# davidskdds/DMSA_LiDAR_SLAM

Measured on AMD Instinct MI355X. Metric: DMSA iterations/sec (10-scan window, 131072 pts/scan), higher is better.
Workload: dtype f32 points/Gaussians, f64 residual sums and normal equations

## Files before the change

### dmsa_lidar_slam_amd/_capi.py

```python
from __future__ import annotations

import ctypes as C
import os

import numpy as np

c_double_p = C.POINTER(C.c_double)
c_float_p = C.POINTER(C.c_float)
c_int32_p = C.POINTER(C.c_int32)
c_int64_p = C.POINTER(C.c_int64)
c_uint32_p = C.POINTER(C.c_uint32)
c_uint64_p = C.POINTER(C.c_uint64)

DMSA_OK = 0
DMSA_ERR_INVALID = -1
DMSA_ERR_NO_DEVICE = -2
DMSA_ERR_HIP = -3
DMSA_ERR_DEPTH = -4
DMSA_ERR_NOMEM = -5

STOP_NUM_ITER, STOP_FEW_GAUSSIANS, STOP_NAN, STOP_NO_IMPROVEMENT, STOP_EPSILON = range(5)

FLAG_POSE_TABLE_HOST = 0x1
FLAG_FIXED_ITERS = 0x2
# ... 262 lines not shown
        "dmsa_window_upload": (C.c_int, [vp, C.POINTER(WindowProblem)]),
        "dmsa_keyframes_upload": (C.c_int, [vp, C.POINTER(KeyframeProblem)]),
        "dmsa_centralize": (C.c_int, [vp]),
        "dmsa_decentralize": (C.c_int, [vp]),
        "dmsa_get_params": (C.c_int, [vp, c_double_p, c_int32_p]),
        "dmsa_set_params": (C.c_int, [vp, c_double_p]),
        "dmsa_additional_errors": (C.c_int, [vp, c_double_p, C.c_int32, c_int32_p]),
        "dmsa_pose_tables": (C.c_int, [vp, C.c_int32, c_double_p, c_float_p]),
        "dmsa_set_pose_tables": (C.c_int, [vp, C.c_int32, c_float_p]),
        "dmsa_num_table_rows": (C.c_int, [vp, c_int32_p]),
        "dmsa_transform_points": (C.c_int, [vp, C.c_int32, c_float_p]),
        "dmsa_build_gaussians": (C.c_int, [vp, C.POINTER(Settings), c_int32_p, c_int64_p]),
        "dmsa_eval_residuals": (C.c_int, [vp, c_double_p]),
        "dmsa_normal_equations": (C.c_int, [vp, C.c_int32, C.c_int32, c_double_p, C.c_double, C.c_double, c_double_p, c_double_p]),
        "dmsa_pose_table_derivatives": (C.c_int, [vp, c_double_p]),
        "dmsa_analytic_jacobian": (C.c_int, [vp, c_double_p, c_double_p]),
        "dmsa_get_voxel_level": (C.c_int, [vp, C.c_int32, C.POINTER(VoxelLevelInfo), c_uint64_p, c_uint32_p, c_int32_p]),
        "dmsa_get_gaussians": (C.c_int, [vp, c_int32_p, c_int32_p, c_float_p, c_float_p]),
        "dmsa_get_timing": (C.c_int, [vp, C.POINTER(Timing), C.c_int32]),
        "dmsa_synchronize": (C.c_int, [vp]),
        "dmsa_get_trace": (C.c_int, [vp, C.POINTER(IterTrace), C.c_int32]),
        "dmsa_detmath_eval": (C.c_int, [vp, C.c_int32, c_double_p, c_double_p, C.c_int64, c_double_p]),
        "dmsa_sort_pairs": (C.c_int, [vp, C.POINTER(C.c_uint32), C.POINTER(C.c_uint32), C.c_int64, C.c_uint32, C.POINTER(C.c_uint32), C.POINTER(C.c_uint32)]),
        "dmsa_leaf_segments": (C.c_int, [vp, C.POINTER(C.c_uint32), C.c_int64, C.c_uint32, c_int32_p, c_int32_p, c_int32_p]),
        "dmsa_serial_fallback_sums": (C.c_int, [vp, C.c_int32, C.POINTER(C.c_uint64)]),
        "dmsa_adaptive_step_size": (C.c_int, [vp, c_double_p, c_double_p, C.c_double, c_int32_p]),
        "dmsa_default_debug_options": (None, [C.POINTER(DebugOptions)]),
        "dmsa_create_ex": (C.c_int, [C.c_int, C.c_uint32, C.POINTER(DebugOptions), C.POINTER(vp)]),
        "dmsa_create_ex2": (C.c_int, [C.c_int, C.c_uint32, C.POINTER(DebugOptions), C.c_uint32, C.POINTER(vp)]),
        "dmsa_create_named": (C.c_int, [C.c_int, C.c_uint32, C.POINTER(DebugOptions), C.c_uint32, C.c_char_p, C.POINTER(vp)]),
        "dmsa_get_debug_counters": (C.c_int, [vp, C.POINTER(DebugCounters)]),
        "dmsa_debug_level_size_classes": (C.c_int, [vp, c_int32_p]),
        "dmsa_debug_next_head": (C.c_int, [vp, c_int64_p]),
        "dmsa_debug_pow_minus_one": (C.c_int, [vp, c_int32_p, C.c_int32, c_float_p]),
        "dmsa_debug_limit_covariance": (C.c_int, [vp, c_float_p, C.c_int64, c_float_p, c_float_p, c_float_p, c_int32_p, c_int32_p]),
        "dmsa_sort_pairs64": (C.c_int, [vp, c_uint64_p, c_uint32_p, C.c_int64, C.c_uint32, c_uint64_p, c_uint32_p]),
        "dmsa_scan_i32": (C.c_int, [vp, c_int32_p, C.c_int64, C.c_int32, c_int32_p]),
        "dmsa_window_upload_aos": (C.c_int, [vp, C.POINTER(WindowProblem), C.POINTER(AosView), C.c_int32, C.POINTER(AosView)]),
        "dmsa_keyframes_upload_aos": (C.c_int, [vp, C.POINTER(KeyframeProblem), C.POINTER(AosView), C.c_int32]),
        "dmsa_optimize_window_aos": (C.c_int, [vp, C.POINTER(WindowProblem), C.POINTER(AosView), C.c_int32, C.POINTER(AosView), C.POINTER(Settings), C.POINTER(Report)]),
        "dmsa_optimize_keyframes_aos": (C.c_int, [vp, C.POINTER(KeyframeProblem), C.POINTER(AosView), C.c_int32, C.POINTER(Settings), C.POINTER(Report)]),
        "dmsa_get_global_points_aos": (C.c_int, [vp, C.c_void_p, C.c_int64, C.c_int32, C.c_int32, C.c_int32]),
        "dmsa_reserve": (C.c_int, [vp, C.c_int64, C.c_int32, C.c_int32]),
        "dmsa_window_ring_push_aos": (C.c_int, [vp, C.POINTER(AosView), C.c_int32]),
        "dmsa_window_upload_from_ring_aos": (C.c_int, [vp, C.POINTER(WindowProblem), C.c_double, C.POINTER(AosView)]),
        "dmsa_window_ring_create": (C.c_int, [vp, C.POINTER(WindowRingConfig)]),
        "dmsa_window_ring_push": (C.c_int, [vp, c_float_p, c_double_p, c_int32_p, C.c_int64]),
        "dmsa_window_ring_points": (C.c_int, [vp, c_int32_p, c_int64_p]),
        "dmsa_window_upload_from_ring": (C.c_int, [vp, C.POINTER(WindowProblem), C.c_double]),
        "dmsa_lm_solve": (C.c_int, [c_double_p, c_double_p, C.c_int32, C.c_double, C.c_int32, c_double_p]),
        "dmsa_lm_solve_device": (C.c_int, [vp, c_double_p, c_double_p, C.c_int32, C.c_double, C.c_double, c_double_p, c_int32_p]),
        "dmsa_neighbourhood_ranges": (C.c_int, [C.c_int32, C.c_int32, C.POINTER(C.c_int32), C.POINTER(C.c_int32)]),
        "dmsa_submap_poses": (C.c_int, [C.c_int32, c_double_p, c_double_p, C.c_int32, C.c_int32, c_double_p, c_double_p, c_double_p, c_double_p]),
        "dmsa_update_poses_from_submap": (C.c_int, [C.c_int32, c_double_p, c_double_p, C.c_int32, C.c_int32, c_double_p, c_double_p]),
        "dmsa_select_static_points": (C.c_int, [vp, C.POINTER(StaticSelectProblem), c_float_p, c_int32_p, C.c_int64, c_int32_p, C.POINTER(StaticSelectResult)]),
        "dmsa_get_overlap": (C.c_int, [vp, c_float_p, C.c_int64, c_float_p, C.c_int64, C.c_float, c_float_p, c_int64_p]),
        "dmsa_random_grid_downsampling": (C.c_int, [vp, c_float_p, C.c_int64, C.c_float, C.c_uint32, c_int32_p, C.c_int64, c_int64_p]),
        "dmsa_radius_exists": (C.c_int, [vp, c_float_p, C.c_int64, c_float_p, C.c_int64, C.c_float, C.POINTER(C.c_uint8)]),
        "dmsa_preprocess_scan": (C.c_int, [vp, c_float_p, C.c_int64, C.POINTER(PreprocessConfig), c_float_p, c_int32_p, C.c_int64, c_int64_p, c_float_p]),
        "dmsa_imu_buffer_create": (C.c_int, [C.c_int32, C.POINTER(vp)]),
        "dmsa_imu_buffer_destroy": (None, [vp]),
        "dmsa_imu_buffer_add": (C.c_int, [vp, c_double_p, c_double_p, C.c_double]),
        "dmsa_imu_buffer_closest": (C.c_int, [vp, C.c_double, c_double_p, c_double_p, c_double_p]),
        "dmsa_imu_buffer_state": (C.c_int, [vp, c_int32_p, c_int32_p, c_double_p, c_double_p, c_double_p]),
        "dmsa_traj_dims": (C.c_int, [C.c_double, C.c_double, C.c_double, c_double_p, c_int32_p]),
        "dmsa_traj_grids": (C.c_int, [C.c_double, C.c_double, C.c_int32, C.c_int32, c_double_p, c_double_p, c_int32_p]),
# ... 42 lines not shown
        "dmsa_pcd_header_normals_binary": (C.c_int, [C.c_int64, C.c_char_p, C.c_int32]),
        "dmsa_dense_cloud_save_pcd_normals": (C.c_int, [vp, C.c_char_p, c_int64_p, c_int64_p]),
        "dmsa_default_dense_outlier_config": (None, [C.POINTER(DenseOutlierConfig)]),
        "dmsa_dense_cloud_knn_mean_distance": (C.c_int, [vp, C.POINTER(DenseOutlierConfig), C.c_int64, C.c_int64, c_float_p]),
        "dmsa_dense_cloud_classify_outliers": (C.c_int, [vp, C.POINTER(DenseOutlierConfig), C.POINTER(C.c_uint8), C.POINTER(DenseOutlierStats)]),
        "dmsa_dense_outlier_threshold": (C.c_int, [C.c_int64, C.c_int64, C.c_int64, C.c_float, c_double_p, c_double_p, c_double_p]),
        "dmsa_dense_cloud_remove_outliers": (C.c_int, [vp, c_int64_p]),
        "dmsa_dense_cloud_save_pcd_retained": (C.c_int, [vp, C.c_char_p, c_int64_p, c_int64_p]),
        "dmsa_default_dense_carve_config": (None, [C.POINTER(DenseCarveConfig)]),
        "dmsa_dense_carve_walk": (C.c_int, [C.c_float, c_float_p, c_float_p, c_int32_p, C.c_int64, c_int64_p]),
        "dmsa_dense_carve_sees_through": (C.c_int, [C.POINTER(DenseCarveConfig), c_float_p, c_float_p, c_float_p]),
        "dmsa_dense_cloud_carve_walk_rows": (C.c_int, [vp, C.POINTER(DenseCarveConfig), C.c_int64, C.c_int64, c_int32_p, c_uint64_p]),
        "dmsa_dense_cloud_count_passes": (C.c_int, [vp, C.POINTER(DenseCarveConfig), c_uint32_p, C.POINTER(DenseCarveStats)]),
        "dmsa_dense_cloud_remove_transients": (C.c_int, [vp, c_int64_p]),
        "dmsa_dense_cloud_with_intensity": (C.c_int, [vp]),
        "dmsa_dense_cloud_has_intensity": (C.c_int, [vp]),
        "dmsa_decode_pointcloud2_field": (C.c_int, [vp, C.POINTER(PointCloud2), C.POINTER(PointCloud2Field), c_float_p]),
        "dmsa_dense_cloud_add_pointcloud2_field": (C.c_int, [vp, C.POINTER(PointCloud2), C.c_int32, C.POINTER(PointCloud2Field), c_float_p, C.c_int64, c_int64_p,
                                                             C.POINTER(DenseStats)]),
        "dmsa_sensor_intensity_field": (C.c_int, [C.c_int32, C.POINTER(PointCloud2Field)]),
        "dmsa_pcd_header_xyzi_binary": (C.c_int, [C.c_int64, C.c_char_p, C.c_int32]),
        "dmsa_pcd_header_xyzi_normals_binary": (C.c_int, [C.c_int64, C.c_char_p, C.c_int32]),
    }
    for name, (res, args) in sig.items():
        fn = getattr(lib, name)
        fn.restype = res
        fn.argtypes = args
    _lib = lib
    return lib


EXPORTED_SYMBOLS = (
    "dmsa_window_upload_aos dmsa_keyframes_upload_aos dmsa_optimize_window_aos dmsa_optimize_keyframes_aos dmsa_get_global_points_aos dmsa_reserve dmsa_window_ring_push_aos dmsa_window_upload_from_ring_aos "
    "dmsa_create dmsa_create_ex dmsa_create_ex2 dmsa_create_named dmsa_default_debug_options dmsa_get_debug_counters dmsa_debug_next_head dmsa_debug_level_size_classes dmsa_debug_pow_minus_one dmsa_debug_limit_covariance dmsa_sort_pairs64 dmsa_scan_i32 dmsa_destroy dmsa_last_error dmsa_default_settings dmsa_optimize_window dmsa_optimize_keyframes "
    "dmsa_get_global_points dmsa_window_upload dmsa_keyframes_upload dmsa_centralize dmsa_decentralize dmsa_get_params "
    "dmsa_set_params dmsa_additional_errors dmsa_pose_tables dmsa_set_pose_tables dmsa_num_table_rows dmsa_transform_points dmsa_build_gaussians "
    "dmsa_eval_residuals dmsa_normal_equations dmsa_pose_table_derivatives dmsa_analytic_jacobian dmsa_get_voxel_level dmsa_get_gaussians dmsa_get_timing dmsa_synchronize dmsa_get_trace dmsa_detmath_eval dmsa_lm_solve dmsa_lm_solve_device dmsa_serial_fallback_sums dmsa_sort_pairs dmsa_leaf_segments dmsa_neighbourhood_ranges dmsa_submap_poses dmsa_update_poses_from_submap dmsa_optimize_resident dmsa_adaptive_step_size dmsa_get_poses "
    "dmsa_select_static_points dmsa_get_overlap dmsa_random_grid_downsampling dmsa_radius_exists dmsa_preprocess_scan "
    "dmsa_imu_buffer_create dmsa_imu_buffer_destroy dmsa_imu_buffer_add dmsa_imu_buffer_closest dmsa_imu_buffer_state dmsa_traj_dims dmsa_traj_grids "
    "dmsa_traj_tform_indices dmsa_traj_transfer_imu dmsa_traj_preint_factors dmsa_traj_update_initial_guess dmsa_traj_submap_gravity_estimate "
    "dmsa_window_ring_create dmsa_window_ring_push dmsa_window_ring_points dmsa_window_upload_from_ring "
    "dmsa_raw_open dmsa_raw_close dmsa_raw_next dmsa_raw_create dmsa_raw_write_pointcloud2 dmsa_raw_write_imu dmsa_raw_finish "
    "dmsa_decode_pointcloud2 dmsa_format_tum_pose dmsa_compose_nonkeyframe_pose dmsa_update_normals dmsa_make_keyframe_cloud "
    "dmsa_get_global_normals dmsa_pcd_header_pointnormal dmsa_format_pcd_rows dmsa_save_pcd_ascii dmsa_save_pcd_ascii_ex"
).split()

DENSE_CLOUD_SYMBOLS = (
    "dmsa_default_dense_config dmsa_dense_cloud_create dmsa_dense_cloud_destroy dmsa_dense_cloud_interpolate dmsa_dense_cloud_add_scan "
    "dmsa_dense_cloud_add_pointcloud2 dmsa_dense_cloud_stats dmsa_dense_cloud_reserve dmsa_dense_cloud_table_info dmsa_pcd_header_xyz_binary "
    "dmsa_dense_cloud_open_pcd dmsa_dense_cloud_close_pcd dmsa_parse_tum_poses"
).split()

DENSE_NORMALS_SYMBOLS = (
    "dmsa_default_dense_normals_config dmsa_dense_cloud_retain dmsa_dense_cloud_retained dmsa_dense_cloud_neighbour_moments "
    "dmsa_dense_cloud_compute_normals dmsa_dense_normal_from_moments dmsa_pcd_header_normals_binary dmsa_dense_cloud_save_pcd_normals"
).split()

DENSE_OUTLIERS_SYMBOLS = (
    "dmsa_default_dense_outlier_config dmsa_dense_cloud_knn_mean_distance dmsa_dense_cloud_classify_outliers dmsa_dense_outlier_threshold "
    "dmsa_dense_cloud_remove_outliers dmsa_dense_cloud_save_pcd_retained"
).split()

DENSE_CARVE_SYMBOLS = (
    "dmsa_default_dense_carve_config dmsa_dense_carve_walk dmsa_dense_carve_sees_through dmsa_dense_cloud_carve_walk_rows "
    "dmsa_dense_cloud_count_passes dmsa_dense_cloud_remove_transients"
).split()

# ... 5 lines not shown
```

### dmsa_lidar_slam_amd/api.py

```python
from __future__ import annotations

import ctypes as C

import numpy as np

from . import _capi as capi
from .problems import ContinuousTrajectory, DmsaOptimSettings, MapManagement


class DmsaError(RuntimeError):
    pass


NAMED_SWITCHES = ("fit_by_level", "batch_stamps", "one_readback", "next_head")


class DmsaOptimizer:

    def __init__(self, device: int = 0, pose_table_host: bool = False, fixed_iters: bool = False, stage_timers: bool = False, debug: dict | None = None):
        self._lib = capi.load_library()
        self._ctx = C.c_void_p()
        flags = (capi.FLAG_POSE_TABLE_HOST if pose_table_host else 0) | (capi.FLAG_FIXED_ITERS if fixed_iters else 0)
        flags |= capi.FLAG_STAGE_TIMERS if stage_timers else 0
        if debug:
            opts = capi.DebugOptions()
            self._lib.dmsa_default_debug_options(C.byref(opts))
            named = []
            for k, v in debug.items():
                if k in NAMED_SWITCHES:
                    named.append(f"{k}={int(v)}")
                elif not hasattr(opts, k):
                    raise KeyError(f"unknown debug switch {k!r} (include/dmsa_debug.h)")
                else:
                    setattr(opts, k, int(v))
            rc = self._lib.dmsa_create_named(int(device), flags, C.byref(opts), C.sizeof(opts), ",".join(named).encode() if named else None, C.byref(self._ctx))
        else:
            rc = self._lib.dmsa_create(int(device), flags, C.byref(self._ctx))
        if rc != capi.DMSA_OK:
            self._ctx = None
            raise DmsaError(f"dmsa_create(device={device}) failed with {rc} (no usable HIP device; there is no CPU fallback)")
        self._problem = None
        self._cprob = None

    def close(self):
        if getattr(self, "_ctx", None):
            self._lib.dmsa_destroy(self._ctx)
            self._ctx = None
# ... 114 lines not shown
        return out

    def limitCovariance(self, cov):
        A = np.ascontiguousarray(np.asarray(cov, np.float32).reshape(-1, 3, 3))
        n = A.shape[0]
        At = np.ascontiguousarray(A.transpose(0, 2, 1))
        out, Vt = np.zeros_like(At), np.zeros_like(At)
        ev = np.zeros((n, 3), np.float32)
        it, info = np.zeros(n, np.int32), np.zeros(n, np.int32)
        self._check(self._lib.dmsa_debug_limit_covariance(self._ctx, capi.ptr(At, C.c_float), n, capi.ptr(out, C.c_float), capi.ptr(ev, C.c_float),
                                                          capi.ptr(Vt, C.c_float), capi.ptr(it, C.c_int32), capi.ptr(info, C.c_int32)), "debug_limit_covariance")
        return np.ascontiguousarray(out.transpose(0, 2, 1)), ev, np.ascontiguousarray(Vt.transpose(0, 2, 1)), it, info

    def optimizeResident(self, settings: DmsaOptimSettings) -> capi.Report:
        cs = settings.to_c()
        rep = capi.Report()
        self._check(self._lib.dmsa_optimize_resident(self._ctx, C.byref(cs), C.byref(rep)), "optimize_resident")
        return rep

    def adaptiveStepSize(self, params, step, error0: float):
        p = np.ascontiguousarray(params, np.float64).copy()
        st = np.ascontiguousarray(step, np.float64)
        k = C.c_int32()
        self._check(self._lib.dmsa_adaptive_step_size(self._ctx, capi.ptr(p, C.c_double), capi.ptr(st, C.c_double), float(error0), C.byref(k)), "adaptive_step_size")
        return p, int(k.value)

    def debugCounters(self) -> dict:
        c = capi.DebugCounters()
        self._check(self._lib.dmsa_get_debug_counters(self._ctx, C.byref(c)), "get_debug_counters")
        out = {n: int(getattr(c, n)) for n, _ in c._fields_}
        head = np.zeros(2, np.int64)
        self._check(self._lib.dmsa_debug_next_head(self._ctx, capi.ptr(head, C.c_int64)), "debug_next_head")
        out["next_head_iterations"], out["next_head_mismatches"] = int(head[0]), int(head[1])
        return out

    def levelSizeClasses(self):
        out = np.zeros(9, np.int32)
        self._check(self._lib.dmsa_debug_level_size_classes(self._ctx, capi.ptr(out, C.c_int32)), "debug_level_size_classes")
        return out[:8].reshape(2, 4).copy(), bool(out[8])

    def lastError(self) -> str:
        msg = self._lib.dmsa_last_error(self._ctx)
        return msg.decode() if msg else ""

    def poses(self):
        p = self._problem
        n = p.relOrientations.shape[0]
        ro, rt = np.zeros((n, 3)), np.zeros((n, 3))
        self._check(self._lib.dmsa_get_poses(self._ctx, capi.ptr(ro, C.c_double), capi.ptr(rt, C.c_double)), "get_poses")
        return ro, rt

    def globalPoints(self) -> np.ndarray:
        n = self._num_points()
        out = np.zeros((n, 4), np.float32)
        self._check(self._lib.dmsa_get_global_points(self._ctx, capi.ptr(out, C.c_float), n), "get_global_points")
        return out

    def getGlobalNormals(self) -> np.ndarray:
        n = self._num_points()
        out = np.zeros((n, 4), np.float32)
        self._check(self._lib.dmsa_get_global_normals(self._ctx, capi.ptr(out, C.c_float), n), "get_global_normals")
        return out

    def upload(self, pointSet):
        cp = pointSet.to_c()
        if isinstance(pointSet, ContinuousTrajectory):
# ... 210 lines not shown
```

### dmsa_lidar_slam_amd/csrc/context.cpp

```cpp
#include "dmsa_ctx.h"

#include <cstddef>

WorkerPool& workers(dmsa_ctx* ctx) {
    if (!ctx->pool) {
        const unsigned want = (unsigned)std::max(1, ctx->dbg.host_threads);
        ctx->pool = new WorkerPool((int)std::min(want, std::max(2u, std::thread::hardware_concurrency())));
    }
    return *ctx->pool;
}
hipEvent_t get_event(dmsa_ctx* ctx) {
    if (!ctx->free_events.empty()) {
        hipEvent_t e = ctx->free_events.back();
        ctx->free_events.pop_back();
        return e;
    }
    hipEvent_t e;
    (void)hipEventCreate(&e);
    return e;
}
void drain_timers(dmsa_ctx* ctx) {
    std::vector<EventPair> later;
    for (auto& ev : ctx->pending) {
        if (hipEventQuery(ev.b) == hipErrorNotReady) {
// ... 324 lines not shown
    SW(key_compress, 1, kMin, kMax),
    SW(fused_segments, 1, kMin, kMax),
    SW(sort_prehist, 0, kMin, kMax),
    SW(overlap_batch, 1, kMin, kMax),
    SW(serial_tree, 1, 0, 3),
    SW(host_threads, 16, 1, 64),
    SW(solve_threads, 12, 1, 16),
    SW(host_timeline, 0, kMin, kMax),
    SW(trace_time, 0, kMin, kMax),
    SW(fused_leaf_scan, 1, kMin, kMax),
    SW(device_sync, 1, kMin, kMax),
    SW(shared_rotations, 1, kMin, kMax),
    SW(eval_skip, 1, kMin, kMax),
    SW(sync_fault, 0, kMin, kMax),
    SW(speculation_fault, 0, kMin, kMax),
    SW(voxel_coherence, 0, kMin, kMax),
    SW(lm_stream, 1, kMin, kMax),
    SW(stream_priority, 0, kMin, kMax),
    SW(gap_stamps, 0, kMin, kMax),
    SW(lattice_hint, 1, kMin, kMax),
    SW(fit_classes, 7, kMin, kMax),
    SW(eigen_l1_bytes, 32 * 1024, 4096, kMax, true),
    SW(small_threshold, 0, kMin, kMax),
    SW(skip_stats, 0, kMin, kMax),
    SW(small_voxel, 0, kMin, kMax),
    SW(long_split, 1, kMin, kMax),
    SW(long_log2, 0, kMin, kMax),
    SW(sort_items, 0, kMin, kMax),
    SW(trial_rows_aside, 1, kMin, kMax),
    {"batch_stamps", sizeof(dmsa_debug_options), 1, 0, 1},
    {"one_readback", sizeof(dmsa_debug_options) + 4, 1, 0, 1},
    {"fit_by_level", sizeof(dmsa_debug_options) + 8, 1, 0, 2},
    {"next_head", sizeof(dmsa_debug_options) + 12, 1, 0, 3},
};
#undef SW
constexpr size_t kNumSwitches = sizeof(kSwitches) / sizeof(kSwitches[0]);
static_assert(kNumSwitches == sizeof(dmsa_switches) / 4 && sizeof(dmsa_switches) == sizeof(dmsa_debug_options) + 16, "one table row per field of dmsa_switches");
constexpr bool switches_in_struct_order() {
    for (size_t i = 0; i < kNumSwitches; ++i)
        if (kSwitches[i].offset != 4 * i) return false;
    return true;
}
static_assert(switches_in_struct_order(), "row i of the table describes field i of dmsa_switches");
int32_t& value(dmsa_switches* o, const Switch& sw) { return *reinterpret_cast<int32_t*>(reinterpret_cast<char*>(o) + sw.offset); }
bool is_public(const Switch& sw) { return sw.offset < sizeof(dmsa_debug_options); }
int32_t& public_value(dmsa_debug_options* o, const Switch& sw) { return *reinterpret_cast<int32_t*>(reinterpret_cast<char*>(o) + sw.offset); }
}

extern "C" {

void dmsa_default_debug_options(dmsa_debug_options* o) {
    if (!o) return;
    for (const Switch& sw : kSwitches)
        if (is_public(sw)) public_value(o, sw) = sw.def;
}
static void apply_named_switches(dmsa_switches* o, const char* e, const char* where) {
    if (!e) return;
    std::string text(e);
    size_t at = 0;
    while (at < text.size()) {
        size_t end = text.find(',', at);
        if (end == std::string::npos) end = text.size();
        const std::string item = text.substr(at, end - at);
        const size_t eq = item.find('=');
        if (eq != std::string::npos) {
            const std::string name = item.substr(0, eq);
            bool known = false;
            for (const Switch& sw : kSwitches)
                if (name == sw.name) value(o, sw) = std::atoi(item.c_str() + eq + 1), known = true;
            if (!known) std::fprintf(stderr, "[dmsa] %s: unknown switch '%s' ignored\n", where, name.c_str());
// ... 10 lines not shown
}
int dmsa_create_named(int device, uint32_t flags, const dmsa_debug_options* options, uint32_t options_bytes, const char* named, dmsa_ctx** out) {
    if (!out) return DMSA_ERR_INVALID;
    dmsa_switches dbg;
    for (const Switch& sw : kSwitches) value(&dbg, sw) = sw.def;
    if (options) {
        if (options_bytes < 4 || options_bytes % 4 != 0 || options_bytes > sizeof(dmsa_debug_options)) return DMSA_ERR_INVALID;
        std::memcpy(static_cast<dmsa_debug_options*>(&dbg), options, options_bytes);
    }
    apply_named_switches(&dbg, named, "dmsa_create_named");
    apply_named_switches(&dbg, std::getenv("DMSA_DEBUG"), "DMSA_DEBUG");
    for (const Switch& sw : kSwitches) {
        int32_t& v = value(&dbg, sw);
        v = v < sw.lo ? (sw.low_is_default ? sw.def : sw.lo) : std::min(v, sw.hi);
    }
    *out = nullptr;
    int count = 0;
    if (hipGetDeviceCount(&count) != hipSuccess || count <= 0 || device < 0 || device >= count) return DMSA_ERR_NO_DEVICE;
    if (hipSetDevice(device) != hipSuccess) return DMSA_ERR_NO_DEVICE;
    dmsa_ctx* ctx = new (std::nothrow) dmsa_ctx();
    if (!ctx) return DMSA_ERR_NOMEM;
    if (flags & ~(DMSA_FLAG_POSE_TABLE_HOST | DMSA_FLAG_FIXED_ITERS | DMSA_FLAG_MIRROR_SUMS | DMSA_FLAG_STAGE_TIMERS)) {
        delete ctx;
        return DMSA_ERR_INVALID;
    }
    ctx->device = device, ctx->flags = flags;
    ctx->dbg = dbg;
    int prio_least = 0, prio_greatest = 0;
    (void)hipDeviceGetStreamPriorityRange(&prio_least, &prio_greatest);
    auto make_stream = [&](hipStream_t* st, int bit) {
        return hipStreamCreateWithPriority(st, hipStreamNonBlocking, ((dbg.stream_priority >> bit) & 1) ? prio_greatest : prio_least / 2 + prio_greatest / 2);
    };
    bool made = make_stream(&ctx->stream, 0) == hipSuccess && make_stream(&ctx->stream2, 1) == hipSuccess && make_stream(&ctx->stream3, 2) == hipSuccess &&
                hipEventCreateWithFlags(&ctx->ev_counts, hipEventDisableTiming) == hipSuccess;
    for (StreamDep* d : ctx->deps) made = made && d->create_events() == hipSuccess;
    if (!made) {
        dmsa_destroy(ctx);
        return DMSA_ERR_HIP;
    }
    if (ctx->h_rb.ensure(sizeof(dmsa_ctx::Readback), nullptr) != hipSuccess) {
        dmsa_destroy(ctx);
        return DMSA_ERR_NOMEM;
    }
    std::memset(ctx->h_rb.p, 0, sizeof(dmsa_ctx::Readback));
    ctx->h_lattice = ctx->rb()->lattice;
    if (hipDeviceGetAttribute(&ctx->wall_clock_khz, hipDeviceAttributeWallClockRate, device) != hipSuccess || ctx->wall_clock_khz <= 0)
        ctx->wall_clock_khz = 0, ctx->dbg.batch_stamps = 0;
    if (ctx->d_sync.ensure(SYNC_SLOTS * 4) != hipSuccess || hipMemsetAsync(ctx->d_sync.p, 0, SYNC_SLOTS * 4, ctx->stream) != hipSuccess ||
        ctx->d_batch_clock.ensure(16) != hipSuccess || hipMemsetAsync(ctx->d_batch_clock.p, 0, 16, ctx->stream) != hipSuccess || hipStreamSynchronize(ctx->stream) != hipSuccess) {
        dmsa_destroy(ctx);
        return DMSA_ERR_HIP;
    }
    *out = ctx;
    return DMSA_OK;
}

void dmsa_destroy(dmsa_ctx* ctx) {
    if (!ctx) return;
    (void)hipSetDevice(ctx->device);
    for (hipStream_t st : {ctx->stream, ctx->stream2, ctx->stream3})
        if (st) (void)hipStreamSynchronize(st);
    drain_timers(ctx);
    for (hipEvent_t e : ctx->free_events) (void)hipEventDestroy(e);
    if (ctx->ev_counts) (void)hipEventDestroy(ctx->ev_counts);
    delete ctx->pool;
    pcd_release(ctx);
    delete ctx->sp;
    for (hipStream_t st : {ctx->stream3, ctx->stream2, ctx->stream})
        if (st) (void)hipStreamDestroy(st);
    delete ctx;
}

const char* dmsa_last_error(const dmsa_ctx* ctx) { return ctx ? ctx->err.c_str() : "null context"; }

void dmsa_default_settings(dmsa_settings* s) {
    if (!s) return;
    s->num_iter = 15, s->epsilon = 1e-5, s->use_analytic_jacobi = 0, s->step_length_optim = 0.05, s->max_step = 0.01, s->gauss_split = 0;
    s->grid_size_1_factor = 2.0f, s->grid_size_2_factor = 5.0f, s->min_num_points_per_set = 6, s->min_num_gaussians = 30;
    s->lambda_diag = 0.00001f, s->use_centralization = 1;
}

int dmsa_window_upload(dmsa_ctx* ctx, const dmsa_window_problem* p) {
    if (!ctx || !p || p->num_points < 0 || p->num_static < 0) return DMSA_ERR_INVALID;
    if ((p->num_points > 0 && (!p->xyz_local || !p->tform_idx || !p->ring_id)) || (p->num_static > 0 && (!p->xyz_static || !p->ring_id_static))) {
        ctx->err = "invalid window problem (null point arrays)";
        return DMSA_ERR_INVALID;
    }
    CHK(window_upload_begin(ctx, p, p->num_points, p->num_static));
    const size_t n = (size_t)ctx->n;
    CHK(ensure_stage(ctx, n * 20 + 64));
    float* loc = ctx->h_stage.as<float>();
    int32_t* ring = reinterpret_cast<int32_t*>(ctx->h_stage.as<char>() + n * 16);
    const int32_t id_row = p->n_total;
    const int64_t N = ctx->N, S = ctx->S;
    std::atomic<bool> bad_row{false};
    auto pack = [&](int64_t i0, int64_t i1) {
        for (int64_t i = i0; i < i1; ++i) {
            if (i < N) {
                const int32_t row = p->tform_idx[i];
                if (row < 0 || row >= p->n_total) {
                    bad_row = true;
// ... 61 lines not shown
```

### dmsa_lidar_slam_amd/csrc/dev_sync.h

```cpp
#pragma once
#include <hip/hip_runtime.h>

#include <cstdint>

namespace dmsa {

struct DevSync {
    const uint32_t* wait_counter = nullptr;
    uint32_t wait_target = 0;
    uint32_t* signal_counter = nullptr;
    int32_t* timed_out = nullptr;
};

struct BatchStamp {
    const long long* begin = nullptr;
    unsigned long long* ticks = nullptr;
};

enum SyncSlot : int {
    SYNC_TIER_FORK = 0,
    SYNC_TIER_JOIN = 1,
    SYNC_TIMED_OUT = 2,
    SYNC_LOOP_STATE = 5,
    SYNC_TABLES = 6,
    SYNC_CLASSES = 7,
    SYNC_LATTICE = 8,
    SYNC_LEVEL1 = 9,
    SYNC_SMALL_L0 = 10,
    SYNC_TRIAL_STEP = 11,
    SYNC_TRIAL_ROWS = 12,
    SYNC_SIZES0 = 13,
    SYNC_SIZES1 = 14,
    SYNC_CLASSES0 = 15,
    SYNC_CLASSES1 = 16,
    SYNC_FIT1 = 17,
    SYNC_BATCH_BEGIN = 18,
    SYNC_SLOTS = 24
};

#if defined(__HIPCC__)
__device__ __forceinline__ void dev_sync_signal(uint32_t* counter) {
    __threadfence();
    __hip_atomic_fetch_add(counter, 1u, __ATOMIC_RELAXED, __HIP_MEMORY_SCOPE_AGENT);
}
constexpr int kSyncMaxSpins = 1 << 23;
__device__ __forceinline__ void dev_sync_wait(const uint32_t* counter, uint32_t target, int32_t* timed_out, int max_spins = kSyncMaxSpins) {
    uint32_t v = 0;
    for (int spin = 0; spin < max_spins; ++spin) {
        v = __hip_atomic_load(counter, __ATOMIC_RELAXED, __HIP_MEMORY_SCOPE_AGENT);
        if ((int32_t)(v - target) >= 0) {
            __builtin_amdgcn_fence(__ATOMIC_ACQUIRE, "agent");
            return;
        }
        if (spin < 4096)
            __builtin_amdgcn_s_sleep(1);
        else
            __builtin_amdgcn_s_sleep(8);
    }
    if (timed_out != nullptr) timed_out[0] = 1, timed_out[1] = (int32_t)target, timed_out[2] = (int32_t)v;
}
__device__ __forceinline__ void dev_sync_enter(const DevSync& sy) {
    if (sy.wait_counter != nullptr && threadIdx.x == 0) dev_sync_wait(sy.wait_counter, sy.wait_target, sy.timed_out);
}
__device__ __forceinline__ void dev_sync_leave(const DevSync& sy) {
    if (sy.signal_counter != nullptr) {
        __syncthreads();
        if (threadIdx.x == 0) dev_sync_signal(sy.signal_counter);
    }
}
// ... 9 lines not shown
```

### dmsa_lidar_slam_amd/csrc/dmsa_api.cpp

```cpp
#include "dmsa_ctx.h"

extern "C" {


int dmsa_centralize(dmsa_ctx* ctx) {
    if (!ctx || ctx->model == MODEL_NONE) return DMSA_ERR_INVALID;
    if (ctx->model == MODEL_KEYFRAMES) return DMSA_OK;
    if (ctx->centralized) return DMSA_OK;
    CHK(set_device(ctx));
    WindowHost& w = ctx->win;
    w.origin = {w.ctrl.rel_t[0], w.ctrl.rel_t[1], w.ctrl.rel_t[2]};
    w.ctrl.rel_t[0] = w.ctrl.rel_t[1] = w.ctrl.rel_t[2] = 0.0;
    w.ctrl.relative_to_global();
    launch_shift_points(ctx->d_local.as<float4>() + ctx->N, ctx->S, (float)w.origin.x, (float)w.origin.y, (float)w.origin.z, -1.0f, ctx->stream);
    HIPCHK(hipGetLastError());
    ctx->centralized = true;
    return DMSA_OK;
}

int dmsa_decentralize(dmsa_ctx* ctx) {
    if (!ctx || ctx->model == MODEL_NONE) return DMSA_ERR_INVALID;
    if (ctx->model == MODEL_KEYFRAMES) return DMSA_OK;
    if (!ctx->centralized) return DMSA_OK;
    CHK(set_device(ctx));
// ... 367 lines not shown
    out->skip_pairs = (int64_t)st[0], out->skip_pairs_equal = (int64_t)st[1], out->skip_mismatches = (int64_t)st[2];
    unsigned long long sp[2] = {0, 0};
    if (ctx->d_split_stats.p) {
        unsigned long long stripes[128];
        HIPCHK(hipStreamSynchronize(ctx->stream));
        HIPCHK(hipStreamSynchronize(ctx->stream2));
        HIPCHK(hipMemcpy(stripes, ctx->d_split_stats.p, sizeof(stripes), hipMemcpyDeviceToHost));
        for (int k = 0; k < 64; ++k) sp[0] += stripes[2 * k], sp[1] += stripes[2 * k + 1];
    }
    out->split_blocks = (int64_t)sp[0], out->split_blocks_skipped = (int64_t)sp[1];
    unsigned long long changed = 0;
    if (ctx->d_coh_count.p) {
        HIPCHK(hipStreamSynchronize(ctx->stream));
        HIPCHK(hipMemcpy(&changed, ctx->d_coh_count.p, 8, hipMemcpyDeviceToHost));
    }
    out->voxel_codes_compared = ctx->coh_compared, out->voxel_codes_changed = (int64_t)changed, out->voxel_lattice_changes = ctx->coh_lattice_changes;
    out->lattice_hints_held = ctx->lattice_hints_held, out->lattice_replays = ctx->lattice_replays;
    out->small_voxel_launches = ctx->small_voxel_launches, out->small_voxel_fallbacks = ctx->small_voxel_fallbacks;
    return DMSA_OK;
}

int dmsa_debug_next_head(dmsa_ctx* ctx, int64_t* out2) {
    if (!ctx || !out2) return DMSA_ERR_INVALID;
    CHK(set_device(ctx));
    unsigned long long differing = 0;
    if (ctx->d_head_mismatches.p) {
        HIPCHK(hipStreamSynchronize(ctx->stream));
        HIPCHK(hipMemcpy(&differing, ctx->d_head_mismatches.p, 8, hipMemcpyDeviceToHost));
    }
    out2[0] = ctx->next_head_iterations, out2[1] = (int64_t)differing;
    return DMSA_OK;
}

int dmsa_debug_level_size_classes(dmsa_ctx* ctx, int32_t* out9) {
    if (!ctx || !out9) return DMSA_ERR_INVALID;
    std::memset(out9, 0, 9 * sizeof(int32_t));
    if (!ctx->gaussians_valid || !ctx->fit_guess_level) return DMSA_OK;
    for (int l = 0; l < 2; ++l) {
        const SerialCounts& c = ctx->serial_counts_level[l];
        out9[4 * l] = c.n_long, out9[4 * l + 1] = c.n_chain - c.n_long, out9[4 * l + 2] = c.n_small, out9[4 * l + 3] = c.max_members;
    }
    out9[8] = 1;
    return DMSA_OK;
}

int dmsa_get_timing(dmsa_ctx* ctx, dmsa_timing* t, int32_t reset) {
    if (!ctx) return DMSA_ERR_INVALID;
    CHK(set_device(ctx));
    HIPCHK(enqueue_batch_ticks(ctx));
    HIPCHK(hipStreamSynchronize(ctx->stream));
    drain_timers(ctx);
    if (t) {
        t->residual_kernel_ms = ctx->t_ms[T_RESIDUAL], t->residual_launches = ctx->residual_launches, t->residual_evaluations = ctx->residual_evals;
        t->residual_algorithmic_bytes = ctx->residual_bytes;
        t->residual_unit_bytes = ctx->residual_unit_bytes;
        t->voxelize_ms = ctx->t_ms[T_VOXEL], t->gaussian_fit_ms = ctx->t_ms[T_FIT], t->pose_table_ms = ctx->t_ms[T_TABLE];
        t->normal_eq_ms = ctx->t_ms[T_NORMAL], t->total_ms = ctx->t_ms[T_TOTAL];
    }
    if (reset) {
        for (double& v : ctx->t_ms) v = 0.0;
        ctx->residual_launches = 0, ctx->residual_evals = 0, ctx->residual_bytes = 0.0, ctx->residual_unit_bytes = 0.0;
    }
    return DMSA_OK;
}

int dmsa_sort_pairs(dmsa_ctx* ctx, const uint32_t* keys, const uint32_t* values, int64_t n, uint32_t end_bit, uint32_t* keys_sorted, uint32_t* values_sorted) {
// ... 207 lines not shown
```

### dmsa_lidar_slam_amd/csrc/dmsa_ctx.h

```cpp
#pragma once
#include <hip/hip_runtime.h>

#include <algorithm>
#include <atomic>
#include <cassert>
#include <chrono>
#include <cmath>
#include <condition_variable>
#include <cstddef>
#include <cstdio>
#include <cstdlib>
#include <cstring>
#include <functional>
#include <limits>
#include <mutex>
#include <string>
#include <thread>
#include <vector>

#include "../../include/dmsa_hip.h"
#include "../../include/dmsa_debug.h"
#include "../../include/dmsa_static_points.h"
#include "../../include/dmsa_window_setup.h"
#include "../../include/dmsa_wire_formats.h"
// ... 210 lines not shown
    long generation_ = 0;
    bool stop_ = false;
};

struct WindowRing {
    int num_scans = 0;
    int64_t cap = 0;
    int head = 0, filled = 0;
    std::vector<int64_t> count;
    DevBuf xyz, stamp, id;
};

struct HostTimeline {
    bool on = false;
    std::vector<std::pair<const char*, std::chrono::steady_clock::time_point>> marks;
    void reset() { marks.clear(); }
    void mark(const char* what) {
        if (on) marks.emplace_back(what, std::chrono::steady_clock::now());
    }
    void print() const {
        if (!on || marks.size() < 2) return;
        std::fprintf(stderr, "[host timeline]");
        for (size_t i = 1; i < marks.size(); ++i)
            std::fprintf(stderr, " %s %.0f |", marks[i].first, std::chrono::duration<double, std::micro>(marks[i].second - marks[i - 1].second).count());
        std::fprintf(stderr, " total %.0f us\n", std::chrono::duration<double, std::micro>(marks.back().second - marks.front().second).count());
    }
};

struct dmsa_switches : dmsa_debug_options {
    int32_t batch_stamps = 1;
    int32_t one_readback = 1;
    int32_t fit_by_level = 1;
    int32_t next_head = 1;
};

struct dmsa_ctx {
    int device = 0;
    uint32_t flags = 0;
    WindowRing ring;
    dmsa_switches dbg{};
    hipStream_t stream = nullptr, stream2 = nullptr;
    hipStream_t stream3 = nullptr;
    StreamDep tier_fork{this, SYNC_TIER_FORK, 1}, tier_join{this, SYNC_TIER_JOIN, 2} , loop_state{this, SYNC_LOOP_STATE, 1},
        tables{this, SYNC_TABLES, 1}, classes{this, SYNC_CLASSES, 1}, lattice{this, SYNC_LATTICE, 1}, level1{this, SYNC_LEVEL1, 1}, small_l0{this, SYNC_SMALL_L0, 0},
        trial_step{this, SYNC_TRIAL_STEP, 0}, trial_rows{this, SYNC_TRIAL_ROWS, 0}, sizes0{this, SYNC_SIZES0, 1}, sizes1{this, SYNC_SIZES1, 1},
        classes0{this, SYNC_CLASSES0, 1}, classes1{this, SYNC_CLASSES1, 1}, fit1{this, SYNC_FIT1, 1};
    StreamDep* const deps[15] = {&tier_fork, &tier_join, &loop_state, &tables, &classes, &lattice, &level1, &small_l0, &trial_step, &trial_rows,
                                 &sizes0, &sizes1, &classes0, &classes1, &fit1};
    int tablesT_batch = 0;
    hipEvent_t ev_counts = nullptr;
    std::string err;

    Model model = MODEL_NONE;
    int64_t n = 0, N = 0, S = 0;
    int rows = 0;
    WindowHost win;
    KeyframeHost key;
    bool centralized = false;
    float min_grid_size = 0.3f;

    DevBuf d_local, d_nlocal, d_ring, d_global, d_nglobal;
    DevBuf d_tables, d_ctrl, d_stamps, d_fhw, d_trajtime;
    int batch = 0;
    PinnedRing h_pin, h_xpin;
    std::vector<float> h_tables;
    PinnedBuf h_stage;
    DevBuf d_aabb, d_code[2], d_idx[2], d_code_s[2], d_idx_s[2], d_head[2], d_leaf_incl[2], d_leaf_start[2], d_slot_acc[2], d_slot_cnt[2],
        d_gauss_of_slot[2], d_memb_of_slot[2], d_pos_slot_rank[2], d_nsorted[2], d_pair_d[2], d_sort_tmp[2], d_scan_tmp[2];
    struct Readback {
        LatticeTable lattice[2];
        GaussCounts g;
        SerialCounts sc;
        SerialCounts sc_level[2];
        IterResult prev;
        double errs[16];
        unsigned long long batch_ticks;
    };
    static constexpr size_t kReadbackBytes = offsetof(Readback, errs);
    DevBuf d_readback;
    DevView d_lattice, d_counts;
    IterResult* d_prev_result() const { return reinterpret_cast<IterResult*>(d_readback.as<char>() + offsetof(Readback, prev)); }
// ... 26 lines not shown
    int64_t lattice_hints_held = 0, lattice_replays = 0;
    DevBuf d_fit_sums;
    DevBuf d_memb_q;
    DevBuf d_pow_codes;
    int64_t pow_n = 0;
    DevBuf d_gauss_rows;
    DevBuf d_row_range;
    DevBuf d_skip_stats;
    int skip_stats_evals = 0;
    DevBuf d_code_prev[2], d_coh_count;
    LatticeTable coh_lattice[2]{};
    bool coh_valid[2] = {false, false}, coh_key32[2] = {false, false}, coh_pending[2] = {false, false}, coh_count_zeroed = false;
    int64_t coh_n[2] = {0, 0};
    int64_t coh_compared = 0, coh_lattice_changes = 0;
    DevBuf d_split_stats;
    int64_t skip_pairs = 0;
    bool fit_guess_valid = false;
    SerialCounts serial_counts{0, 0, 0, 0};
    SerialCounts serial_counts_level[2] = {{0, 0, 0, 0}, {0, 0, 0, 0}};
    bool fit_guess_level = false;
    bool E_is_jacobian = false;
    bool aabb_fresh = false;
    const float* base_table = nullptr;
    LoopModel loop_model{};
    DevBuf d_imu_idx, d_imu_rot, d_imu_pos, d_imu_vel, d_imu_cov;
    DevBuf d_key_grav, d_key_plaus, d_key_odom_t, d_key_odom_R;
    DevBuf d_loop_state;
    DevBuf d_loop_vec;
    DevBuf d_ctrl0;
    DevBuf d_table0;
    DevBuf d_trial_tables;
    DevBuf d_head_check, d_head_mismatches;
    int64_t next_head_iterations = 0;
    DevBuf d_loop_extra;
    DevBuf d_loop_iter;
    DevBuf d_panel_work;
    uint32_t panel_epoch = 0;
    int panel_P = -1;
    DevBuf d_rot_same;
    DevBuf d_sync;
    int wait_seq = 0;
    long long* stamp_voxel = nullptr;
    long long* stamp_fit = nullptr;
    int voxel_calls = 0;
    int small_voxel_launches = 0, small_voxel_fallbacks = 0;
    int sync_retries = 0, speculation_retries = 0;
    DevBuf d_aos_raw, d_aos_idx;
    DevBuf d_static_keep;
    DevBuf d_ctrl_pm, d_dT;
    PinnedBuf h_results;
    const void* rb_extra_src = nullptr;
    void* rb_extra_dst = nullptr;
    size_t rb_extra_bytes = 0;
    int M = 0, M1 = 0;
    int64_t Mm = 0;
    bool gaussians_valid = false;
    DevBuf d_E, d_ne_partial, d_Hp, d_sq_partial, d_sq_out;
    int64_t ldE = 0;
    int extra_rows = 0;
    DevBuf d_batch_clock;
    unsigned long long batch_ticks_seen = 0;
    int wall_clock_khz = 0;
    bool batch_ticks_dirty = false, batch_ticks_in_flight = false;
    std::vector<EventPair> pending;
    std::vector<hipEvent_t> free_events;
    double t_ms[T_COUNT] = {0, 0, 0, 0, 0, 0};
// ... 40 lines not shown
        if (!on) return;
        (void)hipEventRecord(ev.b, ctx->stream);
        ctx->pending.push_back(ev);
    }
};
void drain_timers(dmsa_ctx* ctx);
hipError_t enqueue_batch_ticks(dmsa_ctx* ctx);
hipError_t sync_spin(hipStream_t stream);
int set_device(dmsa_ctx* ctx);
bool sync_wait_timed_out(dmsa_ctx* ctx, std::string* what);
int num_params(const dmsa_ctx* ctx);
PoseChain& chain(dmsa_ctx* ctx);
int num_extra_rows(const dmsa_ctx* ctx);
int alloc_point_buffers(dmsa_ctx* ctx);
int upload_powm1_codes(dmsa_ctx* ctx, int64_t counts);
int upload_loop_model(dmsa_ctx* ctx);
int upload_common(dmsa_ctx* ctx);
void write_back_poses(const PoseChain& c, double* rel_o, double* rel_t);
int ensure_stage(dmsa_ctx* ctx, size_t bytes);
int window_upload_begin(dmsa_ctx* ctx, const dmsa_window_problem* p, int64_t N, int64_t S);
int window_upload_finish(dmsa_ctx* ctx, const dmsa_window_problem* p);
int keyframes_upload_begin(dmsa_ctx* ctx, const dmsa_keyframe_problem* p, int64_t n_points);
int keyframes_upload_finish(dmsa_ctx* ctx, const dmsa_keyframe_problem* p);
int pointcloud2_layout(const dmsa_pointcloud2* msg, int32_t sensor, PointCloud2Fields* f_out, uint64_t* n_out);
int pointcloud2_field_layout(const dmsa_pointcloud2* msg, uint32_t index, uint32_t datatype, uint32_t* offset_out);
void pcd_release(dmsa_ctx* ctx);
int build_gaussians(dmsa_ctx* ctx, const dmsa_settings& s, const std::function<int()>& overlap = nullptr, bool allow_speculation = true,
                    bool allow_compression = true, bool allow_small = true);
int build_tables(dmsa_ctx* ctx, int B, const std::vector<double>& globs, hipStream_t stream = nullptr);
void append_glob(const PoseChain& c, std::vector<double>& out);
void host_set_params(dmsa_ctx* ctx, const double* p);
int transform_points(dmsa_ctx* ctx, int b);
int ensure_E(dmsa_ctx* ctx, int B);
int run_residuals(dmsa_ctx* ctx, int B, const std::vector<double>* extra, const double* d_extra = nullptr, const uint32_t* rot_same = nullptr,
                  const int2* row_range = nullptr );
int device_lm_step(dmsa_ctx* ctx, const double* d_Hp, int P, double lambda, double alpha, double max_step, double* d_step, LoopFlags* d_flags);
constexpr double kTableDerivStep = 1e-5;
int check_analytic_jacobian(dmsa_ctx* ctx, int P);
int host_table_derivatives(dmsa_ctx* ctx, hipStream_t stream);
int upload_extra(dmsa_ctx* ctx, const std::vector<double>& extra, int B);
int analytic_columns(dmsa_ctx* ctx, int P, double inv_h, const float* table0);
int optimize(dmsa_ctx* ctx, const dmsa_settings& s, dmsa_report* rep);
int adaptive_step_size(dmsa_ctx* ctx, double* params, const double* step, double error0, int32_t* best_k);
```

### dmsa_lidar_slam_amd/csrc/dmsa_kernels.h

```cpp
#pragma once
#include <hip/hip_runtime.h>
#include <cstdint>

#include "dev_sync.h"

namespace dmsa {

constexpr int kMaxLatticeEvents = 64;
constexpr int kAabbBlock = 1024;
constexpr uint32_t kStaticRowFlag = 0;

struct LatticeTable {
    int32_t num_events;
    int32_t final_depth;
    int32_t status;
    int32_t defined;
    int64_t first_idx;
    int64_t event_idx[kMaxLatticeEvents + 1];
    double mn[kMaxLatticeEvents + 1][3];
    uint32_t suffix_shift[kMaxLatticeEvents + 1][3];
    int32_t depth[kMaxLatticeEvents + 1];
    double final_mn[3];
    int32_t nbits[3];
    int32_t total_bits;
    uint32_t key_base[3];
    int32_t compressed;
    int32_t out_of_range;
    int32_t pad3;
    uint64_t code_or;
};
__host__ __device__ inline uint64_t lattice_invalid_code(const LatticeTable& t) {
    return (1ull << (t.compressed ? t.total_bits : 3 * t.final_depth)) | t.code_or;
}

struct LevelCounts {
    int32_t num_leaves;
    int32_t num_gauss;
    int32_t num_memb;
    int32_t pad;
};

struct GaussCounts {
// ... 15 lines not shown
    uint32_t* code_s[2];
    uint32_t* idx_s[2];
    GaussCounts* counts;
    float4* memb_local;
    int32_t* memb_idx;
    int32_t* memb_g;
    int32_t* seg_off;
    uint32_t* sync;
    uint32_t sync_target;
    int32_t* timed_out;
    long long* stamps;
};
int small_voxel_max_points();
void launch_voxel_small(const SmallVoxelArgs& a, hipStream_t s);

void launch_transform(const float4* local, const float4* table, float4* global, int64_t n, hipStream_t s);
void launch_transform_normals(const float4* local, const float4* nlocal, const float4* table, float4* global, float4* nglobal, int64_t n, hipStream_t s);
void launch_shift_points(float4* pts, int64_t n, float ox, float oy, float oz, float sign, hipStream_t s);

void launch_window_pose_tables(const double* ctrl, const double* stamps, const double* fh_w, const double* traj_time, int B, int C, int n_t,
                               float* tables, float* tablesT , hipStream_t s,
                               uint32_t* rot_same = nullptr );
void launch_keyframe_pose_tables(const double* frames, int B, int F, float* tables, float* tablesT, hipStream_t s, uint32_t* rot_same = nullptr);
void launch_window_pose_table_deriv(const double* ctrl_pm, const double* stamps, const double* fh_w, const double* traj_time, int P, int C, int n_t, double h,
                                    double* dT, hipStream_t s);
void launch_keyframe_pose_table_deriv(const double* ctrl_pm, int P, int F, double h, double* dT, hipStream_t s);

void launch_detmath_eval(int fn, const double* x, const double* y, int64_t n, double* out, hipStream_t s);

void launch_transform_aabb(const float4* local, const float4* nlocal, const float4* table, float4* global, float4* nglobal, int64_t n, float* aabb, void* zero,
                           size_t zero_bytes, hipStream_t s);
void launch_transform_aabb_adopt(const float4* local, float4* table0, const float4* trials, int rows, const int32_t* head_k, float4* global, int64_t n,
                                 float* aabb, void* zero, size_t zero_bytes, hipStream_t s);
void launch_count_word_mismatches(const void* a, const void* b, int words, unsigned long long* count, hipStream_t s);
void launch_block_aabb(const float4* global, int64_t n, float* aabb , void* zero, size_t zero_bytes, hipStream_t s);
void launch_lattice(const float4* global, int64_t n, const float* aabb, int nb, double res0, double res1, bool compress, LatticeTable* tables ,
                    void* sort_header0, void* sort_header1, hipStream_t s, uint32_t* done = nullptr ,
                    bool use_hint = false );
struct SortPlan;
void launch_voxel_keys(const float4* global, int64_t n, LatticeTable* table, double res, void* code, bool key32, uint32_t* idx, uint64_t code_or,
                       const SortPlan* sort, hipStream_t s);
void launch_head_flags(const void* code_sorted, bool key32, int64_t n, const LatticeTable* table, int32_t* head, hipStream_t s);
struct ChainedScanCall {
    unsigned long long* state;
    uint32_t epoch, ticket_base;
};
constexpr int kLeafSegmentWords = 1, kLeafFinalizeWords = 4;
int leaf_segment_tiles(int64_t n);
void launch_leaf_segments(const void* code_sorted, bool key32, int64_t n, const LatticeTable* table, int32_t* leaf_incl, int32_t* leaf_start, LevelCounts* counts,
                          const ChainedScanCall& call, hipStream_t s);
void launch_leaf_starts(const int32_t* head, const int32_t* leaf_of_pos, const void* code_sorted, bool key32, const LatticeTable* table, int64_t n,
                        int32_t* leaf_start, LevelCounts* counts, hipStream_t s);
void launch_leaf_accept(const int32_t* leaf_start, const uint32_t* idx_sorted, const int32_t* ring, const LevelCounts* counts, int min_pts,
                        int64_t capacity , int32_t* slot_acc , int32_t* slot_cnt, hipStream_t s);
size_t split_scratch_bytes(int64_t n);
void launch_leaf_split(const int32_t* leaf_incl, const int32_t* leaf_start, const uint32_t* idx_sorted, const int32_t* ring, const float4* nglobal,
                       const LevelCounts* counts, int min_pts, int64_t n, float4* nsorted , unsigned long long* pair_best ,
                       int32_t* slot_acc, int32_t* slot_cnt, int32_t* pos_slot_rank, hipStream_t s,
                       unsigned long long* block_stats = nullptr );
void launch_leaf_scan(const int32_t* slot_acc, const int32_t* slot_cnt, int32_t* gauss_of_slot, int32_t* memb_of_slot, LevelCounts* counts, hipStream_t s);
int leaf_finalize_tiles(int64_t n);
void launch_leaf_finalize(const int32_t* slot_acc, const int32_t* slot_cnt, int64_t n , int32_t* gauss_of_slot, int32_t* memb_of_slot,
                          LevelCounts* counts, const ChainedScanCall& call, hipStream_t s,
                          int32_t* gauss_size = nullptr );
void launch_count_code_changes(const void* now, void* prev, bool key32, int64_t n, bool compare, unsigned long long* count, hipStream_t s);
void launch_gather_members(const int32_t* leaf_of_pos, const int32_t* leaf_start, const uint32_t* idx_sorted, const void* code_sorted, bool key32,
                           const LatticeTable* table, const int32_t* slot_acc, const int32_t* gauss_of_slot, const int32_t* memb_of_slot,
                           const int32_t* pos_slot_rank , const float4* local, const int32_t* slot_cnt, const GaussCounts* counts, int level,
                           int64_t n, float4* memb_local, int32_t* memb_idx, int32_t* memb_g, int32_t* seg_off, hipStream_t s,
                           uint32_t* start_signal = nullptr );
void launch_gauss_fit_all(const float4* memb_local, const int32_t* seg_off, const float* table0, const uint32_t* order, const int32_t* sc, const int first[3],
                          const int tasks[3], float* sums, GaussCounts* counts, float* info12, bool with_weights, int id_row, int2* gauss_rows, int eigen_l1_bytes,
                          const uint32_t* pow_codes, int pow_n, float* memb_q , size_t q_stride, hipStream_t s,
                          const int32_t* size0 = nullptr, const int32_t* size1 = nullptr );
// ... 24 lines not shown
```

### dmsa_lidar_slam_amd/csrc/dmsa_kernels.hip

```cpp
#include "dmsa_kernels.h"
#include "dev_sync.h"
#include "k1_pose_math.h"
#include "radix_sort_dev.h"
#include "wave_prims.h"
#include "chained_scan.h"

#include <cfloat>
#include <climits>
#include <type_traits>
#include <cmath>
#include <cstdlib>
#include <cstring>
#include <cstdio>

#include "../../include/dmsa_detmath.h"
#include "../../include/dmsa_hip.h"

namespace dmsa {

__global__ __launch_bounds__(256) void k_transform(const float4* __restrict__ local, const float4* __restrict__ table, float4* __restrict__ global,
                                                   int64_t n) {
    const int64_t stride = (int64_t)gridDim.x * blockDim.x;
    for (int64_t i = (int64_t)blockIdx.x * blockDim.x + threadIdx.x; i < n; i += stride) {
        const float4 p = local[i];
// ... 305 lines not shown
        }
    }
    const int wave = threadIdx.x >> 6, lane = threadIdx.x & 63;
    for (int a = 0; a < 3; ++a) {
        mn[a] = wave_allminf(mn[a]);
        mx[a] = wave_allmaxf(mx[a]);
    }
    if (lane == 0)
        for (int a = 0; a < 3; ++a) s_red[wave][a] = mn[a], s_red[wave][3 + a] = mx[a];
    __syncthreads();
    if (threadIdx.x < 6) {
        float v = s_red[0][threadIdx.x];
        for (int w = 1; w < 4; ++w) v = threadIdx.x < 3 ? fminf(v, s_red[w][threadIdx.x]) : fmaxf(v, s_red[w][threadIdx.x]);
        aabb[(size_t)blockIdx.x * 8 + threadIdx.x] = v;
    }
}
template <bool kNormals>
__global__ __launch_bounds__(256) void k_transform_aabb(const float4* __restrict__ local, const float4* __restrict__ nlocal, const float4* __restrict__ table,
                                                        float4* __restrict__ global, float4* __restrict__ nglobal, int64_t n, float* __restrict__ aabb,
                                                        uint32_t* __restrict__ zero, int zero_words) {
    transform_aabb_body<kNormals>(local, nlocal, table, global, nglobal, n, aabb, zero, zero_words);
}
__global__ __launch_bounds__(256) void k_transform_aabb_adopt(const float4* __restrict__ local, float4* table0, const float4* trials, int table_f4,
                                                              const int32_t* __restrict__ head_k, float4* __restrict__ global, int64_t n,
                                                              float* __restrict__ aabb, uint32_t* __restrict__ zero, int zero_words) {
    const int k = *head_k;
    const float4* table = table0;
    if (k > 0) {
        table = trials + (size_t)(k - 1) * table_f4;
        for (int i = blockIdx.x * 256 + threadIdx.x; i < table_f4; i += gridDim.x * 256) table0[i] = table[i];
    }
    transform_aabb_body<false>(local, nullptr, table, global, nullptr, n, aabb, zero, zero_words);
}
__global__ __launch_bounds__(256) void k_count_word_mismatches(const uint32_t* __restrict__ a, const uint32_t* __restrict__ b, int words,
                                                               unsigned long long* __restrict__ count) {
    const int i = blockIdx.x * 256 + threadIdx.x;
    if (i < words && a[i] != b[i]) atomicAdd(count, 1ull);
}
void launch_transform_aabb_adopt(const float4* local, float4* table0, const float4* trials, int rows, const int32_t* head_k, float4* global, int64_t n,
                                 float* aabb, void* zero, size_t zero_bytes, hipStream_t s) {
    const int nb = (int)((n + kAabbBlock - 1) / kAabbBlock);
    hipLaunchKernelGGL(k_transform_aabb_adopt, dim3(nb), dim3(256), 0, s, local, table0, trials, 3 * rows, head_k, global, n, aabb, static_cast<uint32_t*>(zero),
                       (int)(zero_bytes / 4));
}
void launch_count_word_mismatches(const void* a, const void* b, int words, unsigned long long* count, hipStream_t s) {
    if (words > 0)
        hipLaunchKernelGGL(k_count_word_mismatches, dim3((words + 255) / 256), dim3(256), 0, s, static_cast<const uint32_t*>(a), static_cast<const uint32_t*>(b),
                           words, count);
}
void launch_transform_aabb(const float4* local, const float4* nlocal, const float4* table, float4* global, float4* nglobal, int64_t n, float* aabb, void* zero,
                           size_t zero_bytes, hipStream_t s) {
    if (n <= 0) {
        if (zero_bytes) (void)hipMemsetAsync(zero, 0, zero_bytes, s);
        return;
    }
    const int nb = (int)((n + kAabbBlock - 1) / kAabbBlock);
    if (nlocal)
        hipLaunchKernelGGL(k_transform_aabb<true>, dim3(nb), dim3(256), 0, s, local, nlocal, table, global, nglobal, n, aabb, static_cast<uint32_t*>(zero),
                           (int)(zero_bytes / 4));
    else
        hipLaunchKernelGGL(k_transform_aabb<false>, dim3(nb), dim3(256), 0, s, local, nlocal, table, global, nglobal, n, aabb, static_cast<uint32_t*>(zero),
                           (int)(zero_bytes / 4));
}
void launch_block_aabb(const float4* global, int64_t n, float* aabb, void* zero, size_t zero_bytes, hipStream_t s) {
    if (n <= 0) {
        if (zero_bytes) (void)hipMemsetAsync(zero, 0, zero_bytes, s);
        return;
    }
    const int nb = (int)((n + kAabbBlock - 1) / kAabbBlock);
    hipLaunchKernelGGL(k_block_aabb, dim3(nb), dim3(256), 0, s, global, n, aabb, static_cast<uint32_t*>(zero), (int)(zero_bytes / 4));
}

struct LatticeRun {
    double mn[3], mx[3];
    int depth, defined, nev, status;
};

__device__ void lattice_adopt(LatticeRun& st, const float4 p, const double res, int64_t idx, LatticeTable* tab, uint32_t (*shifts)[3]) {
    const double eps = (double)FLT_EPSILON;
    const float pc[3] = {p.x, p.y, p.z};
    while (true) {
// ... 18 lines not shown
            side = (double)(1u << st.depth) * res - eps;
            for (int a = 0; a < 3; ++a) st.mx[a] = st.mn[a] + side;
            tab->event_idx[st.nev] = idx;
            st.nev += 1;
            for (int a = 0; a < 3; ++a) tab->mn[st.nev][a] = st.mn[a];
            tab->depth[st.nev] = st.depth;
        } else {
            for (int a = 0; a < 3; ++a) {
                st.mn[a] = (double)pc[a] - res / 2;
                st.mx[a] = (double)pc[a] + res / 2;
            }
            unsigned mk[3];
            for (int a = 0; a < 3; ++a) mk[a] = (unsigned)ceil((st.mx[a] - st.mn[a] - eps) / res);
            const unsigned mv = max(max(max(mk[0], mk[1]), mk[2]), 2u);
            st.depth = (int)max(min(32u, (unsigned)ceil(log((double)mv) / log(2.0) - eps)), 0u);
            const double side = (double)(1u << st.depth) * res;
            for (int a = 0; a < 3; ++a) {
                const double over = (side - (st.mx[a] - st.mn[a])) / 2.0;
                if (over > eps) {
                    st.mn[a] -= over;
                    st.mx[a] += over;
                }
            }
            st.defined = 1;
            tab->first_idx = idx;
            for (int a = 0; a < 3; ++a) tab->mn[0][a] = st.mn[a];
            tab->depth[0] = st.depth;
        }
    }
}

constexpr int kLatticeThreads = 1024;
constexpr int kLatticeLdsBlocks = 2048;
__global__ __launch_bounds__(kLatticeThreads) void k_lattice(const float4* __restrict__ global, int64_t n, const float* __restrict__ aabb, int nb, double res0,
                                                            double res1, int compress, LatticeTable* __restrict__ tables, uint32_t* __restrict__ sort_header0,
                                                            uint32_t* __restrict__ sort_header1, uint32_t* done ,
                                                            int use_hint ) {
    static_assert(kLatticeThreads == kAabbBlock, "one thread per point of a block");
#ifdef DMSA_LATTICE_TIMING
    const long long lt0 = wall_clock64();
#define LAT_STAMP(k) if (threadIdx.x == 0) tables[blockIdx.x].mn[kMaxLatticeEvents - 8 + (k)][0] = (double)(wall_clock64() - lt0);
#else
#define LAT_STAMP(k)
#endif
    {
        uint32_t* h = blockIdx.x == 0 ? sort_header0 : sort_header1;
        if (h != nullptr)
            for (unsigned i = threadIdx.x; i < sizeof(SortHeader) / 4; i += kLatticeThreads) h[i] = 0u;
    }
    constexpr int kWaves = kLatticeThreads / 64;
    __shared__ float s_glob[kWaves][6];
    __shared__ LatticeRun st;
    __shared__ uint32_t s_shift[kMaxLatticeEvents][3];
    __shared__ int s_red[2][kWaves];
    __shared__ float s_bb[kLatticeLdsBlocks][6];
    int red_phase = 0;
    LatticeTable* tab = tables + blockIdx.x;
    const double res = blockIdx.x == 0 ? res0 : res1;
    const int tid = threadIdx.x, wave = tid >> 6, lane = tid & 63;
    if (tid == 0) {
        st.defined = 0, st.depth = 0, st.nev = 0, st.status = 0;
        for (int a = 0; a < 3; ++a) st.mn[a] = 0.0, st.mx[a] = 0.0;
        if (!use_hint) tab->first_idx = -1;
    }
    __shared__ int s_ok, s_E, s_nown;
    __shared__ long long s_ev[kMaxLatticeEvents + 1];
    __shared__ long long s_own[kMaxLatticeEvents + 1];
    __shared__ float4 s_q[kMaxLatticeEvents + 1];
    __shared__ double s_bmn[kMaxLatticeEvents + 1][3], s_bmx[kMaxLatticeEvents + 1][3];
    __shared__ double s_tmn[kMaxLatticeEvents + 1][3];
    __shared__ int s_tdepth[kMaxLatticeEvents + 1], s_hdr[3];
    __shared__ int s_e0[kMaxLatticeEvents + 2];
    __shared__ float s_fmn[kMaxLatticeEvents + 1][3], s_fmx[kMaxLatticeEvents + 1][3];
    if (use_hint && tid >= kLatticeThreads - 128 && tid - (kLatticeThreads - 128) <= kMaxLatticeEvents) {
        const int t = tid - (kLatticeThreads - 128);
        s_tdepth[t] = tab->depth[t];
        for (int a = 0; a < 3; ++a) s_tmn[t][a] = tab->mn[t][a];
        if (t < kMaxLatticeEvents) s_ev[1 + t] = tab->event_idx[t];
        if (t == 0) s_hdr[0] = tab->num_events, s_hdr[1] = tab->status, s_hdr[2] = tab->defined, s_ev[0] = tab->first_idx;
    }
    {
        float g6[6] = {INFINITY, INFINITY, INFINITY, -INFINITY, -INFINITY, -INFINITY};
        for (int b2 = tid; b2 < nb; b2 += kLatticeThreads) {
            const float4 lo = *reinterpret_cast<const float4*>(aabb + (size_t)b2 * 8), hi = *reinterpret_cast<const float4*>(aabb + (size_t)b2 * 8 + 4);
            const float bb[6] = {lo.x, lo.y, lo.z, lo.w, hi.x, hi.y};
            if (b2 < kLatticeLdsBlocks)
                for (int a = 0; a < 6; ++a) s_bb[b2][a] = bb[a];
            if (bb[0] <= bb[3])
                for (int a = 0; a < 3; ++a) g6[a] = fminf(g6[a], bb[a]), g6[3 + a] = fmaxf(g6[3 + a], bb[3 + a]);
        }
        for (int a = 0; a < 3; ++a) g6[a] = wave_allminf(g6[a]), g6[3 + a] = wave_allmaxf(g6[3 + a]);
        if (lane == 0)
            for (int a = 0; a < 6; ++a) s_glob[wave][a] = g6[a];
    }
    __syncthreads();
    auto block_min = [&](int v) {
        v = wave_allmin(v);
        if (lane == 0) s_red[red_phase][wave] = v;
        __syncthreads();
        int m = s_red[red_phase][0];
#pragma unroll
        for (int w = 1; w < kWaves; ++w) m = min(m, s_red[red_phase][w]);
        red_phase ^= 1;
        return m;
    };
    LAT_STAMP(0)
    constexpr int kHintBlocks = 12;
    bool verified = false;
    if (use_hint) {
        if (tid == 0) {
            const int E = s_hdr[0];
            const long long first = s_ev[0];
            int ok = s_hdr[1] == 0 && s_hdr[2] == 1 && E >= 0 && E <= kMaxLatticeEvents && first >= 0 && first < n && n < (1ll << 31) - kAabbBlock;
            int nown = 0;
            if (ok) {
                long long prev = first;
                s_own[nown] = first / kAabbBlock, s_e0[nown] = 0, nown += 1;
                for (int e = 0; e < E; ++e) {
                    const long long ie = s_ev[1 + e];
                    ok = ok && ie > first && ie >= prev && ie < n;
                    if (ok && ie / kAabbBlock != s_own[nown - 1]) s_own[nown] = ie / kAabbBlock, s_e0[nown] = e, nown += 1;
                    prev = ie;
                }
                s_e0[nown] = E;
            }
            ok = ok && nown <= kHintBlocks;
            s_ok = ok, s_E = ok ? E : 0, s_nown = ok ? nown : 0;
        }
        __syncthreads();
        LAT_STAMP(1)
        if (s_ok && tid <= s_E) s_q[tid] = global[s_ev[tid]];
        float4 own_pt[kHintBlocks];
        const int nown = s_nown;
#pragma unroll
        for (int k = 0; k < kHintBlocks; ++k) {
            const long long pi = k < nown ? s_own[k] * kAabbBlock + tid : n;
            own_pt[k] = pi < n ? global[pi] : make_float4(NAN, NAN, NAN, 0.0f);
        }
        __syncthreads();
        LAT_STAMP(2)
        if (s_ok && tid == 0) {
            const int E = s_E;
            const double eps = (double)FLT_EPSILON;
            LatticeRun c;
            c.defined = 0, c.depth = 0, c.nev = 0, c.status = 0;
            int ok = 1;
            {
                const float4 q = s_q[0];
                const float pc[3] = {q.x, q.y, q.z};
                ok = ok && isfinite(q.x) && isfinite(q.y) && isfinite(q.z);
                for (int a = 0; a < 3; ++a) c.mn[a] = (double)pc[a] - res / 2, c.mx[a] = (double)pc[a] + res / 2;
                unsigned mk[3];
                for (int a = 0; a < 3; ++a) mk[a] = (unsigned)ceil((c.mx[a] - c.mn[a] - eps) / res);
                const unsigned mv = max(max(max(mk[0], mk[1]), mk[2]), 2u);
                c.depth = (int)max(min(32u, (unsigned)ceil(log((double)mv) / log(2.0) - eps)), 0u);
                const double side = (double)(1u << c.depth) * res;
                for (int a = 0; a < 3; ++a) {
                    const double over = (side - (c.mx[a] - c.mn[a])) / 2.0;
                    if (over > eps) c.mn[a] -= over, c.mx[a] += over;
                }
                c.defined = 1;
                for (int a = 0; a < 3; ++a) ok = ok && __double_as_longlong(c.mn[a]) == __double_as_longlong(s_tmn[0][a]);
                ok = ok && c.depth == s_tdepth[0];
                for (int a = 0; a < 3; ++a) s_bmn[0][a] = c.mn[a], s_bmx[0][a] = c.mx[a];
            }
            for (int e = 0; e < E && ok; ++e) {
                const float4 q = s_q[1 + e];
                const float pc[3] = {q.x, q.y, q.z};
                ok = ok && isfinite(q.x) && isfinite(q.y) && isfinite(q.z);
                bool lo[3], hi[3], viol = false;
// ... 65 lines not shown
#pragma unroll
            for (int k = 0; k < kHintBlocks; ++k) {
                if (k < nown) {
                    const float4 q = own_pt[k];
                    const int base = (int)s_own[k] * kAabbBlock, e0 = s_e0[k], e1 = s_e0[k + 1];
                    float imn[3] = {s_fmn[e0][0], s_fmn[e0][1], s_fmn[e0][2]}, imx[3] = {s_fmx[e0][0], s_fmx[e0][1], s_fmx[e0][2]};
                    for (int e = e0 + 1; e <= e1; ++e)
                        for (int a = 0; a < 3; ++a) imn[a] = fmaxf(imn[a], s_fmn[e][a]), imx[a] = fminf(imx[a], s_fmx[e][a]);
                    const bool inside0 = base + tid > first32 && q.x >= imn[0] && q.x < imx[0] && q.y >= imn[1] && q.y < imx[1] && q.z >= imn[2] && q.z < imx[2];
                    if (!inside0 && isfinite(q.x) && isfinite(q.y) && isfinite(q.z)) {
                        int ep = e0;
                        bool trig = base + tid == first32;
                        for (int e = e0; e < e1; ++e) {
                            const int le = (int)s_ev[1 + e] - base;
                            ep += le < tid ? 1 : 0, trig = trig || le == tid;
                        }
                        const float c3[3] = {q.x, q.y, q.z};
                        if (base + tid < first32)
                            bad = 1;
                        else if (!trig && !fits(c3, c3, ep))
                            bad = 1;
                    }
                }
            }
            verified = block_min(bad ? 0 : 1) == 1;
        }
        LAT_STAMP(4)
        __syncthreads();
        if (!verified && tid == 0) {
            st.defined = 0, st.depth = 0, st.nev = 0, st.status = 0;
            for (int a = 0; a < 3; ++a) st.mn[a] = 0.0, st.mx[a] = 0.0;
            tab->first_idx = -1;
        }
        __syncthreads();
    }
    LAT_STAMP(5)
    int cursor = verified ? nb : 0;
    while (cursor < nb) {
        int found = INT_MAX;
        for (int base = cursor; base < nb; base += kLatticeThreads) {
            const int blk = base + tid;
            int cand = INT_MAX;
            if (blk < nb) {
                float bb[6];
                if (blk < kLatticeLdsBlocks) {
                    for (int a = 0; a < 6; ++a) bb[a] = s_bb[blk][a];
                } else {
                    for (int a = 0; a < 6; ++a) bb[a] = aabb[(size_t)blk * 8 + a];
                }
                if (bb[0] <= bb[3]) {
                    bool viol = !st.defined;
                    for (int a = 0; a < 3; ++a) viol = viol || (double)bb[a] < st.mn[a] || (double)bb[3 + a] >= st.mx[a];
                    if (viol) cand = blk;
                }
            }
            const int m = block_min(cand);
            if (m != INT_MAX) {
                found = m;
                break;
            }
        }
        if (found == INT_MAX) break;
        const int64_t pi = (int64_t)found * kAabbBlock + tid;
        float4 p = float4{0.0f, 0.0f, 0.0f, 0.0f};
        bool live = false;
        if (pi < n) {
            p = global[pi];
            live = isfinite(p.x) && isfinite(p.y) && isfinite(p.z);
        }
        int from = 0;
        while (true) {
            int cand = INT_MAX;
            if (live && tid >= from) {
                bool viol = !st.defined;
                viol = viol || (double)p.x < st.mn[0] || (double)p.x >= st.mx[0];
                viol = viol || (double)p.y < st.mn[1] || (double)p.y >= st.mx[1];
                viol = viol || (double)p.z < st.mn[2] || (double)p.z >= st.mx[2];
                if (viol) cand = tid;
            }
            const int m = block_min(cand);
            if (m == INT_MAX) break;
            if (tid == m) lattice_adopt(st, p, res, pi, tab, s_shift);
            __syncthreads();
            if (st.status != 0) break;
            from = m + 1;
        }
        if (st.status != 0) break;
        cursor = found + 1;
    }
    __syncthreads();
    LAT_STAMP(6)
    if (tid == 0) {
        tab->num_events = st.nev;
        tab->final_depth = st.depth;
        tab->status = st.status;
        tab->defined = st.defined;
        for (int a = 0; a < 3; ++a) tab->final_mn[a] = st.mn[a];
        int total = 0;
        for (int a = 0; a < 3; ++a) {
            float lo = s_glob[0][a], hi = s_glob[0][3 + a];
            for (int w = 1; w < kWaves; ++w) lo = fminf(lo, s_glob[w][a]), hi = fmaxf(hi, s_glob[w][3 + a]);
            int bits = st.depth;
            uint32_t base = 0;
            if (st.defined && lo <= hi) {
                const long long maxk = (1ll << st.depth) - 1;
                long long klo = (long long)floor(((double)lo - st.mn[a]) / res) - 1, khi = (long long)floor(((double)hi - st.mn[a]) / res) + 1;
                klo = klo < 0 ? 0 : klo, khi = khi > maxk ? maxk : khi;
                bits = 0;
                while (bits < st.depth && (klo >> bits) != (khi >> bits)) ++bits;
                base = (uint32_t)(klo >> bits);
            }
            tab->nbits[a] = bits, tab->key_base[a] = base;
            total += bits;
        }
        tab->compressed = compress, tab->out_of_range = 0, tab->code_or = 0;
        tab->pad3 = verified ? 1 : 0;
        tab->total_bits = total;
        uint32_t acc[3] = {0, 0, 0};
        for (int a = 0; a < 3; ++a) tab->suffix_shift[st.nev][a] = 0;
        for (int e = st.nev - 1; e >= 0; --e)
            for (int a = 0; a < 3; ++a) {
                acc[a] += s_shift[e][a];
                tab->suffix_shift[e][a] = acc[a];
            }
    }
    LAT_STAMP(7)
    if (done != nullptr) {
        __syncthreads();
        if (threadIdx.x == 0) dev_sync_signal(done);
    }
}
void launch_lattice(const float4* global, int64_t n, const float* aabb, int nb, double res0, double res1, bool compress, LatticeTable* tables,
                    void* sort_header0, void* sort_header1, hipStream_t s, uint32_t* done, bool use_hint) {
    hipLaunchKernelGGL(k_lattice, dim3(2), dim3(kLatticeThreads), 0, s, global, n, aabb, nb, res0, res1, compress ? 1 : 0, tables,
                       static_cast<uint32_t*>(sort_header0), static_cast<uint32_t*>(sort_header1), done, use_hint ? 1 : 0);
}

__device__ __forceinline__ uint64_t spread3(uint32_t v) {
    uint64_t x = v & 0x1fffffull;
    x = (x | x << 32) & 0x1f00000000ffffull;
    x = (x | x << 16) & 0x1f0000ff0000ffull;
    x = (x | x << 8) & 0x100f00f00f00f00full;
    x = (x | x << 4) & 0x10c30c30c30c30c3ull;
    x = (x | x << 2) & 0x1249249249249249ull;
    return x;
}

template <typename KeyT>
__global__ __launch_bounds__(256) void k_voxel_keys(const float4* __restrict__ global, int64_t n, LatticeTable* __restrict__ table, double res,
                                                    KeyT* __restrict__ code, uint32_t* __restrict__ idx, uint64_t code_or, SortHeader* __restrict__ sort_header,
                                                    uint32_t* __restrict__ sort_state, size_t sort_state_words, int sort_passes, uint32_t sort_last_mask) {
    __shared__ LatticeTable t;
    __shared__ uint32_t s_h[kSortMaxPasses][kSortBins];
    const bool counting = sort_header != nullptr && sizeof(KeyT) == 4;
    if (counting) {
        for (int p = 0; p < kSortMaxPasses; ++p) s_h[p][threadIdx.x] = 0u;
        for (size_t i = (size_t)blockIdx.x * blockDim.x + threadIdx.x; i < sort_state_words; i += (size_t)gridDim.x * blockDim.x) sort_state[i] = 0u;
    }
    {
        const int words = sizeof(LatticeTable) / 4;
        const uint32_t* src = reinterpret_cast<const uint32_t*>(table);
        uint32_t* dst = reinterpret_cast<uint32_t*>(&t);
        for (int i = threadIdx.x; i < words; i += blockDim.x) dst[i] = src[i];
    }
    __syncthreads();
    if (threadIdx.x == 0) t.code_or = code_or;
    if (blockIdx.x == 0 && threadIdx.x == 0) table->code_or = code_or;
    __syncthreads();
    const int nev = t.num_events;
    const uint64_t invalid = lattice_invalid_code(t);
    const int nx = t.nbits[0], ny = t.nbits[1], nz = t.nbits[2];
    const int maxb = max(nx, max(ny, nz));
    const int64_t last_ev = nev > 0 ? t.event_idx[nev - 1] : -1;
    const int64_t stride = (int64_t)gridDim.x * blockDim.x;
    for (int64_t i = (int64_t)blockIdx.x * blockDim.x + threadIdx.x; i < n; i += stride) {
        const float4 p = global[i];
        uint64_t c = invalid;
        if (isfinite(p.x) && isfinite(p.y) && isfinite(p.z)) {
            int e = nev;
            if (i < last_ev) {
                e = 0;
                while (e < nev && t.event_idx[e] <= i) ++e;
            }
            const uint32_t mask = (1u << t.depth[e]) - 1u;
            const uint32_t kx = ((uint32_t)(((double)p.x - t.mn[e][0]) / res) & mask) + t.suffix_shift[e][0];
            const uint32_t ky = ((uint32_t)(((double)p.y - t.mn[e][1]) / res) & mask) + t.suffix_shift[e][1];
            const uint32_t kz = ((uint32_t)(((double)p.z - t.mn[e][2]) / res) & mask) + t.suffix_shift[e][2];
            if (t.compressed) {
                if ((kx >> nx) != t.key_base[0] || (ky >> ny) != t.key_base[1] || (kz >> nz) != t.key_base[2]) table->out_of_range = 1;
                uint64_t cc = 0;
                for (int l = maxb - 1; l >= 0; --l) {
                    if (l < nx) cc = (cc << 1) | ((kx >> l) & 1u);
                    if (l < ny) cc = (cc << 1) | ((ky >> l) & 1u);
                    if (l < nz) cc = (cc << 1) | ((kz >> l) & 1u);
                }
                c = cc | code_or;
            } else {
                c = (spread3(kx) << 2) | (spread3(ky) << 1) | spread3(kz) | code_or;
            }
        }
        code[i] = (KeyT)c;
        idx[i] = (uint32_t)i;
        if (counting) sort_hist_add(s_h, sort_passes, sort_last_mask, (uint32_t)c, true);
    }
    if (counting) {
        __syncthreads();
        for (int p = 0; p < sort_passes; ++p) {
            const uint32_t v = s_h[p][threadIdx.x];
            if (v) atomicAdd(&sort_header->hist[p][threadIdx.x], v);
        }
    }
}
void launch_voxel_keys(const float4* global, int64_t n, LatticeTable* table, double res, void* code, bool key32, uint32_t* idx, uint64_t code_or,
                       const SortPlan* sort, hipStream_t s) {
    if (n <= 0) return;
    SortHeader* h = sort && key32 ? sort->header : nullptr;
    if (key32)
        hipLaunchKernelGGL(k_voxel_keys<uint32_t>, dim3(grid_for(n, 256)), dim3(256), 0, s, global, n, table, res, (uint32_t*)code, idx, code_or, h,
                           h ? sort->tile_state : nullptr, h ? sort->state_words : (size_t)0, h ? sort->passes : 0, h ? sort->last_mask : 255u);
    else
        hipLaunchKernelGGL(k_voxel_keys<uint64_t>, dim3(grid_for(n, 256)), dim3(256), 0, s, global, n, table, res, (uint64_t*)code, idx, code_or,
                           (SortHeader*)nullptr, (uint32_t*)nullptr, (size_t)0, 0, 255u);
}

template <typename KeyT>
__global__ __launch_bounds__(256) void k_count_code_changes(const KeyT* __restrict__ now, KeyT* __restrict__ prev, int64_t n, int compare, unsigned long long* __restrict__ count) {
    const int64_t i = (int64_t)blockIdx.x * blockDim.x + threadIdx.x;
    bool diff = false;
    if (i < n) {
        const KeyT c = now[i];
        diff = compare && prev[i] != c;
        prev[i] = c;
    }
    const unsigned long long m = __ballot(diff);
    if ((threadIdx.x & 63) == 0 && m) atomicAdd(count, (unsigned long long)__popcll(m));
}
void launch_count_code_changes(const void* now, void* prev, bool key32, int64_t n, bool compare, unsigned long long* count, hipStream_t s) {
    if (n <= 0) return;
    const dim3 grid((unsigned)((n + 255) / 256));
    if (key32)
        hipLaunchKernelGGL(k_count_code_changes<uint32_t>, grid, dim3(256), 0, s, (const uint32_t*)now, (uint32_t*)prev, n, compare ? 1 : 0, count);
    else
        hipLaunchKernelGGL(k_count_code_changes<uint64_t>, grid, dim3(256), 0, s, (const uint64_t*)now, (uint64_t*)prev, n, compare ? 1 : 0, count);
}

template <typename KeyT>
__global__ __launch_bounds__(256) void k_head_flags(const KeyT* __restrict__ code, int64_t n, const LatticeTable* __restrict__ table,
                                                    int32_t* __restrict__ head) {
    const KeyT invalid = (KeyT)lattice_invalid_code(*table);
    const int64_t stride = (int64_t)gridDim.x * blockDim.x;
// ... 1990 lines not shown
```

### dmsa_lidar_slam_amd/csrc/loop_kernels.h

```cpp
#pragma once
#include <hip/hip_runtime.h>
#include <cstdint>

#include "dev_sync.h"
#include "pose_math.h"

namespace dmsa {

struct LoopModel {
    int model;
    int n;
    int P;
    int extra;
    const double* stamps;
    const double* fhw;
    const double* traj_time;
    ImuConsts imu;
    KeyframeRowConsts key;
};

inline size_t loop_state_doubles(int n) { return 12 * (size_t)n; }

struct IterResult {
    int32_t stop;
// ... 2 lines not shown
};
struct LoopFlags {
    int32_t stop;
    int32_t nan;
    int32_t head_k;
    int32_t pad;
};

bool loop_chain_fits(const LoopModel& m);
void launch_loop_begin(const LoopModel& m, double* state0, double* paramVec, double* ctrl0, LoopFlags* flags, hipStream_t s,
                       uint32_t* state_ready = nullptr );
void launch_loop_chain(const LoopModel& m, int mode, const double* state_in, double* state_out, const double* paramVec, const double* step, double increment,
                       double* ctrl, double* extra, const LoopFlags* flags, hipStream_t s,
                       int part = 0 ,
                       uint32_t* start_signal = nullptr );
void launch_loop_chain_central(const LoopModel& m, const double* state_in, double h, double* ctrl, const LoopFlags* flags, hipStream_t s);
void launch_loop_scatter_extra(const double* extra, int B, int a, double* E, int64_t ldE, int M, hipStream_t s);
constexpr int kLoopSolveMaxP = 64;
void launch_loop_lm_step(const double* Hp, int P, double lambda, double alpha, double max_step, double* step, LoopFlags* flags, hipStream_t s);
void launch_loop_lm_step_partials(const double* partial, int nsplit, int nt, int P, double lambda, double alpha, double max_step, double* step, LoopFlags* flags,
                                  double* error0_out, hipStream_t s);
constexpr int kLoopPanelMaxP = 1024;
constexpr int kLoopStreamMaxP = 192;
size_t loop_panel_solve_doubles(int P);
void launch_loop_lm_panels(const double* Hp, int P, double lambda, double alpha, double max_step, double* work, unsigned int epoch, double* step,
                           LoopFlags* flags, hipStream_t s);
bool loop_lm_stream_fits(int P);
void launch_loop_lm_stream(const double* Hp, int P, double lambda, double alpha, double max_step, double* work, unsigned int epoch, double* step,
                           LoopFlags* flags, hipStream_t s);
void launch_loop_step_finish(int P, double max_step, double* step, LoopFlags* flags, hipStream_t s);
void launch_loop_finish(const LoopModel& m, const double* state_jac, const double* state_trial, double* state0, double* paramVec, const double* step,
                        const double* error0, const double* trial_errs, int trial_nsplit, int fixed_iters, double epsilon, IterResult* result, LoopFlags* flags,
                        double* ctrl0, int chain_next, hipStream_t s, uint32_t* state_ready = nullptr ,
                        IterResult* result_slot = nullptr );

}
```

### dmsa_lidar_slam_amd/csrc/loop_kernels.hip

```cpp
#include "loop_kernels.h"
#include "wave_prims.h"

#include <cfloat>

namespace dmsa {

namespace {

constexpr int kWave = 64;

__device__ __forceinline__ void store_mat(double* dst, const Mat3& M) {
#pragma unroll
    for (int i = 0; i < 9; ++i) dst[i] = M.a[i];
}
__device__ __forceinline__ Mat3 load_mat(const double* src) {
    Mat3 M;
#pragma unroll
    for (int i = 0; i < 9; ++i) M.a[i] = src[i];
    return M;
}

__device__ void wave_relative_to_global(int n, const double* rel_o, const double* rel_t, double* glob_o, double* glob_t, double* sE, double* sR) {
    const int lane = threadIdx.x;
    for (int k = lane; k < n; k += kWave) store_mat(sE + 9 * k, so3_exp(col3(rel_o, k)));
// ... 1155 lines not shown
        double ss = 0.0;
        for (int i = 0; i < P; ++i) ss += c.org[i] * c.org[i];
        const double norm = sqrt(ss);
        int stop = 0;
        if (best == 0 && !fixed_iters)
            stop = 3;
        else if (norm < epsilon && !fixed_iters)
            stop = 4;
        s_best = best, s_stop = stop, s_norm = norm;
        result->stop = stop, result->best_k = best, result->error0 = error0, result->step_norm = norm;
        if (result_slot != nullptr) *result_slot = *result;
        if (stop != 0) flags->stop = stop;
        flags->head_k = stop == 0 && chain_next ? best : 0;
    }
    __syncthreads();
    load_state(state_trial, n, c.rel_o, c.rel_t, c.glob_o, c.glob_t);
    if (s_stop != 3) {
        const int best = s_best;
        for (int i = threadIdx.x; i < P; i += kWave) c.par[i] = best > 0 ? paramVec[i] + 0.1 * (double)best * c.org[i] : paramVec[i];
        __syncthreads();
        set_params_lds(n, c.par, c.rel_o, c.rel_t);
        if (m.model == 2) wave_relative_to_global(n, c.rel_o, c.rel_t, c.glob_o, c.glob_t, c.E, c.R);
    }
    store_state(state0, n, c.rel_o, c.rel_t, c.glob_o, c.glob_t);
    if (s_stop == 0 && chain_next) {
        __syncthreads();
        begin_body(m, c, state0, paramVec, ctrl0);
    }
}
__global__ __launch_bounds__(kWave) void k_loop_finish(const LoopModel m, const double* __restrict__ state_jac, const double* __restrict__ state_trial,
                                                       double* __restrict__ state0, double* __restrict__ paramVec, const double* __restrict__ step,
                                                       const double* __restrict__ error0_ptr, const double* __restrict__ errs, int errs_nsplit,
                                                       int fixed_iters, double epsilon, IterResult* __restrict__ result, LoopFlags* __restrict__ flags,
                                                       double* __restrict__ ctrl0, int chain_next, uint32_t* state_ready, IterResult* __restrict__ result_slot) {
    extern __shared__ double sm[];
    loop_finish_body(sm, m, state_jac, state_trial, state0, paramVec, step, error0_ptr, errs, errs_nsplit, fixed_iters, epsilon, result, flags, ctrl0, chain_next,
                     result_slot);
    DevSync sy;
    sy.signal_counter = state_ready;
    dev_sync_leave(sy);
}

}

constexpr size_t kChainLdsMax = 160 * 1024 - 256;
bool loop_chain_fits(const LoopModel& m) { return chain_lds_bytes(m) <= kChainLdsMax; }
static void chain_lds_allow(size_t bytes) {
    if (bytes <= 64 * 1024) return;
    (void)hipFuncSetAttribute(reinterpret_cast<const void*>(k_loop_begin), hipFuncAttributeMaxDynamicSharedMemorySize, (int)kChainLdsMax);
    (void)hipFuncSetAttribute(reinterpret_cast<const void*>(k_loop_chain), hipFuncAttributeMaxDynamicSharedMemorySize, (int)kChainLdsMax);
    (void)hipFuncSetAttribute(reinterpret_cast<const void*>(k_loop_finish), hipFuncAttributeMaxDynamicSharedMemorySize, (int)kChainLdsMax);
    (void)hipFuncSetAttribute(reinterpret_cast<const void*>(k_loop_chain_central), hipFuncAttributeMaxDynamicSharedMemorySize, (int)kChainLdsMax);
}
void launch_loop_chain_central(const LoopModel& m, const double* state_in, double h, double* ctrl, const LoopFlags* flags, hipStream_t s) {
    if (m.P <= 0) return;
    chain_lds_allow(chain_lds_bytes(m));
    hipLaunchKernelGGL(k_loop_chain_central, dim3(2 * m.P), dim3(kWave), chain_lds_bytes(m), s, m, state_in, h, ctrl, flags);
}
void launch_loop_begin(const LoopModel& m, double* state0, double* paramVec, double* ctrl0, LoopFlags* flags, hipStream_t s, uint32_t* state_ready) {
    chain_lds_allow(chain_lds_bytes(m));
    hipLaunchKernelGGL(k_loop_begin, dim3(1), dim3(kWave), chain_lds_bytes(m), s, m, state0, paramVec, ctrl0, flags, state_ready);
}
void launch_loop_chain(const LoopModel& m, int mode, const double* state_in, double* state_out, const double* paramVec, const double* step, double increment,
                       double* ctrl, double* extra, const LoopFlags* flags, hipStream_t s, int part, uint32_t* start_signal) {
    const int B = mode == 0 ? 1 + m.P : 9;
    chain_lds_allow(chain_lds_bytes(m));
    hipLaunchKernelGGL(k_loop_chain, dim3(B), dim3(kWave), chain_lds_bytes(m), s, m, mode, state_in, state_out, paramVec, step, increment, ctrl, extra, flags,
                       mode == 1 ? part : 0, start_signal);
// ... 43 lines not shown
void launch_loop_lm_panels(const double* Hp, int P, double lambda, double alpha, double max_step, double* work, unsigned int epoch, double* step,
                           LoopFlags* flags, hipStream_t s) {
    const int nblocks = (2 * P + kPanel - 1) / kPanel;
    const int threads = ((P + 63) / 64) * 64;
    const size_t lds = kPanelLdsHead * sizeof(double) + ((size_t)P + 2) / 2 * sizeof(double) + sizeof(double) + (size_t)P * sizeof(double) + 64;
    hipLaunchKernelGGL(k_loop_lm_panels, dim3(nblocks), dim3(threads), lds, s, Hp, P, lambda, alpha, max_step, work, epoch, step, flags);
}
__global__ __launch_bounds__(64) void k_sync_signal(uint32_t* counter) {
    if (threadIdx.x == 0) dev_sync_signal(counter);
}
__global__ __launch_bounds__(64) void k_sync_wait(const uint32_t* counter, uint32_t target, int32_t* timed_out, int max_spins, const uint32_t* counter2, uint32_t target2,
                                                  uint32_t* pass_on, BatchStamp stamp) {
    if (threadIdx.x == 0) {
        dev_sync_wait(counter, target, timed_out, max_spins);
        if (counter2 != nullptr) dev_sync_wait(counter2, target2, timed_out);
        if (pass_on != nullptr) dev_sync_signal(pass_on);
        if (stamp.ticks != nullptr) *stamp.ticks += (unsigned long long)(wall_clock64() - *stamp.begin);
    }
}
__global__ __launch_bounds__(64) void k_stamp(long long* slot) {
    if (threadIdx.x == 0) *slot = wall_clock64();
}
void launch_stamp(long long* slot, hipStream_t s) { hipLaunchKernelGGL(k_stamp, dim3(1), dim3(64), 0, s, slot); }
void launch_sync_signal(uint32_t* counter, hipStream_t s) { hipLaunchKernelGGL(k_sync_signal, dim3(1), dim3(64), 0, s, counter); }
void launch_sync_wait(const uint32_t* counter, uint32_t target, int32_t* timed_out, hipStream_t s, int max_spins, const uint32_t* counter2, uint32_t target2,
                      uint32_t* pass_on, BatchStamp stamp) {
    hipLaunchKernelGGL(k_sync_wait, dim3(1), dim3(64), 0, s, counter, target, timed_out, max_spins, counter2, target2, pass_on, stamp);
}
void launch_loop_step_finish(int P, double max_step, double* step, LoopFlags* flags, hipStream_t s) {
    hipLaunchKernelGGL(k_loop_step_finish, dim3(1), dim3(64), 0, s, P, max_step, step, flags);
}
void launch_loop_finish(const LoopModel& m, const double* state_jac, const double* state_trial, double* state0, double* paramVec, const double* step,
                        const double* error0, const double* trial_errs, int trial_nsplit, int fixed_iters, double epsilon, IterResult* result, LoopFlags* flags,
                        double* ctrl0, int chain_next, hipStream_t s, uint32_t* state_ready, IterResult* result_slot) {
    chain_lds_allow(chain_lds_bytes(m));
    hipLaunchKernelGGL(k_loop_finish, dim3(1), dim3(kWave), chain_lds_bytes(m), s, m, state_jac, state_trial, state0, paramVec, step, error0, trial_errs,
                       trial_nsplit, fixed_iters, epsilon, result, flags, ctrl0, chain_next, state_ready, result_slot);
}

}
```

### dmsa_lidar_slam_amd/csrc/optimize_loop.cpp

```cpp
#include "dmsa_ctx.h"

int build_tables(dmsa_ctx* ctx, int B, const std::vector<double>& globs, hipStream_t stream) {
    if (stream == nullptr) stream = ctx->stream;
    if (stream == ctx->stream) CHK(ctx->tables.wait_owed(ctx->stream));
    ScopedTimer tm(ctx, T_TABLE);
    const int rows = ctx->rows;
    HIPCHK(ctx->d_tables.ensure((size_t)B * rows * 48));
    const int np = ctx->model == MODEL_WINDOW ? ctx->win.ctrl.n : ctx->key.frames.n;
    if (ctx->flags & DMSA_FLAG_POSE_TABLE_HOST) {
        ctx->h_tables.resize((size_t)B * rows * 12);
        auto build_range = [&](int b0, int b1) {
            PoseChain tmp;
            tmp.resize(np);
            for (int b = b0; b < b1; ++b) {
                for (int k = 0; k < np; ++k)
                    for (int c = 0; c < 3; ++c) {
                        tmp.glob_o[3 * k + c] = globs[((size_t)b * np + k) * 6 + c];
                        tmp.glob_t[3 * k + c] = globs[((size_t)b * np + k) * 6 + 3 + c];
                    }
                float* T = &ctx->h_tables[(size_t)b * rows * 12];
                if (ctx->model == MODEL_WINDOW)
                    window_dense_table(tmp, ctx->win.stamps, ctx->win.fh, ctx->win.traj_time, T);
                else
                    keyframe_table(tmp, T);
// ... 60 lines not shown
}

int transform_points(dmsa_ctx* ctx, int b) {
    const float4* table = ctx->d_tables.as<float4>() + (size_t)b * ctx->rows * 3;
    ctx->base_table = reinterpret_cast<const float*>(table);
    if (ctx->model == MODEL_KEYFRAMES)
        launch_transform_normals(ctx->d_local.as<float4>(), ctx->d_nlocal.as<float4>(), table, ctx->d_global.as<float4>(), ctx->d_nglobal.as<float4>(),
                                 ctx->n, ctx->stream);
    else
        launch_transform(ctx->d_local.as<float4>(), table, ctx->d_global.as<float4>(), ctx->n, ctx->stream);
    HIPCHK(hipGetLastError());
    return DMSA_OK;
}


int ensure_E(dmsa_ctx* ctx, int B) {
    const int a = num_extra_rows(ctx);
    ctx->extra_rows = a;
    const int64_t ld = (((int64_t)ctx->M + a) + 31) / 32 * 32;
    ctx->ldE = ld;
    HIPCHK(ctx->d_E.ensure((size_t)B * ld * 8));
    return DMSA_OK;
}
int upload_extra(dmsa_ctx* ctx, const std::vector<double>& extra, int B) {
    const int a = ctx->extra_rows;
    const size_t need = (size_t)a * B;
    double* slot = nullptr;
    HIPCHK(ctx->h_xpin.next(need, ctx->stream, &slot));
    std::memcpy(slot, extra.data(), need * sizeof(double));
    HIPCHK(hipMemcpy2DAsync(ctx->d_E.as<double>() + ctx->M, (size_t)ctx->ldE * 8, slot, (size_t)a * 8, (size_t)a * 8, (size_t)B, hipMemcpyHostToDevice,
                            ctx->stream));
    return DMSA_OK;
}
int run_residuals(dmsa_ctx* ctx, int B, const std::vector<double>* extra, const double* d_extra, const uint32_t* rot_same, const int2* row_range) {
    CHK(ensure_E(ctx, B));
    CHK(ctx->tables.wait_owed(ctx->stream));
    const int a = ctx->extra_rows;
    if (a > 0 && d_extra != nullptr)
        launch_loop_scatter_extra(d_extra, B, a, ctx->d_E.as<double>(), ctx->ldE, ctx->M, ctx->stream);
    if (a > 0 && extra != nullptr) CHK(upload_extra(ctx, *extra, B));
    if (!ctx->order_valid) {
        ctx->err = "residuals: no size-class order (build the Gaussians first)";
        return DMSA_ERR_INVALID;
    }
    {
        HIPCHK(ctx->d_tablesT.ensure((size_t)B * ctx->rows * 48));
        const bool two = ctx->dbg.serial_streams >= 2 && ctx->serial_counts.n_long > 0;
        const bool three = two && ctx->dbg.serial_streams >= 3;
        BatchStamp stamp;
        if (ctx->dbg.batch_stamps != 0 && two && ctx->tier_join.by_counter() && ctx->d_batch_clock.p != nullptr) {
            stamp.begin = reinterpret_cast<const long long*>(ctx->d_sync.as<uint32_t>() + SYNC_BATCH_BEGIN), stamp.ticks = ctx->d_batch_clock.as<unsigned long long>();
            ctx->batch_ticks_dirty = true;
        }
        ScopedTimer tm(ctx, T_RESIDUAL, stamp.ticks != nullptr);
        if (ctx->tablesT_batch != B) launch_transpose_tables(ctx->d_tables.as<float>(), ctx->rows, B, ctx->d_tablesT.as<float>(), ctx->stream);
        hipStream_t s_long = ctx->stream;
        hipStream_t s_mid = two ? ctx->stream2 : ctx->stream;
        hipStream_t s_small = three ? ctx->stream3 : s_mid;
        const int2* gauss_rows = row_range ? ctx->d_gauss_rows.as<int2>() : nullptr;
        uint32_t* fork_signal = ctx->tier_fork.kernel_signal(ctx->stream, s_mid);
        const bool dev_sync = fork_signal != nullptr;
        if (!dev_sync) {
            CHK(ctx->tier_fork.signal(ctx->stream, s_mid));
            CHK(ctx->tier_fork.wait(s_mid, ctx->stream));
            if (three) CHK(ctx->tier_fork.wait(s_small, ctx->stream));
        }
        LongSplit split_store;
        const LongSplit* split = nullptr;
        const bool split_auto = ctx->dbg.long_split == 1 && ctx->serial_counts.n_long <= 16 && B <= 32 && ctx->model == MODEL_WINDOW;
        if ((split_auto || ctx->dbg.long_split >= 2) && ctx->serial_counts.n_long > 0 && ctx->dbg.serial_tree != 0) {
            const SerialShape shp = serial_shape(B);
            const size_t items = (size_t)ctx->serial_counts.n_long * shp.nsub_long;
            split_store.helpers = 8;
            split_store.lead_gaussians = 16;
            split_store.min_members = ctx->dbg.long_split >= 2 ? ctx->dbg.long_split : 0;
            const size_t H = (size_t)split_store.helpers;
            if (items > ctx->long_split_items) {
                const size_t cap = items + items / 2 + 16;
                HIPCHK(ctx->d_long_split.ensure(cap * (8 + 48 * 4 + H * 16 * 12) + 64));
                HIPCHK(hipMemsetAsync(ctx->d_long_split.p, 0, ctx->d_long_split.cap, ctx->stream));
                ctx->long_split_items = cap;
            }
            const size_t cap = ctx->long_split_items;
            char* w = ctx->d_long_split.as<char>();
            split_store.partial = reinterpret_cast<double*>(w), w += cap * H * 16 * 8;
            split_store.means = reinterpret_cast<float*>(w), w += cap * 48 * 4;
            split_store.partial_key = reinterpret_cast<int*>(w), w += cap * H * 16 * 4;
            split_store.done = reinterpret_cast<uint32_t*>(w), w += cap * 4;
            split_store.ready = reinterpret_cast<uint32_t*>(w);
            split_store.timed_out = StreamDep::timed_out(ctx);
            ctx->long_split_epoch += 1;
            if (ctx->long_split_epoch == 0) ctx->long_split_epoch = 1;
            split_store.epoch = ctx->long_split_epoch;
            split = &split_store;
        }
        if (dev_sync) {
            launch_residuals_serial(ctx->d_memb_local.as<float4>(), ctx->d_seg_off.as<int32_t>(), ctx->d_info12.as<float>(), ctx->d_tablesT.as<float>(), B,
                                    ctx->d_order.as<uint32_t>(), ctx->serial_counts, ctx->d_E.as<double>(), ctx->ldE, s_long, s_mid, s_small, ctx->dbg.serial_tree,
                                    fork_signal, 1, rot_same, row_range, gauss_rows, split);
            CHK(ctx->tier_fork.wait(s_mid, ctx->stream));
            if (three) CHK(ctx->tier_fork.wait(s_small, ctx->stream));
            launch_residuals_serial(ctx->d_memb_local.as<float4>(), ctx->d_seg_off.as<int32_t>(), ctx->d_info12.as<float>(), ctx->d_tablesT.as<float>(), B,
                                    ctx->d_order.as<uint32_t>(), ctx->serial_counts, ctx->d_E.as<double>(), ctx->ldE, s_long, s_mid, s_small, ctx->dbg.serial_tree, nullptr, 6,
                                    rot_same, row_range, gauss_rows);
        } else {
            launch_residuals_serial(ctx->d_memb_local.as<float4>(), ctx->d_seg_off.as<int32_t>(), ctx->d_info12.as<float>(), ctx->d_tablesT.as<float>(), B,
                                    ctx->d_order.as<uint32_t>(), ctx->serial_counts, ctx->d_E.as<double>(), ctx->ldE, s_long, s_mid, s_small, ctx->dbg.serial_tree,
                                    nullptr, 7, rot_same, row_range, gauss_rows, split);
        }
        if (dev_sync) {
            CHK(ctx->tier_join.signal(s_mid, ctx->stream));
            if (three) CHK(ctx->tier_join.signal(s_small, ctx->stream));
            WaitCarry end;
            end.stamp = stamp;
            CHK(ctx->tier_join.wait(ctx->stream, s_mid, 0, &end));
        } else {
            if (three) {
                CHK(ctx->tier_join.signal(s_small, ctx->stream, 1));
                CHK(ctx->tier_join.wait(ctx->stream, s_small, 1));
            }
            CHK(ctx->tier_join.signal(s_mid, ctx->stream));
            CHK(ctx->tier_join.wait(ctx->stream, s_mid));
        }
    }
    ctx->E_is_jacobian = false;
    ctx->residual_launches += 1;
    ctx->residual_evals += B;
    ctx->residual_bytes += 16.0 * (double)ctx->Mm + 48.0 * ctx->M + (double)B * (48.0 * ctx->rows + 8.0 * ctx->M);
    ctx->residual_unit_bytes += (double)B * (16.0 * (double)ctx->Mm + 56.0 * ctx->M + 48.0 * ctx->rows);
    HIPCHK(hipGetLastError());
    return DMSA_OK;
}


static int host_adaptive_step_size(dmsa_ctx* ctx, int P, std::vector<double>& paramVec, const std::vector<double>& step, double error0, int* bestK_out) {
    std::vector<double> globs, extra, test((size_t)P);
    int bestK = 0;
        globs.clear(), extra.clear();
        if (ctx->model == MODEL_KEYFRAMES && P >= 48) {
            const int a = num_extra_rows(ctx);
            const size_t gsz = (size_t)chain(ctx).n * 6;
            globs.resize(9 * gsz);
            extra.resize((size_t)9 * a);
            const KeyframeHost base = ctx->key;
            workers(ctx).run_all([&](int t, int nthr) {
                KeyframeHost kh = base;
                std::vector<double> tp((size_t)P), g;
// ... 483 lines not shown
    {
        PoseChain& c = chain(ctx);
        double* pin = nullptr;
        CHK(pinned_doubles(ctx, st, &pin));
        std::copy(c.rel_o.begin(), c.rel_o.end(), pin);
        std::copy(c.rel_t.begin(), c.rel_t.end(), pin + 3 * n);
        std::copy(c.glob_o.begin(), c.glob_o.end(), pin + 6 * n);
        std::copy(c.glob_t.begin(), c.glob_t.end(), pin + 9 * n);
        HIPCHK(hipMemcpyAsync(S0, pin, st * 8, hipMemcpyHostToDevice, ctx->stream));
        HIPCHK(hipMemsetAsync(ctx->d_loop_iter.p, 0, sizeof(LoopFlags) + (size_t)(num_iter + 1) * sizeof(IterResult), ctx->stream));
    }
    mark("seeded");
    long long* iter_stamps = nullptr;
    CHK(gap_stamps_begin(ctx, num_iter, &iter_stamps));
    HostLmSolve lm;
    int last_M = 0, last_M1 = 0;
    int64_t last_Mm = 0;
    int nan_evals = 0;
    hipStream_t side = ctx->dbg.dual_stream != 0 ? ctx->stream3 : ctx->stream;
    constexpr int64_t kNextHeadMinPoints = 0;
    const int head_mode = ctx->dbg.next_head;
    const bool head_on = head_mode != 0 && ctx->model == MODEL_WINDOW && ctx->n > 0 && (ctx->flags & DMSA_FLAG_STAGE_TIMERS) == 0 && (a == 0 || head_mode == 3) &&
                         (head_mode >= 2 || ctx->n >= kNextHeadMinPoints);
    if (head_on) {
        HIPCHK(ctx->d_trial_tables.ensure((size_t)9 * ctx->rows * 48));
        if (head_mode == 3) {
            HIPCHK(ctx->d_head_check.ensure((size_t)ctx->rows * 48));
            if (ctx->d_head_mismatches.p == nullptr) {
                HIPCHK(ctx->d_head_mismatches.ensure(8));
                HIPCHK(hipMemsetAsync(ctx->d_head_mismatches.p, 0, 8, ctx->stream));
            }
        }
    }
    for (int iter = 0; iter < num_iter; ++iter) {
        ctx->tl.on = ctx->dbg.host_timeline != 0, ctx->tl.reset(), ctx->tl.mark("start");
        if (iter_stamps) {
            launch_stamp(iter_stamps + 8 * iter + 0, ctx->stream);
            ctx->stamp_voxel = iter_stamps + 8 * iter + 1, ctx->stamp_fit = iter_stamps + 8 * iter + 2;
        }
        if (iter == 0)
            launch_loop_begin(m, S0, d_param, ctx->d_ctrl0.as<double>(), d_flags, ctx->stream, ctx->loop_state.kernel_signal(ctx->stream, side));
        const bool adopt = head_on && iter > 0;
        if (!adopt) {
            ScopedTimer tm(ctx, T_TABLE);
            CHK(device_tables(ctx, 1, ctx->d_ctrl0.as<double>(), ctx->d_table0.as<float>(), nullptr, ctx->stream));
        }
        ctx->base_table = ctx->d_table0.as<float>();
        if (adopt) {
            ScopedTimer tm(ctx, T_VOXEL);
            launch_transform_aabb_adopt(ctx->d_local.as<float4>(), ctx->d_table0.as<float4>(), ctx->d_trial_tables.as<float4>(), ctx->rows, &d_flags->head_k,
                                        ctx->d_global.as<float4>(), ctx->n, ctx->d_aabb.as<float>(), ctx->d_counts.p, sizeof(GaussCounts) + sizeof(SerialCounts),
                                        ctx->stream);
            ctx->aabb_fresh = true;
            ctx->next_head_iterations += 1;
            if (head_mode == 3) {
                CHK(device_tables(ctx, 1, ctx->d_ctrl0.as<double>(), ctx->d_head_check.as<float>(), nullptr, ctx->stream));
                launch_count_word_mismatches(ctx->d_table0.p, ctx->d_head_check.p, ctx->rows * 12, ctx->d_head_mismatches.as<unsigned long long>(), ctx->stream);
            }
        } else {
            ScopedTimer tm(ctx, T_VOXEL);
            launch_transform_aabb(ctx->d_local.as<float4>(), ctx->model == MODEL_KEYFRAMES ? ctx->d_nlocal.as<float4>() : nullptr, ctx->d_table0.as<float4>(),
                                  ctx->d_global.as<float4>(), ctx->model == MODEL_KEYFRAMES ? ctx->d_nglobal.as<float4>() : nullptr, ctx->n,
                                  ctx->d_aabb.as<float>(), ctx->d_counts.p, sizeof(GaussCounts) + sizeof(SerialCounts), ctx->stream);
            ctx->aabb_fresh = true;
        }
        if (!ctx->loop_state.by_counter()) CHK(ctx->loop_state.signal(ctx->stream, side));
        CHK(ctx->loop_state.wait(side, ctx->stream));
        launch_loop_chain(m, 0, S0, S1, d_param, d_step, increment, ctx->d_ctrl.as<double>(), d_extra_jac, d_flags, side);
        uint32_t* rot_same = ctx->dbg.shared_rotations != 0 && !analytic ? ctx->d_rot_same.as<uint32_t>() : nullptr;
        if (analytic) {
            launch_loop_chain_central(m, S0, kTableDerivStep, ctx->d_ctrl_pm.as<double>(), d_flags, side);
            CHK(table_derivatives(ctx, ctx->d_ctrl_pm.as<double>(), side));
            CHK(device_tables(ctx, 1, ctx->d_ctrl.as<double>(), ctx->d_tables.as<float>(), ctx->d_tablesT.as<float>(), side));
            ctx->batch = 1, ctx->tablesT_batch = 1;
        } else {
            CHK(device_tables(ctx, 1 + P, ctx->d_ctrl.as<double>(), ctx->d_tables.as<float>(), ctx->d_tablesT.as<float>(), side, rot_same));
            ctx->batch = 1 + P, ctx->tablesT_batch = 1 + P;
        }
        if (skip_mode != 0)
            launch_eval_row_ranges(m.model, ctx->d_ctrl.as<double>(), 1 + P, n, ctx->d_stamps.as<double>(), ctx->d_trajtime.as<double>(), ctx->rows - 1,
                                   ctx->d_row_range.as<int2>(), side);
        CHK(ctx->tables.signal_owed(side, ctx->stream));
        ctx->tl.mark("begin+batch enq");
        if (iter > 0 && ctx->dbg.one_readback == 0) {
            ctx->rb_extra_src = d_results + (iter - 1), ctx->rb_extra_dst = h_results + (iter - 1), ctx->rb_extra_bytes = sizeof(IterResult);
        } else {
            ctx->rb_extra_bytes = 0;
        }
        const int rc = build_gaussians(ctx, s);
        ctx->rb_extra_bytes = 0;
        CHK(rc);
        if (iter > 0 && ctx->dbg.one_readback != 0) h_results[iter - 1] = ctx->rb()->prev;
        drain_timers(ctx);
        ctx->tl.mark("build_gaussians (incl. sync A)");
        if (iter == 0) mark("first-counts");
        if (iter == 1) mark("second-counts");
        if (iter > 1 && ctx->dbg.trace_time >= 2) {
            char what[96];
            std::snprintf(what, sizeof(what), "[M %d Mm %lld grown %lld] counts", ctx->M, (long long)ctx->Mm, DevBuf::reallocations());
            mark(what);
        }
        if (iter > 0 && h_results[iter - 1].stop != 0) break;
        ++iters;
        last_M = ctx->M, last_M1 = ctx->M1, last_Mm = ctx->Mm;
        ctx->trace.push_back(dmsa_iter_trace{ctx->M, ctx->M1, ctx->Mm, 0.0, 0.0, 0, 0});
        if (ctx->M < s.min_num_gaussians) {
            stop = DMSA_STOP_FEW_GAUSSIANS;
            break;
        }
        if (analytic) {
            ctx->evaluations += 1;
            CHK(ensure_E(ctx, 1 + P));
            CHK(run_residuals(ctx, 1, nullptr));
            if (a > 0) launch_loop_scatter_extra(d_extra_jac, 1 + P, a, ctx->d_E.as<double>(), ctx->ldE, ctx->M, ctx->stream);
            CHK(analytic_columns(ctx, P, one_div_incr, ctx->d_table0.as<float>()));
        } else {
            ctx->evaluations += 1 + P;
            if (skip_mode != 0) ctx->skip_pairs += (int64_t)ctx->M * P;
            CHK(run_residuals(ctx, 1 + P, nullptr, d_extra_jac, rot_same, skip_mode == 1 ? ctx->d_row_range.as<int2>() : nullptr));
        }
        const int rowsE = ctx->M + ctx->extra_rows;
        const bool stamps = ctx->dbg.gap_stamps != 0;
        if (stamps) {
// ... 26 lines not shown
            const std::vector<double>& step = lm.step;
            for (double v : step) host_nan = host_nan || std::isnan(v);
            double* pin = nullptr;
            CHK(pinned_doubles(ctx, (size_t)P, &pin));
            std::memcpy(pin, step.data(), (size_t)P * 8);
            HIPCHK(hipMemcpyAsync(d_step, pin, (size_t)P * 8, hipMemcpyHostToDevice, ctx->stream));
            launch_loop_step_finish(P, s.max_step, d_step, d_flags, ctx->stream);
            ctx->tl.mark("solve");
        }
        if (stamps) launch_stamp(ctx->d_gap_stamps.as<long long>() + 2, ctx->stream);
        if (iter_stamps) launch_stamp(iter_stamps + 8 * iter + 5, ctx->stream);
        const bool rows_aside = ctx->dbg.trial_rows_aside != 0 && a > 0 && ctx->model == MODEL_WINDOW && ctx->trial_step.by_counter() && side != ctx->stream;
        if (rows_aside) {
            CHK(ensure_E(ctx, 9));
            launch_loop_chain(m, 1, S1, S2, d_param, d_step, increment, ctx->d_ctrl.as<double>(), d_extra_trial, d_flags, ctx->stream, 1,
                              ctx->trial_step.kernel_signal(ctx->stream, side));
            CHK(ctx->trial_step.wait(side, ctx->stream));
            launch_loop_chain(m, 1, S1, S2, d_param, d_step, increment, ctx->d_ctrl.as<double>(), d_extra_trial, d_flags, side, 2);
            launch_loop_scatter_extra(d_extra_trial, 9, a, ctx->d_E.as<double>(), ctx->ldE, ctx->M, side);
            CHK(ctx->trial_rows.signal(side, ctx->stream));
        } else {
            launch_loop_chain(m, 1, S1, S2, d_param, d_step, increment, ctx->d_ctrl.as<double>(), d_extra_trial, d_flags, ctx->stream);
        }
        {
            ScopedTimer tm(ctx, T_TABLE);
            CHK(device_tables(ctx, 9, ctx->d_ctrl.as<double>(), head_on ? ctx->d_trial_tables.as<float>() : ctx->d_tables.as<float>(), ctx->d_tablesT.as<float>(),
                              ctx->stream));
            ctx->batch = 9, ctx->tablesT_batch = 9;
        }
        if (stamps) launch_stamp(ctx->d_gap_stamps.as<long long>() + 3, ctx->stream);
        if (iter_stamps) launch_stamp(iter_stamps + 8 * iter + 6, ctx->stream);
        if (!host_nan) ctx->evaluations += 9;
        nan_evals = host_nan ? 0 : 9;
        CHK(run_residuals(ctx, 9, nullptr, rows_aside ? nullptr : d_extra_trial));
        {
            ScopedTimer tm(ctx, T_NORMAL);
            HIPCHK(ctx->d_sq_partial.ensure((size_t)squared_sums_blocked_partial_doubles(rowsE, P, 9) * 8));
            DevSync rows_in;
            if (rows_aside) ctx->trial_rows.kernel_wait(rows_in);
            launch_squared_sums_blocked(ctx->d_E.as<double>(), ctx->ldE, rowsE, P, 9, ctx->d_sq_partial.as<double>(), nullptr, ctx->stream,
                                        rows_aside ? &rows_in : nullptr);
        }
        {
            launch_loop_finish(m, S1, S2, S0, d_param, d_step, d_error0, ctx->d_sq_partial.as<double>(), normal_equations_partials(rowsE, P).nsplit, fixed ? 1 : 0,
                               s.epsilon, d_results + iter, d_flags, ctx->d_ctrl0.as<double>(), iter + 1 < num_iter ? 1 : 0, ctx->stream,
                               ctx->loop_state.kernel_signal(ctx->stream, side), ctx->dbg.one_readback != 0 ? ctx->d_prev_result() : nullptr);
        }
        if (iter_stamps) launch_stamp(iter_stamps + 8 * iter + 7, ctx->stream);
        HIPCHK(hipGetLastError());
        ctx->tl.mark("iteration enq");
        if (host_nan) break;
    }
    ctx->tl.print();
    mark("all-enqueued");
    std::vector<double> fin(st);
    {
        double* pin = nullptr;
        CHK(pinned_doubles(ctx, st, &pin));
        HIPCHK(hipMemcpyAsync(pin, S0, st * 8, hipMemcpyDeviceToHost, ctx->stream));
        if (iters > 0) HIPCHK(hipMemcpyAsync(h_results, d_results, (size_t)iters * sizeof(IterResult), hipMemcpyDeviceToHost, ctx->stream));
        HIPCHK(enqueue_batch_ticks(ctx));
        HIPCHK(hipStreamSynchronize(ctx->stream));
        std::copy(pin, pin + st, fin.begin());
    }
    mark("state-back");
    drain_timers(ctx);
    ctx->stamp_voxel = ctx->stamp_fit = nullptr;
    CHK(gap_stamps_print(ctx, iter_stamps, iters, P));
    {
        PoseChain& c = chain(ctx);
        std::copy(fin.begin(), fin.begin() + 3 * n, c.rel_o.begin());
        std::copy(fin.begin() + 3 * n, fin.begin() + 6 * n, c.rel_t.begin());
        std::copy(fin.begin() + 6 * n, fin.begin() + 9 * n, c.glob_o.begin());
        std::copy(fin.begin() + 9 * n, fin.begin() + 12 * n, c.glob_t.begin());
    }
    for (int i = 0; i < iters && i < (int)ctx->trace.size(); ++i) {
        const IterResult& r = h_results[i];
        const bool ran = !(stop == DMSA_STOP_FEW_GAUSSIANS && i == iters - 1);
        if (!ran) break;
// ... 17 lines not shown
```

### dmsa_lidar_slam_amd/csrc/voxelize_driver.cpp

```cpp
#include "dmsa_ctx.h"

int build_gaussians(dmsa_ctx* ctx, const dmsa_settings& s, const std::function<int()>& overlap, bool allow_speculation, bool allow_compression, bool allow_small) {
    const int64_t n = ctx->n;
    ctx->gaussians_valid = false;
    ctx->order_valid = false;
    ctx->M = 0, ctx->M1 = 0, ctx->Mm = 0;
    const bool lvl_on[2] = {s.grid_size_1_factor > std::numeric_limits<float>::min(), s.grid_size_2_factor > std::numeric_limits<float>::min()};
    ctx->level_res[0] = (double)(s.grid_size_1_factor * ctx->min_grid_size);
    ctx->level_res[1] = (double)(s.grid_size_2_factor * ctx->min_grid_size);
    if (!lvl_on[0]) ctx->level_res[0] = ctx->level_res[1];
    if (!lvl_on[1]) ctx->level_res[1] = ctx->level_res[0];
    const bool compress = ctx->dbg.key_compress != 0 && allow_compression;
    const bool small = allow_small && ctx->dbg.small_voxel != 0 && n <= small_voxel_max_points() && lvl_on[0] && lvl_on[1] &&
                       !(s.gauss_split != 0 && ctx->model == MODEL_KEYFRAMES) && ctx->dbg.voxel_coherence == 0;
    ctx->voxel_calls += 1;
    if (allow_speculation && ctx->dbg.speculation_fault > 0 && ctx->voxel_calls == ctx->dbg.speculation_fault)
        for (int l = 0; l < 2; ++l) {
            if (ctx->depth_guess[l] > 1) ctx->depth_guess[l] -= 1;
            if (ctx->bits_guess[l] > 3) ctx->bits_guess[l] -= 3;
        }
    const bool speculate = small || (allow_speculation && ctx->depth_guess[0] >= 0 && ctx->depth_guess[1] >= 0 && ctx->depth_guess[0] < 20 && ctx->depth_guess[1] < 20 &&
                                     (!compress || (ctx->bits_guess[0] >= 0 && ctx->bits_guess[1] >= 0)));
    const bool prehist = ctx->dbg.sort_prehist != 0;
    const bool two = ctx->dbg.dual_stream != 0 && lvl_on[0] && lvl_on[1];
    hipStream_t st[2] = {ctx->stream, two ? ctx->stream2 : ctx->stream};
    const bool by_level = (ctx->dbg.fit_by_level >= 2 || (ctx->dbg.fit_by_level == 1 && n >= 200000)) && two && !small && ctx->dbg.fused_leaf_scan != 0;
    int32_t* const gsize[2] = {ctx->d_gauss_size[0].as<int32_t>(), ctx->d_gauss_size[1].as<int32_t>()};
    uint32_t* lattice_signal = nullptr;
    {
        ScopedTimer tm(ctx, T_VOXEL);
        const int nb = (int)((n + kAabbBlock - 1) / kAabbBlock);
        if (!ctx->aabb_fresh)
            launch_block_aabb(ctx->d_global.as<float4>(), n, ctx->d_aabb.as<float>(), ctx->d_counts.p, sizeof(GaussCounts) + sizeof(SerialCounts),
                              ctx->stream);
        ctx->aabb_fresh = false;
        if (!small) lattice_signal = ctx->lattice.kernel_signal(ctx->stream, st[1], 2);
        launch_lattice(ctx->d_global.as<float4>(), n, ctx->d_aabb.as<float>(), nb, ctx->level_res[0], ctx->level_res[1], compress,
                       ctx->d_lattice.as<LatticeTable>(), ctx->d_sort_tmp[0].p, ctx->d_sort_tmp[1].p, ctx->stream,
                       lattice_signal, ctx->dbg.lattice_hint != 0 && ctx->lattice_hint_valid);
        ctx->lattice_hint_valid = true;
        if (!speculate) {
            HIPCHK(hipMemcpyAsync(ctx->h_lattice, ctx->d_lattice.p, 2 * sizeof(LatticeTable), hipMemcpyDeviceToHost, ctx->stream));
            HIPCHK(sync_spin(ctx->stream));
        }
    }
    int sort_depth[2], sort_bits[2];
    for (int l = 0; l < 2; ++l) {
        sort_depth[l] = speculate ? ctx->depth_guess[l] : ctx->h_lattice[l].final_depth;
        sort_bits[l] = !compress ? 3 * sort_depth[l] : (speculate ? ctx->bits_guess[l] : ctx->h_lattice[l].total_bits);
        if (!speculate && lvl_on[l] && ctx->h_lattice[l].status != 0) return ctx->h_lattice[l].status;
    }
    GaussCounts* counts = ctx->d_counts.as<GaussCounts>();
    const bool split = s.gauss_split != 0 && ctx->model == MODEL_KEYFRAMES;
    if (split && !ctx->d_split_stats.p) {
        HIPCHK(ctx->d_split_stats.ensure(64 * 16));
        HIPCHK(hipMemsetAsync(ctx->d_split_stats.p, 0, 64 * 16, ctx->stream));
        HIPCHK(hipStreamSynchronize(ctx->stream));
    }
    if (split)
        for (int l = 0; l < 2; ++l) {
            HIPCHK(ctx->d_pos_slot_rank[l].ensure((size_t)n * 4));
            HIPCHK(ctx->d_nsorted[l].ensure((size_t)n * 16));
            HIPCHK(ctx->d_pair_d[l].ensure(split_scratch_bytes(n)));
        }
    bool k32v[2] = {false, false};
    if (ctx->dbg.trace_time >= 3) std::fprintf(stderr, "[voxelize] key bits (without the marker of non-finite points): level 0 %d, level 1 %d\n", sort_bits[0], sort_bits[1]);
    const int tag_bit = std::max(sort_bits[0], sort_bits[1]) + 1;
    const unsigned end_bit = (unsigned)(tag_bit + 1);
    const bool k32 = small || end_bit <= 32;
    {
        const size_t ksz = k32 ? 4 : 8;
        for (int l = 0; l < 2; ++l) {
            k32v[l] = ctx->key32[l] = k32;
            ctx->code_v[l] = ctx->d_code[0].as<char>() + (size_t)l * n * ksz, ctx->code_s_v[l] = ctx->d_code_s[0].as<char>() + (size_t)l * n * ksz;
            ctx->idx_v[l] = ctx->d_idx[0].as<uint32_t>() + (size_t)l * n, ctx->idx_s_v[l] = ctx->d_idx_s[0].as<uint32_t>() + (size_t)l * n;
        }
    }
    const bool merged = ctx->dbg.merge_sort < 0 ? n <= (int64_t)(1 << 20) : ctx->dbg.merge_sort != 0;
    const bool prepared = prehist && k32;
    const int items = ctx->dbg.sort_items;
    SortPlan plan[2];
    for (int l = 0; l < 2 && !small; ++l)
        plan[l] = merged ? sort_pairs_u32_plan(ctx->d_sort_tmp[0].p, (size_t)(2 * n), end_bit, items)
                         : sort_pairs_u32_plan(ctx->d_sort_tmp[l].p, (size_t)n, (unsigned)(sort_bits[l] + 1), items);
    auto stage_keys = [&](int l, hipStream_t stream) {
        SortPlan pl = plan[l];
        if (merged && l == 1) pl.state_words = 0;
        launch_voxel_keys(ctx->d_global.as<float4>(), n, ctx->d_lattice.as<LatticeTable>() + l, ctx->level_res[l], ctx->code_v[l], k32, ctx->idx_v[l],
                          l == 0 ? 0ull : (1ull << tag_bit), prepared ? &pl : nullptr, stream);
        if (ctx->dbg.voxel_coherence != 0 && lvl_on[l]) {
            const size_t ksz = k32 ? 4 : 8;
            const bool compare = ctx->coh_valid[l] && ctx->d_code_prev[l].cap >= (size_t)n * ksz && ctx->coh_key32[l] == k32 && ctx->coh_n[l] == n;
            if (ctx->d_code_prev[l].ensure((size_t)n * ksz) != hipSuccess || ctx->d_coh_count.ensure(8) != hipSuccess) return;
            if (!ctx->coh_count_zeroed) (void)hipMemsetAsync(ctx->d_coh_count.p, 0, 8, stream), ctx->coh_count_zeroed = true;
            launch_count_code_changes(ctx->code_v[l], ctx->d_code_prev[l].p, k32, n, compare, ctx->d_coh_count.as<unsigned long long>(), stream);
            if (compare) ctx->coh_compared += n;
            ctx->coh_pending[l] = compare;
            ctx->coh_valid[l] = true, ctx->coh_key32[l] = k32, ctx->coh_n[l] = n;
        }
    };
    auto stage_sort_both = [&]() -> int {
        stage_keys(0, ctx->stream), stage_keys(1, ctx->stream);
        if (k32 && prepared)
            HIPCHK(sort_pairs_u32_onesweep(ctx->d_sort_tmp[0].p, ctx->d_sort_tmp[0].cap, ctx->d_code[0].as<uint32_t>(), ctx->d_code_s[0].as<uint32_t>(),
                                           ctx->d_idx[0].as<uint32_t>(), ctx->d_idx_s[0].as<uint32_t>(), (size_t)(2 * n), end_bit, items, ctx->stream, 2));
        else if (k32)
            HIPCHK(sort_pairs_u32_u32(ctx->d_sort_tmp[0].p, ctx->d_sort_tmp[0].cap, ctx->d_code[0].as<uint32_t>(), ctx->d_code_s[0].as<uint32_t>(),
                                      ctx->d_idx[0].as<uint32_t>(), ctx->d_idx_s[0].as<uint32_t>(), (size_t)(2 * n), end_bit, items, ctx->stream, true ));
        else
            HIPCHK(sort_pairs_u64_u32(ctx->d_sort_tmp[0].p, ctx->d_sort_tmp[0].cap, ctx->d_code[0].as<uint64_t>(), ctx->d_code_s[0].as<uint64_t>(),
                                      ctx->d_idx[0].as<uint32_t>(), ctx->d_idx_s[0].as<uint32_t>(), (size_t)(2 * n), end_bit, items, ctx->stream));
        return DMSA_OK;
    };
    auto stage_sort = [&](int l) -> int {
        stage_keys(l, st[l]);
        const unsigned eb = (unsigned)(sort_bits[l] + 1);
        if (k32 && prepared)
            HIPCHK(sort_pairs_u32_onesweep(ctx->d_sort_tmp[l].p, ctx->d_sort_tmp[l].cap, (const uint32_t*)ctx->code_v[l], (uint32_t*)ctx->code_s_v[l], ctx->idx_v[l],
                                           ctx->idx_s_v[l], (size_t)n, eb, items, st[l], 2));
        else if (k32)
            HIPCHK(sort_pairs_u32_u32(ctx->d_sort_tmp[l].p, ctx->d_sort_tmp[l].cap, (const uint32_t*)ctx->code_v[l], (uint32_t*)ctx->code_s_v[l], ctx->idx_v[l],
                                      ctx->idx_s_v[l], (size_t)n, eb, items, st[l], true ));
// ... 34 lines not shown
    };
    auto stage_gather = [&](int l, hipStream_t gs, uint32_t* start_signal = nullptr) {
        const LatticeTable* tab = ctx->d_lattice.as<LatticeTable>() + l;
        launch_gather_members(ctx->d_leaf_incl[l].as<int32_t>(), ctx->d_leaf_start[l].as<int32_t>(), ctx->idx_s_v[l],
                              ctx->code_s_v[l], k32v[l], tab, ctx->d_slot_acc[l].as<int32_t>(), ctx->d_gauss_of_slot[l].as<int32_t>(),
                              ctx->d_memb_of_slot[l].as<int32_t>(), split ? ctx->d_pos_slot_rank[l].as<int32_t>() : nullptr, ctx->d_local.as<float4>(),
                              ctx->d_slot_cnt[l].as<int32_t>(), counts, l, n, ctx->d_memb_local.as<float4>(), ctx->d_memb_idx.as<int32_t>(),
                              ctx->d_memb_g.as<int32_t>(), ctx->d_seg_off.as<int32_t>(), gs, start_signal);
    };
    if (small) {
        ScopedTimer tm(ctx, T_VOXEL);
        SmallVoxelArgs a{};
        a.global = ctx->d_global.as<float4>(), a.local = ctx->d_local.as<float4>(), a.ring = ctx->d_ring.as<int32_t>();
        a.n = (int)n, a.min_pts = s.min_num_points_per_set;
        a.tables = ctx->d_lattice.as<LatticeTable>();
        for (int l = 0; l < 2; ++l) {
            a.res[l] = ctx->level_res[l];
            a.code[l] = (uint32_t*)ctx->code_v[l], a.idx[l] = ctx->idx_v[l], a.code_s[l] = (uint32_t*)ctx->code_s_v[l], a.idx_s[l] = ctx->idx_s_v[l];
        }
        a.counts = counts;
        a.memb_local = ctx->d_memb_local.as<float4>(), a.memb_idx = ctx->d_memb_idx.as<int32_t>(), a.memb_g = ctx->d_memb_g.as<int32_t>();
        a.seg_off = ctx->d_seg_off.as<int32_t>();
        ctx->small_l0.inside_kernel(&a.sync, &a.sync_target, &a.timed_out);
        if (ctx->dbg.gap_stamps == 3) {
            HIPCHK(ctx->d_sv_stamps.ensure(2 * 16 * 8));
            a.stamps = ctx->d_sv_stamps.as<long long>();
        }
        launch_voxel_small(a, ctx->stream);
        ctx->small_voxel_launches += 1;
        HIPCHK(hipGetLastError());
    } else {
        ScopedTimer tm(ctx, T_VOXEL);
        if (merged) CHK(stage_sort_both());
        if (merged || !lattice_signal) CHK(ctx->lattice.signal(ctx->stream, st[1]));
        CHK(ctx->lattice.wait(st[1], ctx->stream));
        if (!merged)
            for (int l = 0; l < 2; ++l)
                if (lvl_on[l]) CHK(stage_sort(l));
        for (int l = 0; l < 2; ++l) {
            if (!lvl_on[l]) continue;
            CHK(stage_leaves(l));
        }
        if (!by_level) {
            CHK(ctx->level1.signal(st[1], ctx->stream));
            if (lvl_on[0]) stage_gather(0, ctx->stream);
            CHK(ctx->level1.wait(ctx->stream, st[1]));
            if (lvl_on[1]) stage_gather(1, ctx->stream);
        } else {
            uint32_t* sig = ctx->sizes0.kernel_signal(st[0], ctx->stream3);
            if (!sig) CHK(ctx->sizes0.signal(st[0], ctx->stream3));
            stage_gather(0, st[0], sig);
            WaitCarry carry;
            carry.pass_on = ctx->sizes1.kernel_signal(st[1], ctx->stream3);
            CHK(ctx->sizes0.wait(st[1], st[0], 0, &carry));
            if (!carry.pass_on) CHK(ctx->sizes1.signal(st[1], ctx->stream3));
            stage_gather(1, st[1]);
        }
    }
    hipStream_t rb = ctx->dbg.dual_stream != 0 ? ctx->stream3 : ctx->stream;
    const int auto_threshold = ctx->M > 0 ? (ctx->M < 2000 ? 8 : ctx->M < 6000 ? 32 : 0) : (n < 60000 ? 8 : n < 200000 ? 32 : 0);
    const int small_threshold = ctx->dbg.small_threshold > 0 ? ctx->dbg.small_threshold : auto_threshold;
    SerialCounts* const d_serial = reinterpret_cast<SerialCounts*>(ctx->d_counts.as<char>() + sizeof(GaussCounts));
    uint32_t* const order_level[2] = {ctx->d_order_level.as<uint32_t>(), ctx->d_order_level.as<uint32_t>() + n + 8};
    StreamDep* const sizes_dep[2] = {&ctx->sizes0, &ctx->sizes1};
    StreamDep* const classes_dep[2] = {&ctx->classes0, &ctx->classes1};
    if (!by_level) {
        DevSync sy;
        ctx->tables.kernel_wait_owed(sy);
// ... 179 lines not shown
```

### include/dmsa_debug.h

```cpp
#ifndef DMSA_DEBUG_H
#define DMSA_DEBUG_H

#include "dmsa_hip.h"

#ifdef __cplusplus
extern "C" {
#endif

typedef struct dmsa_debug_options {
    int32_t device_loop;
    int32_t dual_stream;
    int32_t serial_streams;
    int32_t merge_sort;
    int32_t key_compress;
    int32_t fused_segments;
    int32_t sort_prehist;
    int32_t overlap_batch;
    int32_t serial_tree;
    int32_t host_threads;
    int32_t solve_threads;
    int32_t host_timeline;
    int32_t trace_time;
    int32_t fused_leaf_scan;
    int32_t device_sync;
// ... 5 lines not shown
    int32_t lm_stream;
    int32_t stream_priority;
    int32_t gap_stamps;
    int32_t lattice_hint;
    int32_t fit_classes;
    int32_t eigen_l1_bytes;
    int32_t small_threshold;
    int32_t skip_stats;
    int32_t small_voxel;
    int32_t long_split;
    int32_t long_log2;
    int32_t sort_items;
    int32_t trial_rows_aside;
} dmsa_debug_options;

typedef struct dmsa_debug_counters {
    int64_t sync_retries;
    int64_t speculation_retries;
    int64_t skip_pairs;
    int64_t skip_pairs_equal;
    int64_t skip_mismatches;
    int64_t split_blocks;
    int64_t split_blocks_skipped;
    int64_t voxel_codes_compared;
    int64_t voxel_codes_changed;
    int64_t lattice_hints_held;
    int64_t lattice_replays;
    int64_t voxel_lattice_changes;
    int64_t small_voxel_launches;
    int64_t small_voxel_fallbacks;
} dmsa_debug_counters;
int dmsa_get_debug_counters(dmsa_ctx* ctx, dmsa_debug_counters* out);
int dmsa_debug_next_head(dmsa_ctx* ctx, int64_t* out2);
int dmsa_debug_level_size_classes(dmsa_ctx* ctx, int32_t* out9);
int dmsa_debug_pow_minus_one(dmsa_ctx* ctx, const int32_t* counts, int32_t count, float* out);
int dmsa_debug_limit_covariance(dmsa_ctx* ctx, const float* cov9, int64_t count, float* out9, float* evals3, float* V9, int32_t* iterations, int32_t* info);
int dmsa_sort_pairs64(dmsa_ctx* ctx, const uint64_t* keys, const uint32_t* values, int64_t n, uint32_t end_bit, uint64_t* keys_sorted, uint32_t* values_sorted);
int dmsa_scan_i32(dmsa_ctx* ctx, const int32_t* in, int64_t n, int32_t inclusive, int32_t* out);

void dmsa_default_debug_options(dmsa_debug_options* o);
int dmsa_create_ex(int device, uint32_t flags, const dmsa_debug_options* options, dmsa_ctx** out);
int dmsa_create_ex2(int device, uint32_t flags, const dmsa_debug_options* options, uint32_t options_bytes, dmsa_ctx** out);
int dmsa_create_named(int device, uint32_t flags, const dmsa_debug_options* options, uint32_t options_bytes, const char* named, dmsa_ctx** out);

#ifdef __cplusplus
}
#endif
#endif
```

Before: 1330.

## Precompute candidate lattices for all line-search trials beside residual evaluation

During the line-search residual batch, a new side stream computes per-trial bounding boxes and lattice tables for all nine trial poses. The next iteration's voxelization then adopts the winning trial's lattice instead of recomputing it. The global-point transform is also folded into the voxel-key kernel, which removes the separate transform, AABB and lattice passes from the critical path. The cost is extra speculative work for trials that are discarded, a fourth stream, and more buffers; a debug mode cross-checks the adopted tables against a recompute.

Result: no change. 1335, median of 5 (+0.4%).

```diff
diff --git a/dmsa_lidar_slam_amd/_capi.py b/dmsa_lidar_slam_amd/_capi.py
--- a/dmsa_lidar_slam_amd/_capi.py
+++ b/dmsa_lidar_slam_amd/_capi.py
@@ -318,6 +318,7 @@
         "dmsa_get_debug_counters": (C.c_int, [vp, C.POINTER(DebugCounters)]),
         "dmsa_debug_level_size_classes": (C.c_int, [vp, c_int32_p]),
         "dmsa_debug_next_head": (C.c_int, [vp, c_int64_p]),
+        "dmsa_debug_next_lattice": (C.c_int, [vp, c_int64_p]),
         "dmsa_debug_pow_minus_one": (C.c_int, [vp, c_int32_p, C.c_int32, c_float_p]),
         "dmsa_debug_limit_covariance": (C.c_int, [vp, c_float_p, C.c_int64, c_float_p, c_float_p, c_float_p, c_int32_p, c_int32_p]),
         "dmsa_sort_pairs64": (C.c_int, [vp, c_uint64_p, c_uint32_p, C.c_int64, C.c_uint32, c_uint64_p, c_uint32_p]),
@@ -426,7 +427,7 @@
 
 EXPORTED_SYMBOLS = (
     "dmsa_window_upload_aos dmsa_keyframes_upload_aos dmsa_optimize_window_aos dmsa_optimize_keyframes_aos dmsa_get_global_points_aos dmsa_reserve dmsa_window_ring_push_aos dmsa_window_upload_from_ring_aos "
-    "dmsa_create dmsa_create_ex dmsa_create_ex2 dmsa_create_named dmsa_default_debug_options dmsa_get_debug_counters dmsa_debug_next_head dmsa_debug_level_size_classes dmsa_debug_pow_minus_one dmsa_debug_limit_covariance dmsa_sort_pairs64 dmsa_scan_i32 dmsa_destroy dmsa_last_error dmsa_default_settings dmsa_optimize_window dmsa_optimize_keyframes "
+    "dmsa_create dmsa_create_ex dmsa_create_ex2 dmsa_create_named dmsa_default_debug_options dmsa_get_debug_counters dmsa_debug_next_head dmsa_debug_next_lattice dmsa_debug_level_size_classes dmsa_debug_pow_minus_one dmsa_debug_limit_covariance dmsa_sort_pairs64 dmsa_scan_i32 dmsa_destroy dmsa_last_error dmsa_default_settings dmsa_optimize_window dmsa_optimize_keyframes "
     "dmsa_get_global_points dmsa_window_upload dmsa_keyframes_upload dmsa_centralize dmsa_decentralize dmsa_get_params "
     "dmsa_set_params dmsa_additional_errors dmsa_pose_tables dmsa_set_pose_tables dmsa_num_table_rows dmsa_transform_points dmsa_build_gaussians "
     "dmsa_eval_residuals dmsa_normal_equations dmsa_pose_table_derivatives dmsa_analytic_jacobian dmsa_get_voxel_level dmsa_get_gaussians dmsa_get_timing dmsa_synchronize dmsa_get_trace dmsa_detmath_eval dmsa_lm_solve dmsa_lm_solve_device dmsa_serial_fallback_sums dmsa_sort_pairs dmsa_leaf_segments dmsa_neighbourhood_ranges dmsa_submap_poses dmsa_update_poses_from_submap dmsa_optimize_resident dmsa_adaptive_step_size dmsa_get_poses "
diff --git a/dmsa_lidar_slam_amd/api.py b/dmsa_lidar_slam_amd/api.py
--- a/dmsa_lidar_slam_amd/api.py
+++ b/dmsa_lidar_slam_amd/api.py
@@ -12,7 +12,7 @@
     pass
 
 
-NAMED_SWITCHES = ("fit_by_level", "batch_stamps", "one_readback", "next_head")
+NAMED_SWITCHES = ("fit_by_level", "batch_stamps", "one_readback", "next_head", "next_lattice")
 
 
 class DmsaOptimizer:
@@ -193,6 +193,10 @@
         head = np.zeros(2, np.int64)
         self._check(self._lib.dmsa_debug_next_head(self._ctx, capi.ptr(head, C.c_int64)), "debug_next_head")
         out["next_head_iterations"], out["next_head_mismatches"] = int(head[0]), int(head[1])
+        lat = np.zeros(4, np.int64)
+        self._check(self._lib.dmsa_debug_next_lattice(self._ctx, capi.ptr(lat, C.c_int64)), "debug_next_lattice")
+        out["next_lattice_iterations"], out["next_lattice_table_mismatches"] = int(lat[0]), int(lat[1])
+        out["next_lattice_bounds_mismatches"], out["next_lattice_point_mismatches"] = int(lat[2]), int(lat[3])
         return out
 
     def levelSizeClasses(self):
diff --git a/dmsa_lidar_slam_amd/csrc/context.cpp b/dmsa_lidar_slam_amd/csrc/context.cpp
--- a/dmsa_lidar_slam_amd/csrc/context.cpp
+++ b/dmsa_lidar_slam_amd/csrc/context.cpp
@@ -380,10 +380,11 @@
     {"one_readback", sizeof(dmsa_debug_options) + 4, 1, 0, 1},
     {"fit_by_level", sizeof(dmsa_debug_options) + 8, 1, 0, 2},
     {"next_head", sizeof(dmsa_debug_options) + 12, 1, 0, 3},
+    {"next_lattice", sizeof(dmsa_debug_options) + 16, 1, 0, 3},
 };
 #undef SW
 constexpr size_t kNumSwitches = sizeof(kSwitches) / sizeof(kSwitches[0]);
-static_assert(kNumSwitches == sizeof(dmsa_switches) / 4 && sizeof(dmsa_switches) == sizeof(dmsa_debug_options) + 16, "one table row per field of dmsa_switches");
+static_assert(kNumSwitches == sizeof(dmsa_switches) / 4 && sizeof(dmsa_switches) == sizeof(dmsa_debug_options) + 20, "one table row per field of dmsa_switches");
 constexpr bool switches_in_struct_order() {
     for (size_t i = 0; i < kNumSwitches; ++i)
         if (kSwitches[i].offset != 4 * i) return false;
@@ -460,6 +461,7 @@
         return hipStreamCreateWithPriority(st, hipStreamNonBlocking, ((dbg.stream_priority >> bit) & 1) ? prio_greatest : prio_least / 2 + prio_greatest / 2);
     };
     bool made = make_stream(&ctx->stream, 0) == hipSuccess && make_stream(&ctx->stream2, 1) == hipSuccess && make_stream(&ctx->stream3, 2) == hipSuccess &&
+                make_stream(&ctx->stream4, 3) == hipSuccess &&
                 hipEventCreateWithFlags(&ctx->ev_counts, hipEventDisableTiming) == hipSuccess;
     for (StreamDep* d : ctx->deps) made = made && d->create_events() == hipSuccess;
     if (!made) {
@@ -486,7 +488,7 @@
 void dmsa_destroy(dmsa_ctx* ctx) {
     if (!ctx) return;
     (void)hipSetDevice(ctx->device);
-    for (hipStream_t st : {ctx->stream, ctx->stream2, ctx->stream3})
+    for (hipStream_t st : {ctx->stream, ctx->stream2, ctx->stream3, ctx->stream4})
         if (st) (void)hipStreamSynchronize(st);
     drain_timers(ctx);
     for (hipEvent_t e : ctx->free_events) (void)hipEventDestroy(e);
@@ -494,7 +496,7 @@
     delete ctx->pool;
     pcd_release(ctx);
     delete ctx->sp;
-    for (hipStream_t st : {ctx->stream3, ctx->stream2, ctx->stream})
+    for (hipStream_t st : {ctx->stream4, ctx->stream3, ctx->stream2, ctx->stream})
         if (st) (void)hipStreamDestroy(st);
     delete ctx;
 }
diff --git a/dmsa_lidar_slam_amd/csrc/dev_sync.h b/dmsa_lidar_slam_amd/csrc/dev_sync.h
--- a/dmsa_lidar_slam_amd/csrc/dev_sync.h
+++ b/dmsa_lidar_slam_amd/csrc/dev_sync.h
@@ -35,6 +35,7 @@
     SYNC_CLASSES1 = 16,
     SYNC_FIT1 = 17,
     SYNC_BATCH_BEGIN = 18,
+    SYNC_CAND_LATTICE = 20,
     SYNC_SLOTS = 24
 };
 
diff --git a/dmsa_lidar_slam_amd/csrc/dmsa_api.cpp b/dmsa_lidar_slam_amd/csrc/dmsa_api.cpp
--- a/dmsa_lidar_slam_amd/csrc/dmsa_api.cpp
+++ b/dmsa_lidar_slam_amd/csrc/dmsa_api.cpp
@@ -423,6 +423,19 @@
     return DMSA_OK;
 }
 
+int dmsa_debug_next_lattice(dmsa_ctx* ctx, int64_t* out4) {
+    if (!ctx || !out4) return DMSA_ERR_INVALID;
+    CHK(set_device(ctx));
+    unsigned long long differing[3] = {0, 0, 0};
+    if (ctx->d_lattice_mismatches.p) {
+        HIPCHK(hipStreamSynchronize(ctx->stream));
+        HIPCHK(hipMemcpy(differing, ctx->d_lattice_mismatches.p, 24, hipMemcpyDeviceToHost));
+    }
+    out4[0] = ctx->next_lattice_iterations;
+    for (int k = 0; k < 3; ++k) out4[1 + k] = (int64_t)differing[k];
+    return DMSA_OK;
+}
+
 int dmsa_debug_level_size_classes(dmsa_ctx* ctx, int32_t* out9) {
     if (!ctx || !out9) return DMSA_ERR_INVALID;
     std::memset(out9, 0, 9 * sizeof(int32_t));
diff --git a/dmsa_lidar_slam_amd/csrc/dmsa_ctx.h b/dmsa_lidar_slam_amd/csrc/dmsa_ctx.h
--- a/dmsa_lidar_slam_amd/csrc/dmsa_ctx.h
+++ b/dmsa_lidar_slam_amd/csrc/dmsa_ctx.h
@@ -266,6 +266,7 @@
     int32_t one_readback = 1;
     int32_t fit_by_level = 1;
     int32_t next_head = 1;
+    int32_t next_lattice = 1;
 };
 
 struct dmsa_ctx {
@@ -274,13 +275,14 @@
     WindowRing ring;
     dmsa_switches dbg{};
     hipStream_t stream = nullptr, stream2 = nullptr;
+    hipStream_t stream4 = nullptr;
     hipStream_t stream3 = nullptr;
     StreamDep tier_fork{this, SYNC_TIER_FORK, 1}, tier_join{this, SYNC_TIER_JOIN, 2} , loop_state{this, SYNC_LOOP_STATE, 1},
         tables{this, SYNC_TABLES, 1}, classes{this, SYNC_CLASSES, 1}, lattice{this, SYNC_LATTICE, 1}, level1{this, SYNC_LEVEL1, 1}, small_l0{this, SYNC_SMALL_L0, 0},
         trial_step{this, SYNC_TRIAL_STEP, 0}, trial_rows{this, SYNC_TRIAL_ROWS, 0}, sizes0{this, SYNC_SIZES0, 1}, sizes1{this, SYNC_SIZES1, 1},
-        classes0{this, SYNC_CLASSES0, 1}, classes1{this, SYNC_CLASSES1, 1}, fit1{this, SYNC_FIT1, 1};
-    StreamDep* const deps[15] = {&tier_fork, &tier_join, &loop_state, &tables, &classes, &lattice, &level1, &small_l0, &trial_step, &trial_rows,
-                                 &sizes0, &sizes1, &classes0, &classes1, &fit1};
+        classes0{this, SYNC_CLASSES0, 1}, classes1{this, SYNC_CLASSES1, 1}, fit1{this, SYNC_FIT1, 1}, cand_lattice{this, SYNC_CAND_LATTICE, 0};
+    StreamDep* const deps[16] = {&tier_fork, &tier_join, &loop_state, &tables, &classes, &lattice, &level1, &small_l0, &trial_step, &trial_rows,
+                                 &sizes0, &sizes1, &classes0, &classes1, &fit1, &cand_lattice};
     int tablesT_batch = 0;
     hipEvent_t ev_counts = nullptr;
     std::string err;
@@ -373,6 +375,12 @@
     DevBuf d_trial_tables;
     DevBuf d_head_check, d_head_mismatches;
     int64_t next_head_iterations = 0;
+    DevBuf d_cand_aabb, d_cand_lattice;
+    DevBuf d_lattice_check, d_global_check, d_aabb_check;
+    DevBuf d_lattice_mismatches;
+    int64_t next_lattice_iterations = 0;
+    bool lattice_prepared = false;
+    bool points_pending = false;
     DevBuf d_loop_extra;
     DevBuf d_loop_iter;
     DevBuf d_panel_work;
@@ -479,8 +487,15 @@
 void host_set_params(dmsa_ctx* ctx, const double* p);
 int transform_points(dmsa_ctx* ctx, int b);
 int ensure_E(dmsa_ctx* ctx, int B);
+struct BesideBatch {
+    hipStream_t stream;
+    int signals;
+    std::function<int(hipStream_t)> first;
+    std::function<int(hipStream_t, uint32_t*)> launch;
+};
 int run_residuals(dmsa_ctx* ctx, int B, const std::vector<double>* extra, const double* d_extra = nullptr, const uint32_t* rot_same = nullptr,
-                  const int2* row_range = nullptr );
+                  const int2* row_range = nullptr ,
+                  const BesideBatch* beside = nullptr);
 int device_lm_step(dmsa_ctx* ctx, const double* d_Hp, int P, double lambda, double alpha, double max_step, double* d_step, LoopFlags* d_flags);
 constexpr double kTableDerivStep = 1e-5;
 int check_analytic_jacobian(dmsa_ctx* ctx, int P);
diff --git a/dmsa_lidar_slam_amd/csrc/dmsa_kernels.h b/dmsa_lidar_slam_amd/csrc/dmsa_kernels.h
--- a/dmsa_lidar_slam_amd/csrc/dmsa_kernels.h
+++ b/dmsa_lidar_slam_amd/csrc/dmsa_kernels.h
@@ -8,6 +8,7 @@
 
 constexpr int kMaxLatticeEvents = 64;
 constexpr int kAabbBlock = 1024;
+constexpr int kLineSearchTrials = 9;
 constexpr uint32_t kStaticRowFlag = 0;
 
 struct LatticeTable {
@@ -89,14 +90,28 @@
                            size_t zero_bytes, hipStream_t s);
 void launch_transform_aabb_adopt(const float4* local, float4* table0, const float4* trials, int rows, const int32_t* head_k, float4* global, int64_t n,
                                  float* aabb, void* zero, size_t zero_bytes, hipStream_t s);
-void launch_count_word_mismatches(const void* a, const void* b, int words, unsigned long long* count, hipStream_t s);
+void launch_count_word_mismatches(const void* a, const void* b, int words, unsigned long long* count, hipStream_t s, const int32_t* sel = nullptr,
+                                  size_t sel_stride_words = 0);
 void launch_block_aabb(const float4* global, int64_t n, float* aabb , void* zero, size_t zero_bytes, hipStream_t s);
 void launch_lattice(const float4* global, int64_t n, const float* aabb, int nb, double res0, double res1, bool compress, LatticeTable* tables ,
                     void* sort_header0, void* sort_header1, hipStream_t s, uint32_t* done = nullptr ,
                     bool use_hint = false );
 struct SortPlan;
+struct LatticeSelect {
+    const int32_t* head_k;
+    const LatticeTable* cand;
+    const float4* local;
+    float4* table0;
+    const float4* trials;
+    int rows;
+    float4* global_out;
+};
 void launch_voxel_keys(const float4* global, int64_t n, LatticeTable* table, double res, void* code, bool key32, uint32_t* idx, uint64_t code_or,
-                       const SortPlan* sort, hipStream_t s);
+                       const SortPlan* sort, hipStream_t s, const LatticeSelect* select = nullptr);
+void launch_candidate_bounds(const float4* local, const float4* trials, int rows, int64_t n, float* cand_aabb, hipStream_t s);
+void launch_lattice_candidates(const float4* local, const float4* trials, int rows, int64_t n, const float* cand_aabb, int nb, double res0, double res1, bool compress,
+                               LatticeTable* live , LatticeTable* cand , void* sort_header0, void* sort_header1, hipStream_t s, uint32_t* done,
+                               bool use_hint);
 void launch_head_flags(const void* code_sorted, bool key32, int64_t n, const LatticeTable* table, int32_t* head, hipStream_t s);
 struct ChainedScanCall {
     unsigned long long* state;
diff --git a/dmsa_lidar_slam_amd/csrc/dmsa_kernels.hip b/dmsa_lidar_slam_amd/csrc/dmsa_kernels.hip
--- a/dmsa_lidar_slam_amd/csrc/dmsa_kernels.hip
+++ b/dmsa_lidar_slam_amd/csrc/dmsa_kernels.hip
@@ -361,8 +361,95 @@
     }
     transform_aabb_body<false>(local, nullptr, table, global, nullptr, n, aabb, zero, zero_words);
 }
+__device__ __forceinline__ float wave_min_to_last(float v) {
+#define DMSA_DPP_MIN(ctrl, rows) v = fminf(v, __int_as_float(__builtin_amdgcn_update_dpp(__float_as_int(v), __float_as_int(v), ctrl, rows, 0xf, false)))
+    DMSA_DPP_MIN(0x111, 0xf);
+    DMSA_DPP_MIN(0x112, 0xf);
+    DMSA_DPP_MIN(0x114, 0xf);
+    DMSA_DPP_MIN(0x118, 0xf);
+    DMSA_DPP_MIN(0x142, 0xa);
+    DMSA_DPP_MIN(0x143, 0xc);
+#undef DMSA_DPP_MIN
+    return v;
+}
+__global__ __launch_bounds__(256) void k_candidate_bounds(const float4* __restrict__ local, const float4* __restrict__ trials, int table_f4, int64_t n,
+                                                          float* __restrict__ cand_aabb) {
+    constexpr int T = kLineSearchTrials;
+    __shared__ float s_red[4][T][6];
+    const int64_t base = (int64_t)blockIdx.x * kAabbBlock;
+    float mn[T][3], mx[T][3];
+#pragma unroll
+    for (int t = 0; t < T; ++t)
+        for (int a = 0; a < 3; ++a) mn[t][a] = INFINITY, mx[t][a] = -INFINITY;
+    constexpr int K = kAabbBlock / 256;
+    auto take = [&](const int t, const float4 r0, const float4 r1, const float4 r2, const float4 p) {
+        const float3 g = apply_row3(r0, r1, r2, p.x, p.y, p.z);
+        if (isfinite(g.x) && isfinite(g.y) && isfinite(g.z)) {
+            mn[t][0] = fminf(mn[t][0], g.x), mn[t][1] = fminf(mn[t][1], g.y), mn[t][2] = fminf(mn[t][2], g.z);
+            mx[t][0] = fmaxf(mx[t][0], g.x), mx[t][1] = fmaxf(mx[t][1], g.y), mx[t][2] = fmaxf(mx[t][2], g.z);
+        }
+    };
+    float4 pt[K];
+    bool one_row = base + kAabbBlock <= n;
+    int first_row = 0;
+    if (one_row) {
+#pragma unroll
+        for (int k = 0; k < K; ++k) pt[k] = local[base + threadIdx.x + 256 * k];
+        first_row = __builtin_amdgcn_readfirstlane(__float_as_int(pt[0].w));
+#pragma unroll
+        for (int k = 0; k < K; ++k) one_row = one_row && __float_as_int(pt[k].w) == first_row;
+        one_row = __all(one_row);
+    }
+    if (one_row) {
+#pragma unroll
+        for (int t = 0; t < T; ++t) {
+            const float4* table = trials + (size_t)t * table_f4;
+            const float4 r0 = table[3 * first_row], r1 = table[3 * first_row + 1], r2 = table[3 * first_row + 2];
+#pragma unroll
+            for (int k = 0; k < K; ++k) take(t, r0, r1, r2, pt[k]);
+        }
+    } else {
+#pragma unroll
+        for (int k = 0; k < K; ++k) {
+            const int64_t i = base + threadIdx.x + 256 * k;
+            if (i < n) {
+                const float4 p = local[i];
+                const int row = __float_as_int(p.w);
+#pragma unroll
+                for (int t = 0; t < T; ++t) {
+                    const float4* table = trials + (size_t)t * table_f4;
+                    take(t, table[3 * row], table[3 * row + 1], table[3 * row + 2], p);
+                }
+            }
+        }
+    }
+    const int wave = threadIdx.x >> 6, lane = threadIdx.x & 63;
+#pragma unroll
+    for (int t = 0; t < T; ++t)
+        for (int a = 0; a < 3; ++a) {
+            mn[t][a] = wave_min_to_last(mn[t][a]);
+            mx[t][a] = -wave_min_to_last(-mx[t][a]);
+        }
+    if (lane == 63) {
+#pragma unroll
+        for (int t = 0; t < T; ++t)
+            for (int a = 0; a < 3; ++a) s_red[wave][t][a] = mn[t][a], s_red[wave][t][3 + a] = mx[t][a];
+    }
+    __syncthreads();
+    if (threadIdx.x < 6 * T) {
+        const int t = threadIdx.x / 6, c = threadIdx.x - 6 * t;
+        float v = s_red[0][t][c];
+        for (int w = 1; w < 4; ++w) v = c < 3 ? fminf(v, s_red[w][t][c]) : fmaxf(v, s_red[w][t][c]);
+        cand_aabb[((size_t)t * gridDim.x + blockIdx.x) * 8 + c] = v;
+    }
+}
 __global__ __launch_bounds__(256) void k_count_word_mismatches(const uint32_t* __restrict__ a, const uint32_t* __restrict__ b, int words,
-                                                               unsigned long long* __restrict__ count) {
+                                                               unsigned long long* __restrict__ count, const int32_t* __restrict__ sel, size_t sel_stride_words) {
+    if (sel != nullptr) {
+        const int k = *sel;
+        if (k <= 0) return;
+        a += (size_t)(k - 1) * sel_stride_words;
+    }
     const int i = blockIdx.x * 256 + threadIdx.x;
     if (i < words && a[i] != b[i]) atomicAdd(count, 1ull);
 }
@@ -372,10 +459,14 @@
     hipLaunchKernelGGL(k_transform_aabb_adopt, dim3(nb), dim3(256), 0, s, local, table0, trials, 3 * rows, head_k, global, n, aabb, static_cast<uint32_t*>(zero),
                        (int)(zero_bytes / 4));
 }
-void launch_count_word_mismatches(const void* a, const void* b, int words, unsigned long long* count, hipStream_t s) {
+void launch_candidate_bounds(const float4* local, const float4* trials, int rows, int64_t n, float* cand_aabb, hipStream_t s) {
+    const int nb = (int)((n + kAabbBlock - 1) / kAabbBlock);
+    if (nb > 0) hipLaunchKernelGGL(k_candidate_bounds, dim3(nb), dim3(256), 0, s, local, trials, 3 * rows, n, cand_aabb);
+}
+void launch_count_word_mismatches(const void* a, const void* b, int words, unsigned long long* count, hipStream_t s, const int32_t* sel, size_t sel_stride_words) {
     if (words > 0)
         hipLaunchKernelGGL(k_count_word_mismatches, dim3((words + 255) / 256), dim3(256), 0, s, static_cast<const uint32_t*>(a), static_cast<const uint32_t*>(b),
-                           words, count);
+                           words, count, sel, sel_stride_words);
 }
 void launch_transform_aabb(const float4* local, const float4* nlocal, const float4* table, float4* global, float4* nglobal, int64_t n, float* aabb, void* zero,
                            size_t zero_bytes, hipStream_t s) {
@@ -460,19 +551,34 @@
 
 constexpr int kLatticeThreads = 1024;
 constexpr int kLatticeLdsBlocks = 2048;
-__global__ __launch_bounds__(kLatticeThreads) void k_lattice(const float4* __restrict__ global, int64_t n, const float* __restrict__ aabb, int nb, double res0,
-                                                            double res1, int compress, LatticeTable* __restrict__ tables, uint32_t* __restrict__ sort_header0,
-                                                            uint32_t* __restrict__ sort_header1, uint32_t* done ,
-                                                            int use_hint ) {
+struct StoredPoints {
+    const float4* __restrict__ global;
+    __device__ __forceinline__ float4 operator()(int64_t i) const { return global[i]; }
+};
+struct TrialPoints {
+    const float4* __restrict__ local;
+    const float4* __restrict__ table;
+    __device__ __forceinline__ float4 operator()(int64_t i) const {
+        const float4 p = local[i];
+        const int row = __float_as_int(p.w);
+        const float3 g = apply_row3(table[3 * row], table[3 * row + 1], table[3 * row + 2], p.x, p.y, p.z);
+        return make_float4(g.x, g.y, g.z, 1.0f);
+    }
+};
+template <class Points>
+__device__ __forceinline__ void lattice_body(const Points pts, int64_t n, const float* __restrict__ aabb, int nb, const double res, int compress,
+                                             const LatticeTable* hint, LatticeTable* tab, uint32_t* __restrict__ sort_header,
+                                             uint32_t* done ,
+                                             int use_hint , const bool candidate) {
     static_assert(kLatticeThreads == kAabbBlock, "one thread per point of a block");
 #ifdef DMSA_LATTICE_TIMING
     const long long lt0 = wall_clock64();
-#define LAT_STAMP(k) if (threadIdx.x == 0) tables[blockIdx.x].mn[kMaxLatticeEvents - 8 + (k)][0] = (double)(wall_clock64() - lt0);
+#define LAT_STAMP(k) if (threadIdx.x == 0) tab->mn[kMaxLatticeEvents - 8 + (k)][0] = (double)(wall_clock64() - lt0);
 #else
 #define LAT_STAMP(k)
 #endif
     {
-        uint32_t* h = blockIdx.x == 0 ? sort_header0 : sort_header1;
+        uint32_t* h = sort_header;
         if (h != nullptr)
             for (unsigned i = threadIdx.x; i < sizeof(SortHeader) / 4; i += kLatticeThreads) h[i] = 0u;
     }
@@ -483,8 +589,6 @@
     __shared__ int s_red[2][kWaves];
     __shared__ float s_bb[kLatticeLdsBlocks][6];
     int red_phase = 0;
-    LatticeTable* tab = tables + blockIdx.x;
-    const double res = blockIdx.x == 0 ? res0 : res1;
     const int tid = threadIdx.x, wave = tid >> 6, lane = tid & 63;
     if (tid == 0) {
         st.defined = 0, st.depth = 0, st.nev = 0, st.status = 0;
@@ -502,10 +606,10 @@
     __shared__ float s_fmn[kMaxLatticeEvents + 1][3], s_fmx[kMaxLatticeEvents + 1][3];
     if (use_hint && tid >= kLatticeThreads - 128 && tid - (kLatticeThreads - 128) <= kMaxLatticeEvents) {
         const int t = tid - (kLatticeThreads - 128);
-        s_tdepth[t] = tab->depth[t];
-        for (int a = 0; a < 3; ++a) s_tmn[t][a] = tab->mn[t][a];
-        if (t < kMaxLatticeEvents) s_ev[1 + t] = tab->event_idx[t];
-        if (t == 0) s_hdr[0] = tab->num_events, s_hdr[1] = tab->status, s_hdr[2] = tab->defined, s_ev[0] = tab->first_idx;
+        s_tdepth[t] = hint->depth[t];
+        for (int a = 0; a < 3; ++a) s_tmn[t][a] = hint->mn[t][a];
+        if (t < kMaxLatticeEvents) s_ev[1 + t] = hint->event_idx[t];
+        if (t == 0) s_hdr[0] = hint->num_events, s_hdr[1] = hint->status, s_hdr[2] = hint->defined, s_ev[0] = hint->first_idx;
     }
     {
         float g6[6] = {INFINITY, INFINITY, INFINITY, -INFINITY, -INFINITY, -INFINITY};
@@ -557,13 +661,13 @@
         }
         __syncthreads();
         LAT_STAMP(1)
-        if (s_ok && tid <= s_E) s_q[tid] = global[s_ev[tid]];
+        if (s_ok && tid <= s_E) s_q[tid] = pts(s_ev[tid]);
         float4 own_pt[kHintBlocks];
         const int nown = s_nown;
 #pragma unroll
         for (int k = 0; k < kHintBlocks; ++k) {
             const long long pi = k < nown ? s_own[k] * kAabbBlock + tid : n;
-            own_pt[k] = pi < n ? global[pi] : make_float4(NAN, NAN, NAN, 0.0f);
+            own_pt[k] = pi < n ? pts(pi) : make_float4(NAN, NAN, NAN, 0.0f);
         }
         __syncthreads();
         LAT_STAMP(2)
@@ -695,6 +799,12 @@
             for (int a = 0; a < 3; ++a) st.mn[a] = 0.0, st.mx[a] = 0.0;
             tab->first_idx = -1;
         }
+        if (verified && candidate && tid <= s_E) {
+            tab->depth[tid] = s_tdepth[tid];
+            for (int a = 0; a < 3; ++a) tab->mn[tid][a] = s_tmn[tid][a];
+            if (tid < s_E) tab->event_idx[tid] = s_ev[1 + tid];
+            if (tid == 0) tab->first_idx = s_ev[0];
+        }
         __syncthreads();
     }
     LAT_STAMP(5)
@@ -728,7 +838,7 @@
         float4 p = float4{0.0f, 0.0f, 0.0f, 0.0f};
         bool live = false;
         if (pi < n) {
-            p = global[pi];
+            p = pts(pi);
             live = isfinite(p.x) && isfinite(p.y) && isfinite(p.z);
         }
         int from = 0;
@@ -788,10 +898,42 @@
             }
     }
     LAT_STAMP(7)
+    if (candidate) {
+        const int nev = st.nev;
+        for (int e = nev + tid; e <= kMaxLatticeEvents; e += kLatticeThreads) {
+            tab->event_idx[e] = 0;
+            if (e > nev) {
+                tab->depth[e] = 0;
+                for (int a = 0; a < 3; ++a) tab->mn[e][a] = 0.0, tab->suffix_shift[e][a] = 0u;
+            }
+        }
+    }
     if (done != nullptr) {
         __syncthreads();
         if (threadIdx.x == 0) dev_sync_signal(done);
     }
+}
+__global__ __launch_bounds__(kLatticeThreads) void k_lattice(const float4* __restrict__ global, int64_t n, const float* __restrict__ aabb, int nb, double res0,
+                                                            double res1, int compress, LatticeTable* tables, uint32_t* __restrict__ sort_header0,
+                                                            uint32_t* __restrict__ sort_header1, uint32_t* done ,
+                                                            int use_hint ) {
+    LatticeTable* tab = tables + blockIdx.x;
+    lattice_body(StoredPoints{global}, n, aabb, nb, blockIdx.x == 0 ? res0 : res1, compress, tab, tab, blockIdx.x == 0 ? sort_header0 : sort_header1, done,
+                 use_hint, false);
+}
+__global__ __launch_bounds__(kLatticeThreads) void k_lattice_candidates(const float4* __restrict__ local, const float4* __restrict__ trials, int table_f4, int64_t n,
+                                                                       const float* __restrict__ cand_aabb, int nb, double res0, double res1, int compress,
+                                                                       LatticeTable* live, LatticeTable* cand, uint32_t* __restrict__ sort_header0,
+                                                                       uint32_t* __restrict__ sort_header1, uint32_t* done, int use_hint) {
+    const int t = blockIdx.x >> 1, l = blockIdx.x & 1;
+    if (t == 0 && threadIdx.x == 0) live[l].out_of_range = 0;
+    lattice_body(TrialPoints{local, trials + (size_t)t * table_f4}, n, cand_aabb + (size_t)t * nb * 8, nb, l == 0 ? res0 : res1, compress, live + l, cand + 2 * t + l,
+                 t == 0 ? (l == 0 ? sort_header0 : sort_header1) : nullptr, done, use_hint, true);
+}
+void launch_lattice_candidates(const float4* local, const float4* trials, int rows, int64_t n, const float* cand_aabb, int nb, double res0, double res1, bool compress,
+                               LatticeTable* live, LatticeTable* cand, void* sort_header0, void* sort_header1, hipStream_t s, uint32_t* done, bool use_hint) {
+    hipLaunchKernelGGL(k_lattice_candidates, dim3(2 * kLineSearchTrials), dim3(kLatticeThreads), 0, s, local, trials, 3 * rows, n, cand_aabb, nb, res0, res1,
+                       compress ? 1 : 0, live, cand, static_cast<uint32_t*>(sort_header0), static_cast<uint32_t*>(sort_header1), done, use_hint ? 1 : 0);
 }
 void launch_lattice(const float4* global, int64_t n, const float* aabb, int nb, double res0, double res1, bool compress, LatticeTable* tables,
                     void* sort_header0, void* sort_header1, hipStream_t s, uint32_t* done, bool use_hint) {
@@ -809,10 +951,21 @@
     return x;
 }
 
-template <typename KeyT>
+struct KeyAdopt {
+    const int32_t* head_k = nullptr;
+    const LatticeTable* cand = nullptr;
+    const float4* local = nullptr;
+    const float4* table0 = nullptr;
+    const float4* trials = nullptr;
+    int table_f4 = 0;
+    float4* global_out = nullptr;
+    float4* table0_out = nullptr;
+};
+template <typename KeyT, bool kAdopt = false>
 __global__ __launch_bounds__(256) void k_voxel_keys(const float4* __restrict__ global, int64_t n, LatticeTable* __restrict__ table, double res,
                                                     KeyT* __restrict__ code, uint32_t* __restrict__ idx, uint64_t code_or, SortHeader* __restrict__ sort_header,
-                                                    uint32_t* __restrict__ sort_state, size_t sort_state_words, int sort_passes, uint32_t sort_last_mask) {
+                                                    uint32_t* __restrict__ sort_state, size_t sort_state_words, int sort_passes, uint32_t sort_last_mask,
+                                                    const KeyAdopt adopt = KeyAdopt()) {
     __shared__ LatticeTable t;
     __shared__ uint32_t s_h[kSortMaxPasses][kSortBins];
     const bool counting = sort_header != nullptr && sizeof(KeyT) == 4;
@@ -823,10 +976,31 @@
     {
         const int words = sizeof(LatticeTable) / 4;
         const uint32_t* src = reinterpret_cast<const uint32_t*>(table);
+        if (kAdopt) {
+            const int k = *adopt.head_k;
+            if (k > 0) src = reinterpret_cast<const uint32_t*>(adopt.cand + 2 * (k - 1));
+        }
         uint32_t* dst = reinterpret_cast<uint32_t*>(&t);
         for (int i = threadIdx.x; i < words; i += blockDim.x) dst[i] = src[i];
     }
     __syncthreads();
+    const float4* pose_table = nullptr;
+    if (kAdopt) {
+        const int k = *adopt.head_k;
+        pose_table = adopt.table0;
+        if (k > 0) {
+            pose_table = adopt.trials + (size_t)(k - 1) * adopt.table_f4;
+            if (adopt.table0_out != nullptr)
+                for (int i = blockIdx.x * 256 + threadIdx.x; i < adopt.table_f4; i += gridDim.x * 256) adopt.table0_out[i] = pose_table[i];
+        }
+    }
+    if (kAdopt && blockIdx.x == 0 && *adopt.head_k > 0) {
+        uint32_t* live = reinterpret_cast<uint32_t*>(table);
+        const uint32_t* chosen = reinterpret_cast<const uint32_t*>(&t);
+        for (int i = threadIdx.x; i < (int)(offsetof(LatticeTable, out_of_range) / 4); i += blockDim.x) live[i] = chosen[i];
+        if (threadIdx.x == 0) table->pad3 = t.pad3;
+        __syncthreads();
+    }
     if (threadIdx.x == 0) t.code_or = code_or;
     if (blockIdx.x == 0 && threadIdx.x == 0) table->code_or = code_or;
     __syncthreads();
@@ -837,7 +1011,16 @@
     const int64_t last_ev = nev > 0 ? t.event_idx[nev - 1] : -1;
     const int64_t stride = (int64_t)gridDim.x * blockDim.x;
     for (int64_t i = (int64_t)blockIdx.x * blockDim.x + threadIdx.x; i < n; i += stride) {
-        const float4 p = global[i];
+        float4 p;
+        if (kAdopt) {
+            const float4 q = adopt.local[i];
+            const int row = __float_as_int(q.w);
+            const float3 g = apply_row3(pose_table[3 * row], pose_table[3 * row + 1], pose_table[3 * row + 2], q.x, q.y, q.z);
+            p = make_float4(g.x, g.y, g.z, 1.0f);
+            if (adopt.global_out != nullptr) adopt.global_out[i] = p;
+        } else {
+            p = global[i];
+        }
         uint64_t c = invalid;
         if (isfinite(p.x) && isfinite(p.y) && isfinite(p.z)) {
             int e = nev;
@@ -875,10 +1058,16 @@
     }
 }
 void launch_voxel_keys(const float4* global, int64_t n, LatticeTable* table, double res, void* code, bool key32, uint32_t* idx, uint64_t code_or,
-                       const SortPlan* sort, hipStream_t s) {
+                       const SortPlan* sort, hipStream_t s, const LatticeSelect* select) {
     if (n <= 0) return;
     SortHeader* h = sort && key32 ? sort->header : nullptr;
-    if (key32)
+    if (key32 && select) {
+        KeyAdopt a;
+        a.head_k = select->head_k, a.cand = select->cand, a.local = select->local, a.table0 = select->table0, a.trials = select->trials, a.table_f4 = 3 * select->rows;
+        a.global_out = select->global_out, a.table0_out = select->global_out != nullptr ? select->table0 : nullptr;
+        hipLaunchKernelGGL((k_voxel_keys<uint32_t, true>), dim3(grid_for(n, 256)), dim3(256), 0, s, global, n, table, res, (uint32_t*)code, idx, code_or, h,
+                           h ? sort->tile_state : nullptr, h ? sort->state_words : (size_t)0, h ? sort->passes : 0, h ? sort->last_mask : 255u, a);
+    } else if (key32)
         hipLaunchKernelGGL(k_voxel_keys<uint32_t>, dim3(grid_for(n, 256)), dim3(256), 0, s, global, n, table, res, (uint32_t*)code, idx, code_or, h,
                            h ? sort->tile_state : nullptr, h ? sort->state_words : (size_t)0, h ? sort->passes : 0, h ? sort->last_mask : 255u);
     else
diff --git a/dmsa_lidar_slam_amd/csrc/loop_kernels.h b/dmsa_lidar_slam_amd/csrc/loop_kernels.h
--- a/dmsa_lidar_slam_amd/csrc/loop_kernels.h
+++ b/dmsa_lidar_slam_amd/csrc/loop_kernels.h
@@ -58,6 +58,7 @@
 void launch_loop_finish(const LoopModel& m, const double* state_jac, const double* state_trial, double* state0, double* paramVec, const double* step,
                         const double* error0, const double* trial_errs, int trial_nsplit, int fixed_iters, double epsilon, IterResult* result, LoopFlags* flags,
                         double* ctrl0, int chain_next, hipStream_t s, uint32_t* state_ready = nullptr ,
-                        IterResult* result_slot = nullptr );
+                        IterResult* result_slot = nullptr ,
+                        void* zero = nullptr, size_t zero_bytes = 0 );
 
 }
diff --git a/dmsa_lidar_slam_amd/csrc/loop_kernels.hip b/dmsa_lidar_slam_amd/csrc/loop_kernels.hip
--- a/dmsa_lidar_slam_amd/csrc/loop_kernels.hip
+++ b/dmsa_lidar_slam_amd/csrc/loop_kernels.hip
@@ -1211,8 +1211,10 @@
                                                        double* __restrict__ state0, double* __restrict__ paramVec, const double* __restrict__ step,
                                                        const double* __restrict__ error0_ptr, const double* __restrict__ errs, int errs_nsplit,
                                                        int fixed_iters, double epsilon, IterResult* __restrict__ result, LoopFlags* __restrict__ flags,
-                                                       double* __restrict__ ctrl0, int chain_next, uint32_t* state_ready, IterResult* __restrict__ result_slot) {
+                                                       double* __restrict__ ctrl0, int chain_next, uint32_t* state_ready, IterResult* __restrict__ result_slot,
+                                                       uint32_t* __restrict__ zero, int zero_words) {
     extern __shared__ double sm[];
+    for (int i = threadIdx.x; i < zero_words; i += kWave) zero[i] = 0u;
     loop_finish_body(sm, m, state_jac, state_trial, state0, paramVec, step, error0_ptr, errs, errs_nsplit, fixed_iters, epsilon, result, flags, ctrl0, chain_next,
                      result_slot);
     DevSync sy;
@@ -1322,10 +1324,11 @@
 }
 void launch_loop_finish(const LoopModel& m, const double* state_jac, const double* state_trial, double* state0, double* paramVec, const double* step,
                         const double* error0, const double* trial_errs, int trial_nsplit, int fixed_iters, double epsilon, IterResult* result, LoopFlags* flags,
-                        double* ctrl0, int chain_next, hipStream_t s, uint32_t* state_ready, IterResult* result_slot) {
+                        double* ctrl0, int chain_next, hipStream_t s, uint32_t* state_ready, IterResult* result_slot, void* zero, size_t zero_bytes) {
     chain_lds_allow(chain_lds_bytes(m));
     hipLaunchKernelGGL(k_loop_finish, dim3(1), dim3(kWave), chain_lds_bytes(m), s, m, state_jac, state_trial, state0, paramVec, step, error0, trial_errs,
-                       trial_nsplit, fixed_iters, epsilon, result, flags, ctrl0, chain_next, state_ready, result_slot);
-}
-
-}
+                       trial_nsplit, fixed_iters, epsilon, result, flags, ctrl0, chain_next, state_ready, result_slot, static_cast<uint32_t*>(zero),
+                       (int)(zero_bytes / 4));
+}
+
+}
diff --git a/dmsa_lidar_slam_amd/csrc/optimize_loop.cpp b/dmsa_lidar_slam_amd/csrc/optimize_loop.cpp
--- a/dmsa_lidar_slam_amd/csrc/optimize_loop.cpp
+++ b/dmsa_lidar_slam_amd/csrc/optimize_loop.cpp
@@ -116,7 +116,8 @@
                             ctx->stream));
     return DMSA_OK;
 }
-int run_residuals(dmsa_ctx* ctx, int B, const std::vector<double>* extra, const double* d_extra, const uint32_t* rot_same, const int2* row_range) {
+int run_residuals(dmsa_ctx* ctx, int B, const std::vector<double>* extra, const double* d_extra, const uint32_t* rot_same, const int2* row_range,
+                  const BesideBatch* beside) {
     CHK(ensure_E(ctx, B));
     CHK(ctx->tables.wait_owed(ctx->stream));
     const int a = ctx->extra_rows;
@@ -144,6 +145,9 @@
         const int2* gauss_rows = row_range ? ctx->d_gauss_rows.as<int2>() : nullptr;
         uint32_t* fork_signal = ctx->tier_fork.kernel_signal(ctx->stream, s_mid);
         const bool dev_sync = fork_signal != nullptr;
+        const bool beside_forked = beside != nullptr && dev_sync && beside->stream != ctx->stream;
+        if (beside != nullptr) CHK(beside->first(ctx->stream));
+        if (beside != nullptr && !beside_forked) CHK(beside->launch(ctx->stream, nullptr));
         if (!dev_sync) {
             CHK(ctx->tier_fork.signal(ctx->stream, s_mid));
             CHK(ctx->tier_fork.wait(s_mid, ctx->stream));
@@ -184,6 +188,10 @@
                                     fork_signal, 1, rot_same, row_range, gauss_rows, split);
             CHK(ctx->tier_fork.wait(s_mid, ctx->stream));
             if (three) CHK(ctx->tier_fork.wait(s_small, ctx->stream));
+            if (beside_forked) {
+                CHK(ctx->tier_fork.wait(beside->stream, ctx->stream));
+                CHK(beside->launch(beside->stream, ctx->cand_lattice.kernel_signal(beside->stream, ctx->stream, beside->signals)));
+            }
             launch_residuals_serial(ctx->d_memb_local.as<float4>(), ctx->d_seg_off.as<int32_t>(), ctx->d_info12.as<float>(), ctx->d_tablesT.as<float>(), B,
                                     ctx->d_order.as<uint32_t>(), ctx->serial_counts, ctx->d_E.as<double>(), ctx->ldE, s_long, s_mid, s_small, ctx->dbg.serial_tree, nullptr, 6,
                                     rot_same, row_range, gauss_rows);
@@ -197,6 +205,7 @@
             if (three) CHK(ctx->tier_join.signal(s_small, ctx->stream));
             WaitCarry end;
             end.stamp = stamp;
+            if (beside_forked) ctx->cand_lattice.kernel_wait(end.second_wait);
             CHK(ctx->tier_join.wait(ctx->stream, s_mid, 0, &end));
         } else {
             if (three) {
@@ -746,6 +755,32 @@
             }
         }
     }
+    constexpr int64_t kNextLatticeMaxPoints = 400000;
+    const int lat_mode = ctx->dbg.next_lattice;
+    const bool lat_on = lat_mode != 0 && head_on && a == 0 && s.grid_size_1_factor > std::numeric_limits<float>::min() &&
+                        s.grid_size_2_factor > std::numeric_limits<float>::min() && !(ctx->dbg.small_voxel != 0 && ctx->n <= small_voxel_max_points()) &&
+                        (lat_mode >= 2 || ctx->n < kNextLatticeMaxPoints);
+    const int nb_aabb = (int)((ctx->n + kAabbBlock - 1) / kAabbBlock);
+    ctx->lattice_prepared = false, ctx->points_pending = false;
+    if (lat_on) {
+        HIPCHK(ctx->d_cand_aabb.ensure((size_t)kLineSearchTrials * nb_aabb * 8 * 4));
+        if (ctx->d_cand_lattice.p == nullptr) {
+            HIPCHK(ctx->d_cand_lattice.ensure((size_t)kLineSearchTrials * 2 * sizeof(LatticeTable)));
+            HIPCHK(hipMemsetAsync(ctx->d_cand_lattice.p, 0, ctx->d_cand_lattice.cap, ctx->stream));
+        }
+        if (lat_mode == 3) {
+            HIPCHK(ctx->d_lattice_check.ensure(2 * sizeof(LatticeTable)));
+            HIPCHK(ctx->d_global_check.ensure((size_t)ctx->n * 16 + 16));
+            HIPCHK(ctx->d_aabb_check.ensure((size_t)nb_aabb * 8 * 4));
+            if (ctx->d_lattice_mismatches.p == nullptr) {
+                HIPCHK(ctx->d_lattice_mismatches.ensure(24));
+                HIPCHK(hipMemsetAsync(ctx->d_lattice_mismatches.p, 0, 24, ctx->stream));
+            }
+            HIPCHK(hipMemsetAsync(ctx->d_cand_aabb.p, 0, ctx->d_cand_aabb.cap, ctx->stream));
+            HIPCHK(hipMemsetAsync(ctx->d_aabb_check.p, 0, (size_t)nb_aabb * 8 * 4, ctx->stream));
+        }
+    }
+    hipStream_t candidate_stream = ctx->dbg.dual_stream != 0 ? ctx->stream4 : ctx->stream;
     for (int iter = 0; iter < num_iter; ++iter) {
         ctx->tl.on = ctx->dbg.host_timeline != 0, ctx->tl.reset(), ctx->tl.mark("start");
         if (iter_stamps) {
@@ -762,14 +797,20 @@
         ctx->base_table = ctx->d_table0.as<float>();
         if (adopt) {
             ScopedTimer tm(ctx, T_VOXEL);
-            launch_transform_aabb_adopt(ctx->d_local.as<float4>(), ctx->d_table0.as<float4>(), ctx->d_trial_tables.as<float4>(), ctx->rows, &d_flags->head_k,
-                                        ctx->d_global.as<float4>(), ctx->n, ctx->d_aabb.as<float>(), ctx->d_counts.p, sizeof(GaussCounts) + sizeof(SerialCounts),
-                                        ctx->stream);
+            ctx->points_pending = ctx->lattice_prepared;
+            if (!ctx->points_pending)
+                launch_transform_aabb_adopt(ctx->d_local.as<float4>(), ctx->d_table0.as<float4>(), ctx->d_trial_tables.as<float4>(), ctx->rows, &d_flags->head_k,
+                                            ctx->d_global.as<float4>(), ctx->n, ctx->d_aabb.as<float>(), ctx->d_counts.p, sizeof(GaussCounts) + sizeof(SerialCounts),
+                                            ctx->stream);
             ctx->aabb_fresh = true;
             ctx->next_head_iterations += 1;
             if (head_mode == 3) {
                 CHK(device_tables(ctx, 1, ctx->d_ctrl0.as<double>(), ctx->d_head_check.as<float>(), nullptr, ctx->stream));
-                launch_count_word_mismatches(ctx->d_table0.p, ctx->d_head_check.p, ctx->rows * 12, ctx->d_head_mismatches.as<unsigned long long>(), ctx->stream);
+                if (!ctx->points_pending)
+                    launch_count_word_mismatches(ctx->d_table0.p, ctx->d_head_check.p, ctx->rows * 12, ctx->d_head_mismatches.as<unsigned long long>(), ctx->stream);
+                else
+                    launch_count_word_mismatches(ctx->d_trial_tables.p, ctx->d_head_check.p, ctx->rows * 12, ctx->d_head_mismatches.as<unsigned long long>(), ctx->stream,
+                                                 &d_flags->head_k, (size_t)ctx->rows * 12);
             }
         } else {
             ScopedTimer tm(ctx, T_VOXEL);
@@ -802,7 +843,7 @@
             ctx->rb_extra_bytes = 0;
         }
         const int rc = build_gaussians(ctx, s);
-        ctx->rb_extra_bytes = 0;
+        ctx->rb_extra_bytes = 0, ctx->lattice_prepared = false, ctx->points_pending = false;
         CHK(rc);
         if (iter > 0 && ctx->dbg.one_readback != 0) h_results[iter - 1] = ctx->rb()->prev;
         drain_timers(ctx);
@@ -895,7 +936,22 @@
         if (iter_stamps) launch_stamp(iter_stamps + 8 * iter + 6, ctx->stream);
         if (!host_nan) ctx->evaluations += 9;
         nan_evals = host_nan ? 0 : 9;
-        CHK(run_residuals(ctx, 9, nullptr, rows_aside ? nullptr : d_extra_trial));
+        BesideBatch candidates{candidate_stream, 2 * kLineSearchTrials,
+                               [&](hipStream_t cs) -> int {
+                                   launch_candidate_bounds(ctx->d_local.as<float4>(), ctx->d_trial_tables.as<float4>(), ctx->rows, ctx->n, ctx->d_cand_aabb.as<float>(), cs);
+                                   return DMSA_OK;
+                               },
+                               [&](hipStream_t cs, uint32_t* done) -> int {
+                                   launch_lattice_candidates(ctx->d_local.as<float4>(), ctx->d_trial_tables.as<float4>(), ctx->rows, ctx->n, ctx->d_cand_aabb.as<float>(),
+                                                             nb_aabb, ctx->level_res[0], ctx->level_res[1], ctx->dbg.key_compress != 0, ctx->d_lattice.as<LatticeTable>(),
+                                                             ctx->d_cand_lattice.as<LatticeTable>(), ctx->d_sort_tmp[0].p, ctx->d_sort_tmp[1].p, cs, done,
+                                                             ctx->dbg.lattice_hint != 0 && ctx->lattice_hint_valid);
+                                   HIPCHK(hipGetLastError());
+                                   return DMSA_OK;
+                               }};
+        const bool prepare = lat_on && iter + 1 < num_iter && !host_nan;
+        CHK(run_residuals(ctx, 9, nullptr, rows_aside ? nullptr : d_extra_trial, nullptr, nullptr, prepare ? &candidates : nullptr));
+        ctx->lattice_prepared = prepare;
         {
             ScopedTimer tm(ctx, T_NORMAL);
             HIPCHK(ctx->d_sq_partial.ensure((size_t)squared_sums_blocked_partial_doubles(rowsE, P, 9) * 8));
@@ -907,7 +963,8 @@
         {
             launch_loop_finish(m, S1, S2, S0, d_param, d_step, d_error0, ctx->d_sq_partial.as<double>(), normal_equations_partials(rowsE, P).nsplit, fixed ? 1 : 0,
                                s.epsilon, d_results + iter, d_flags, ctx->d_ctrl0.as<double>(), iter + 1 < num_iter ? 1 : 0, ctx->stream,
-                               ctx->loop_state.kernel_signal(ctx->stream, side), ctx->dbg.one_readback != 0 ? ctx->d_prev_result() : nullptr);
+                               ctx->loop_state.kernel_signal(ctx->stream, side), ctx->dbg.one_readback != 0 ? ctx->d_prev_result() : nullptr,
+                               ctx->d_counts.p, ctx->lattice_prepared ? sizeof(GaussCounts) + sizeof(SerialCounts) : 0);
         }
         if (iter_stamps) launch_stamp(iter_stamps + 8 * iter + 7, ctx->stream);
         HIPCHK(hipGetLastError());
diff --git a/dmsa_lidar_slam_amd/csrc/voxelize_driver.cpp b/dmsa_lidar_slam_amd/csrc/voxelize_driver.cpp
--- a/dmsa_lidar_slam_amd/csrc/voxelize_driver.cpp
+++ b/dmsa_lidar_slam_amd/csrc/voxelize_driver.cpp
@@ -27,6 +27,20 @@
     const bool by_level = (ctx->dbg.fit_by_level >= 2 || (ctx->dbg.fit_by_level == 1 && n >= 200000)) && two && !small && ctx->dbg.fused_leaf_scan != 0;
     int32_t* const gsize[2] = {ctx->d_gauss_size[0].as<int32_t>(), ctx->d_gauss_size[1].as<int32_t>()};
     uint32_t* lattice_signal = nullptr;
+    const bool candidates_ready = ctx->lattice_prepared, points_pending = ctx->points_pending;
+    ctx->lattice_prepared = false, ctx->points_pending = false;
+    bool guess32 = false;
+    if (speculate && !small) {
+        const int b0 = !compress ? 3 * ctx->depth_guess[0] : ctx->bits_guess[0], b1 = !compress ? 3 * ctx->depth_guess[1] : ctx->bits_guess[1];
+        guess32 = std::max(b0, b1) + 2 <= 32;
+    }
+    const bool adopt_lattice = candidates_ready && points_pending && !small && speculate && guess32 && lvl_on[0] && lvl_on[1] && allow_compression;
+    const int32_t* const head_k = candidates_ready ? &ctx->d_loop_iter.as<LoopFlags>()->head_k : nullptr;
+    const bool keys_transform = adopt_lattice && points_pending;
+    const bool check = adopt_lattice && ctx->dbg.next_lattice == 3;
+    if (points_pending && !adopt_lattice)
+        launch_transform_aabb_adopt(ctx->d_local.as<float4>(), ctx->d_table0.as<float4>(), ctx->d_trial_tables.as<float4>(), ctx->rows, head_k,
+                                    ctx->d_global.as<float4>(), n, ctx->d_aabb.as<float>(), ctx->d_counts.p, sizeof(GaussCounts) + sizeof(SerialCounts), ctx->stream);
     {
         ScopedTimer tm(ctx, T_VOXEL);
         const int nb = (int)((n + kAabbBlock - 1) / kAabbBlock);
@@ -34,10 +48,27 @@
             launch_block_aabb(ctx->d_global.as<float4>(), n, ctx->d_aabb.as<float>(), ctx->d_counts.p, sizeof(GaussCounts) + sizeof(SerialCounts),
                               ctx->stream);
         ctx->aabb_fresh = false;
-        if (!small) lattice_signal = ctx->lattice.kernel_signal(ctx->stream, st[1], 2);
-        launch_lattice(ctx->d_global.as<float4>(), n, ctx->d_aabb.as<float>(), nb, ctx->level_res[0], ctx->level_res[1], compress,
-                       ctx->d_lattice.as<LatticeTable>(), ctx->d_sort_tmp[0].p, ctx->d_sort_tmp[1].p, ctx->stream,
-                       lattice_signal, ctx->dbg.lattice_hint != 0 && ctx->lattice_hint_valid);
+        if (adopt_lattice) {
+            ctx->next_lattice_iterations += 1;
+            if (check) {
+                constexpr int kTableWords = (int)(offsetof(LatticeTable, out_of_range) / 4), kSlotWords = (int)(2 * sizeof(LatticeTable) / 4);
+                unsigned long long* differing = ctx->d_lattice_mismatches.as<unsigned long long>();
+                launch_transform_aabb_adopt(ctx->d_local.as<float4>(), ctx->d_table0.as<float4>(), ctx->d_trial_tables.as<float4>(), ctx->rows, head_k,
+                                            ctx->d_global_check.as<float4>(), n, ctx->d_aabb_check.as<float>(), nullptr, 0, ctx->stream);
+                HIPCHK(hipMemsetAsync(ctx->d_lattice_check.p, 0, 2 * sizeof(LatticeTable), ctx->stream));
+                launch_lattice(ctx->d_global_check.as<float4>(), n, ctx->d_aabb_check.as<float>(), nb, ctx->level_res[0], ctx->level_res[1], compress,
+                               ctx->d_lattice_check.as<LatticeTable>(), nullptr, nullptr, ctx->stream);
+                for (int l = 0; l < 2; ++l)
+                    launch_count_word_mismatches(ctx->d_cand_lattice.as<LatticeTable>() + l, ctx->d_lattice_check.as<LatticeTable>() + l, kTableWords, differing,
+                                                 ctx->stream, head_k, kSlotWords);
+                launch_count_word_mismatches(ctx->d_cand_aabb.p, ctx->d_aabb_check.p, nb * 8, differing + 1, ctx->stream, head_k, (size_t)nb * 8);
+            }
+        } else {
+            if (!small) lattice_signal = ctx->lattice.kernel_signal(ctx->stream, st[1], 2);
+            launch_lattice(ctx->d_global.as<float4>(), n, ctx->d_aabb.as<float>(), nb, ctx->level_res[0], ctx->level_res[1], compress,
+                           ctx->d_lattice.as<LatticeTable>(), ctx->d_sort_tmp[0].p, ctx->d_sort_tmp[1].p, ctx->stream,
+                           lattice_signal, ctx->dbg.lattice_hint != 0 && ctx->lattice_hint_valid);
+        }
         ctx->lattice_hint_valid = true;
         if (!speculate) {
             HIPCHK(hipMemcpyAsync(ctx->h_lattice, ctx->d_lattice.p, 2 * sizeof(LatticeTable), hipMemcpyDeviceToHost, ctx->stream));
@@ -86,8 +117,12 @@
     auto stage_keys = [&](int l, hipStream_t stream) {
         SortPlan pl = plan[l];
         if (merged && l == 1) pl.state_words = 0;
+        const LatticeSelect choose{head_k, ctx->d_cand_lattice.as<LatticeTable>() + l, ctx->d_local.as<float4>(), ctx->d_table0.as<float4>(),
+                                   ctx->d_trial_tables.as<float4>(), ctx->rows, l == 0 ? ctx->d_global.as<float4>() : nullptr};
         launch_voxel_keys(ctx->d_global.as<float4>(), n, ctx->d_lattice.as<LatticeTable>() + l, ctx->level_res[l], ctx->code_v[l], k32, ctx->idx_v[l],
-                          l == 0 ? 0ull : (1ull << tag_bit), prepared ? &pl : nullptr, stream);
+                          l == 0 ? 0ull : (1ull << tag_bit), prepared ? &pl : nullptr, stream, adopt_lattice ? &choose : nullptr);
+        if (check && l == 0)
+            launch_count_word_mismatches(ctx->d_global.p, ctx->d_global_check.p, (int)(n * 4), ctx->d_lattice_mismatches.as<unsigned long long>() + 2, stream);
         if (ctx->dbg.voxel_coherence != 0 && lvl_on[l]) {
             const size_t ksz = k32 ? 4 : 8;
             const bool compare = ctx->coh_valid[l] && ctx->d_code_prev[l].cap >= (size_t)n * ksz && ctx->coh_key32[l] == k32 && ctx->coh_n[l] == n;
@@ -188,8 +223,12 @@
     } else {
         ScopedTimer tm(ctx, T_VOXEL);
         if (merged) CHK(stage_sort_both());
-        if (merged || !lattice_signal) CHK(ctx->lattice.signal(ctx->stream, st[1]));
-        CHK(ctx->lattice.wait(st[1], ctx->stream));
+        if (keys_transform && !merged) {
+            CHK(ctx->loop_state.wait(st[1], ctx->stream));
+        } else {
+            if (merged || !lattice_signal) CHK(ctx->lattice.signal(ctx->stream, st[1]));
+            CHK(ctx->lattice.wait(st[1], ctx->stream));
+        }
         if (!merged)
             for (int l = 0; l < 2; ++l)
                 if (lvl_on[l]) CHK(stage_sort(l));
diff --git a/include/dmsa_debug.h b/include/dmsa_debug.h
--- a/include/dmsa_debug.h
+++ b/include/dmsa_debug.h
@@ -61,6 +61,7 @@
 } dmsa_debug_counters;
 int dmsa_get_debug_counters(dmsa_ctx* ctx, dmsa_debug_counters* out);
 int dmsa_debug_next_head(dmsa_ctx* ctx, int64_t* out2);
+int dmsa_debug_next_lattice(dmsa_ctx* ctx, int64_t* out4);
 int dmsa_debug_level_size_classes(dmsa_ctx* ctx, int32_t* out9);
 int dmsa_debug_pow_minus_one(dmsa_ctx* ctx, const int32_t* counts, int32_t count, float* out);
 int dmsa_debug_limit_covariance(dmsa_ctx* ctx, const float* cov9, int64_t count, float* out9, float* evals3, float* V9, int32_t* iterations, int32_t* info);
```
